# piljoong-jeong/nerf_meets_mlx

Hardware: AMD Instinct MI355X
Metric: train+render rays/sec on Lego 800x800 (synthetic), coarse+fine 64+128 (higher is better)
Workload: dtype split16 (fp16x2 render / bf16x2 train MFMA operands ~ 22 / 16 significand bits; fp32 accumulate)

## Files before the change

nerf_meets_mlx_amd/csrc/mlp.hip:

```cpp
#include "common.h"
#include "mlp_ring.h"
#include "mlp_layout.h"
#include "mlp_frag.h"
#include "mlp_arch2.h"
#include "mlp_input2.h"
#include "mlp_pack.h"
#include "hash_common.h"
#include "mlp_params.h"
#include "mlp_model.h"
#include "dw_split.h"
#include <limits.h>
#include <string.h>


namespace nerf {

extern int g_hash_combine_max_res;







// ... 781 lines not shown
      const int n = t - nw;
      src = base + 64 * 1024 + n;
      dst = a.grads + jb.b_off + n;
      if (jb.aux_row0 > 0) {
        if (n >= jb.aux_row0) dst = a.aux + (jb.n_valid - jb.aux_row0) * jb.k_valid + (n - jb.aux_row0);
        else if (n >= jb.n_grad) continue;
      }
    }
    float sum = 0.0f;
    int sidx = 0;
    for (; sidx + 8 <= S; sidx += 8) {
      float v[8];
#pragma unroll
      for (int q = 0; q < 8; ++q) v[q] = __builtin_nontemporal_load(src + (size_t)(sidx + q) * DW_SLOT_FLOATS);
#pragma unroll
      for (int q = 0; q < 8; ++q) sum += v[q];
    }
    for (; sidx < S; ++sidx) sum += __builtin_nontemporal_load(src + (size_t)sidx * DW_SLOT_FLOATS);
    *dst = sum;
  }
}



static_assert(LI::F_CHUNKS * RING_CHUNK == LI::F_TOTAL && LI::B_CHUNKS * RING_CHUNK == LI::B_PADDED, "whole ring chunks");

template <bool STORE, class WS>
__device__ __forceinline__ void fwd_tiles_img(const ImgArgs& a, WS& ws, int64_t tile0, int64_t ntiles, int lane) {
  constexpr int ST = 1;
  const int r = lane & 31, h = lane >> 5;
  int64_t tile = tile0 < ntiles ? tile0 : ntiles - 1;
  int64_t m = tile * 32 + r; if (m >= a.M) m = a.M - 1;
  bf16x8 xin[ST][3];
#pragma unroll
  for (int ks = 0; ks < 3; ++ks) row_pairs<CvtBf16>(a.x + m * LI::CIN, ks, h, LI::CIN, xin[0][ks]);
  int bad = nonfinite_flags<32>(nonfinite_bits(xin[0][0]) | nonfinite_bits(xin[0][1]) | nonfinite_bits(xin[0][2]), 0u);
  asm volatile("" : "+v"(bad));
  if (STORE) { store_frags<3>(a.acts, tile0, a.astride, LI::A_X, xin[0], r, h); ws.note_stores(3); }
  bf16x8 ha[ST][16], hb[ST][16];
  u32x4 mk[ST];
#define IMG_LAYER(KS, FB, BS, IN, OUT, LYR)                                                        \
  do { mk[0] = u32x4{0u, 0u, 0u, 0u};                                                              \
       layer_fwd<ST, KS, 8, true, STORE>(ws, FB, BS, IN, OUT, mk, lane);                           \
       if (STORE) { store_frags<16>(a.acts, tile0, a.astride, LI::A_H0 + 16 * (LYR), OUT[0], r, h); \
                    *reinterpret_cast<u32x4*>(frag_ptr(a.acts, tile0, a.astride, LI::A_MASK + (LYR), r, h)) = mk[0]; ws.note_stores(17); } } while (0)
  IMG_LAYER(3, LI::F_L0, 0, xin, ha, 0);
  IMG_LAYER(16, LI::F_L1 + 0 * 128, 256, ha, hb, 1);
  IMG_LAYER(16, LI::F_L1 + 1 * 128, 512, hb, ha, 2);
  IMG_LAYER(16, LI::F_L1 + 2 * 128, 768, ha, hb, 3);
  IMG_LAYER(16, LI::F_L1 + 3 * 128, 1024, hb, ha, 4);
  {
    bf16x8 cat[ST][19];
    if (STORE) {
#pragma unroll
      for (int k = 0; k < 3; ++k) xin[0][k] = *frag_ptr(a.acts, tile0, a.astride, LI::A_X + k, r, h);
    }
#pragma unroll
    for (int k = 0; k < 3; ++k) cat[0][k] = xin[0][k];
#pragma unroll
    for (int k = 0; k < 16; ++k) cat[0][3 + k] = ha[0][k];
    IMG_LAYER(19, LI::F_L5, 1280, cat, hb, 5);
  }
  IMG_LAYER(16, LI::F_L6, 1536, hb, ha, 6);
  IMG_LAYER(16, LI::F_L7, 1792, ha, hb, 7);
#undef IMG_LAYER
  f32x16 acc;
  acc_init_bias(acc, ws, LI::BI_OUT, h);
#pragma unroll
  for (int ks = 0; ks < 16; ++ks) {
    const bf16x8 wo = next_frag(ws, LI::F_OUT + ks, lane);
    acc = __builtin_amdgcn_mfma_f32_32x32x16_bf16(wo, hb[0][ks], acc, 0, 0, 0);
  }
  const int64_t mo = tile0 * 32 + r;
  if (h == 0 && tile0 < ntiles && mo < a.M) {
#pragma unroll
    for (int c = 0; c < 4; ++c)
      if (c < a.out_ch) a.out[mo * a.out_ch + c] = bad ? __builtin_nanf("") : acc[c];
  }
}

template <bool STORE>
__global__ void __launch_bounds__(512, 2) mlp_img_fwd_ring_kernel(ImgArgs a) {
  const int lane = threadIdx.x & 63;
  const int wv = __builtin_amdgcn_readfirstlane(threadIdx.x >> 6);
  const int64_t ntiles = (a.M + 31) >> 5, nsuper = (ntiles + 7) >> 3;
  RingW<LI::F_CHUNKS, LI::F_TOTAL, (STORE ? 2 : 4)> ws;
  ws.wsrc = reinterpret_cast<const char*>(a.wf);
  ws.lane16 = 16 * lane;
  ws.lds0 = __builtin_amdgcn_readfirstlane(lds_addr_of(ring_smem));
  ws.wv = wv;
  ws.start(lane);
  ring_load_bias(a.bias, LI::BI_TOTAL);
  __syncthreads();
  for (int64_t sp = blockIdx.x; sp < nsuper; sp += gridDim.x) {
    int ln = lane;
    asm volatile("" : "+v"(ln));
    ws.new_pass();
    fwd_tiles_img<STORE>(a, ws, sp * 8 + wv, ntiles, ln);
  }
  ws.drain();
}

__global__ void __launch_bounds__(512, 2) mlp_img_bwd_ring_kernel(ImgArgs a) {
  constexpr int ST = 1;
  const int lane0 = threadIdx.x & 63;
  const int wv = __builtin_amdgcn_readfirstlane(threadIdx.x >> 6);
  const int64_t ntiles = (a.M + 31) >> 5, nsuper = (ntiles + 7) >> 3;
  RingW<LI::B_CHUNKS, LI::B_TOTAL> ws;
  ws.wsrc = reinterpret_cast<const char*>(a.wb);
  ws.lane16 = 16 * lane0;
  ws.lds0 = __builtin_amdgcn_readfirstlane(lds_addr_of(ring_smem));
  ws.wv = wv;
  ws.start(lane0);
  for (int64_t sp = blockIdx.x; sp < nsuper; sp += gridDim.x) {
    int lane = lane0;
    asm volatile("" : "+v"(lane));
    ws.new_pass();
    const int r = lane & 31, h = lane >> 5;
    const int64_t tile0 = sp * 8 + wv;
    const int64_t tile = tile0 < ntiles ? tile0 : ntiles - 1;
    const int64_t m = tile * 32 + r;
    bf16x8 zo[ST][1];
#pragma unroll
    for (int j = 0; j < 8; ++j) zo[0][0][j] = (__bf16)0.0f;
    if (tile0 < ntiles && m < a.M && h == 0) {
#pragma unroll
      for (int c = 0; c < 4; ++c)
        if (c < a.out_ch) zo[0][0][c] = (__bf16)a.d_out[m * a.out_ch + c];
    }
    u32x4 mk[8][ST];
#pragma unroll
    for (int l = 0; l < 8; ++l)
      mk[l][0] = *reinterpret_cast<const u32x4*>(frag_ptr(a.acts, tile, a.astride, LI::A_MASK + l, r, h));
    store_frags<1>(a.dz, tile0, a.zstride, LI::Z_OUT, zo[0], r, h); ws.note_stores(1);
    bf16x8 za[ST][16], zb[ST][16];
    layer_bwd<ST, 1, 8, true>(ws, LI::B_OUT, zo, zb, mk[7], lane);
    store_frags<16>(a.dz, tile0, a.zstride, LI::Z_L0 + 112, zb[0], r, h); ws.note_stores(16);
    layer_bwd<ST, 16, 8, true>(ws, LI::B_L7 + 0 * 128, zb, za, mk[6], lane);
    store_frags<16>(a.dz, tile0, a.zstride, LI::Z_L0 + 96, za[0], r, h); ws.note_stores(16);
    layer_bwd<ST, 16, 8, true>(ws, LI::B_L7 + 1 * 128, za, zb, mk[5], lane);
    store_frags<16>(a.dz, tile0, a.zstride, LI::Z_L0 + 80, zb[0], r, h); ws.note_stores(16);
    layer_bwd<ST, 16, 8, true>(ws, LI::B_L7 + 2 * 128, zb, za, mk[4], lane);
    store_frags<16>(a.dz, tile0, a.zstride, LI::Z_L0 + 64, za[0], r, h); ws.note_stores(16);
    layer_bwd<ST, 16, 8, true>(ws, LI::B_L7 + 3 * 128, za, zb, mk[3], lane);
    store_frags<16>(a.dz, tile0, a.zstride, LI::Z_L0 + 48, zb[0], r, h); ws.note_stores(16);
    layer_bwd<ST, 16, 8, true>(ws, LI::B_L7 + 4 * 128, zb, za, mk[2], lane);
    store_frags<16>(a.dz, tile0, a.zstride, LI::Z_L0 + 32, za[0], r, h); ws.note_stores(16);
    layer_bwd<ST, 16, 8, true>(ws, LI::B_L7 + 5 * 128, za, zb, mk[1], lane);
    store_frags<16>(a.dz, tile0, a.zstride, LI::Z_L0 + 16, zb[0], r, h); ws.note_stores(16);
    layer_bwd<ST, 16, 8, true>(ws, LI::B_L7 + 6 * 128, zb, za, mk[0], lane);
    store_frags<16>(a.dz, tile0, a.zstride, LI::Z_L0 + 0, za[0], r, h); ws.note_stores(16);
  }
  ws.drain();
}



struct LdsW {
  __device__ __forceinline__ bf16x8 frag(int f, int lane) { return *reinterpret_cast<const bf16x8*>(ring_smem + f * 1024 + lane * 16); }
  __device__ __forceinline__ void note_stores(int) {}
  __device__ __forceinline__ float4 bias4(int slot) { return *reinterpret_cast<const float4*>(ring_smem + 32 * 1024 + slot * 4); }
};
__device__ __forceinline__ void lds_load_stream(const bf16x8* __restrict__ w, const float* __restrict__ bias) {
  for (int i = threadIdx.x; i < 32 * 64; i += blockDim.x) *reinterpret_cast<bf16x8*>(ring_smem + i * 16) = w[i];
  if (bias)
    for (int i = threadIdx.x; i < LN::BI_TOTAL; i += blockDim.x) *reinterpret_cast<float*>(ring_smem + 32 * 1024 + 4 * i) = bias[i];
  __syncthreads();
}


template <bool STORE, bool FUSED, bool LW = false>
__global__ void __launch_bounds__(512) mlp_small_fwd_kernel(SmallArgs a) {
  constexpr int ST = 1;
  lds_load_stream(a.wf, a.bias);
  const int lane0 = threadIdx.x & 63, wv = threadIdx.x >> 6;
  const bool rmaj = FUSED && !STORE && a.ray_major;
  const int64_t ntiles = rmaj ? ((a.B + 31) >> 5) * a.n : (a.M + 31) >> 5;
  LdsW ws;
  for (int64_t tile0 = (int64_t)blockIdx.x * 8 + wv; tile0 < ntiles; tile0 += (int64_t)gridDim.x * 8) {
    int lane = lane0;
    asm volatile("" : "+v"(lane));
    const int r = lane & 31, h = lane >> 5;
    const TileSample ts = small_tile_sample(a, tile0, r, rmaj);
    const int64_t m = ts.m;
    const bool valid = ts.valid;
    bf16x8 in[3];
    if (FUSED) {
      if (a.tables_h) ngp_row<true, LW, CvtBf16>(a, m, h, in);
      else ngp_row<false, LW, CvtBf16>(a, m, h, in);
    } else {
      small_row<CvtBf16>(a.x + m * LN::CIN, h, in);
    }
    bf16x8 xin[ST][2], din[ST][1];
    xin[0][0] = in[0]; xin[0][1] = in[1]; din[0][0] = in[2];
    int bad = nonfinite_flags<32>(nonfinite_bits(xin[0][0]) | nonfinite_bits(xin[0][1]), nonfinite_bits(din[0][0]));
    asm volatile("" : "+v"(bad));
#define SINK(slot0) FragSink<STORE>{a.acts, tile0, a.astride, slot0, r, h}
#define MASK_STORE(layer) do { if (STORE) *reinterpret_cast<u32x4*>(frag_ptr(a.acts, tile0, a.astride, LN::A_MASK + (layer), r, h)) = mk[0]; } while (0)
    if (STORE) { store_frags<2>(a.acts, tile0, a.astride, LN::A_X, xin[0], r, h); store_frags<1>(a.acts, tile0, a.astride, LN::A_DX, din[0], r, h); }
    u32x4 mk[ST];
    bf16x8 h0[ST][4], h1[ST][4], ft[ST][4];
    mk[0] = u32x4{0u, 0u, 0u, 0u};
    layer_fwd<ST, 2, 2, true, STORE>(ws, LN::F_L0, LN::BI_L0, xin, h0, mk, lane, SINK(LN::A_H0));
    MASK_STORE(0);
    mk[0] = u32x4{0u, 0u, 0u, 0u};
    layer_fwd<ST, 4, 2, true, STORE>(ws, LN::F_L1, LN::BI_L1, h0, h1, mk, lane, SINK(LN::A_H1));
    MASK_STORE(1);
    layer_fwd<ST, 4, 2, false, false>(ws, LN::F_FA, LN::BI_FEAT, h1, ft, mk, lane, SINK(LN::A_FEAT));
    float alpha;
    {
      f32x16 acc;
      acc_init_bias(acc, ws, LN::BI_ALPHA, h);
#pragma unroll
      for (int ks = 0; ks < 4; ++ks) acc = __builtin_amdgcn_mfma_f32_32x32x16_bf16(ws.frag(LN::F_FA + 8 + ks, lane), h1[0][ks], acc, 0, 0, 0);
      alpha = acc[0];
    }
    bf16x8 hd[ST][2];
    {
      bf16x8 cat[ST][5];
#pragma unroll
      for (int k = 0; k < 4; ++k) cat[0][k] = ft[0][k];
      cat[0][4] = din[0][0];
      mk[0] = u32x4{0u, 0u, 0u, 0u};
      layer_fwd<ST, 5, 1, true, STORE>(ws, LN::F_DIR, LN::BI_DIR, cat, hd, mk, lane, SINK(LN::A_HD));
      MASK_STORE(2);
    }
    {
      f32x16 acc;
      acc_init_bias(acc, ws, LN::BI_RGB, h);
#pragma unroll
      for (int ks = 0; ks < 2; ++ks) acc = __builtin_amdgcn_mfma_f32_32x32x16_bf16(ws.frag(LN::F_RGB + ks, lane), hd[0][ks], acc, 0, 0, 0);
      if (h == 0 && valid) {
        float4 o; o.x = acc[0]; o.y = acc[1]; o.z = acc[2]; o.w = alpha;
        *reinterpret_cast<float4*>(a.out + m * 4) = poison_raw(o, bad);
      }
    }
#undef SINK
#undef MASK_STORE
  }
}

__global__ void __launch_bounds__(512) mlp_small_bwd_kernel(SmallArgs a) {
  constexpr int ST = 1;
  lds_load_stream(a.wb, nullptr);
  const int lane0 = threadIdx.x & 63, wv = threadIdx.x >> 6;
  const int64_t ntiles = (a.M + 31) >> 5;
  LdsW ws;
  for (int64_t tile0 = (int64_t)blockIdx.x * 8 + wv; tile0 < ntiles; tile0 += (int64_t)gridDim.x * 8) {
    int lane = lane0;
    asm volatile("" : "+v"(lane));
    const int r = lane & 31, h = lane >> 5;
    const int64_t m = tile0 * 32 + r;
    float4 g = make_float4(0.f, 0.f, 0.f, 0.f);
    if (m < a.M && h == 0) g = *reinterpret_cast<const float4*>(a.d_raw + m * 4);
    bf16x8 zrgb[ST][1], zal[ST][1];
#pragma unroll
    for (int j = 0; j < 8; ++j) { zrgb[0][0][j] = (__bf16)0.0f; zal[0][0][j] = (__bf16)0.0f; }
    zrgb[0][0][0] = (__bf16)g.x; zrgb[0][0][1] = (__bf16)g.y; zrgb[0][0][2] = (__bf16)g.z;
    zal[0][0][0] = (__bf16)g.w;
    u32x4 mk[3][ST];
#pragma unroll
    for (int l = 0; l < 3; ++l)
      mk[l][0] = *reinterpret_cast<const u32x4*>(frag_ptr(const_cast<void*>(a.acts), tile0, a.astride, LN::A_MASK + l, r, h));
    store_frags<1>(a.dz, tile0, a.zstride, LN::Z_RGB, zrgb[0], r, h);
    store_frags<1>(a.dz, tile0, a.zstride, LN::Z_A, zal[0], r, h);
#define ZSINK(slot0) FragSink<true>{a.dz, tile0, a.zstride, slot0, r, h}
    bf16x8 zd[ST][2], zf[ST][4], z1[ST][4], z0[ST][4];
    layer_bwd<ST, 1, 1, true>(ws, LN::B_RGB, zrgb, zd, mk[2], lane, ZSINK(LN::Z_D));
    layer_bwd<ST, 2, 2, false>(ws, LN::B_DIR, zd, zf, mk[2], lane, ZSINK(LN::Z_F));
    {
      bf16x8 cat[ST][5];
#pragma unroll
      for (int k = 0; k < 4; ++k) cat[0][k] = zf[0][k];
      cat[0][4] = zal[0][0];
      layer_bwd<ST, 5, 2, true>(ws, LN::B_FA, cat, z1, mk[1], lane, ZSINK(LN::Z_L1));
    }
    layer_bwd<ST, 4, 2, true>(ws, LN::B_L1, z1, z0, mk[0], lane, ZSINK(LN::Z_L0));
#undef ZSINK
    if (a.d_x) {
      f32x16 acc;
#pragma unroll
      for (int i = 0; i < 16; ++i) acc[i] = 0.0f;
#pragma unroll
      for (int ns = 0; ns < 4; ++ns) acc = __builtin_amdgcn_mfma_f32_32x32x16_bf16(ws.frag(LN::B_L0 + ns, lane), z0[0][ns], acc, 0, 0, 0);
      if (m < a.M) {
#pragma unroll
        for (int q = 0; q < 4; ++q) {
          float4 o; o.x = acc[4 * q]; o.y = acc[4 * q + 1]; o.z = acc[4 * q + 2]; o.w = acc[4 * q + 3];
          *reinterpret_cast<float4*>(a.d_x + m * LN::CPOS + 8 * q + 4 * h) = o;
        }
      }
    }
  }
}

static int g_dw_wgs = 0;
static int g_dw_bias = -1;
static int g_bwd_stage = 0;
static int g_dw_ring_cap = 8;
static int g_dw_private = 4;
static int g_dw16_variant = 1;
static int g_dw_narrow_first = 1;
static int g_dw_factor = 1;
static int g_dw_job_mask = 0;
static int g_mlp_variant = 0;
static int g_ring_wgs = 0;
static int g_ngp_ray_major = 1;
int g_pass_queue = 1;
static int g_ring_split = 1;

static int cu_count() {
  constexpr int MAX_DEVICES = 64;
  static int n[MAX_DEVICES] = {};
  int dev = 0;
  if (hipGetDevice(&dev) != hipSuccess || dev < 0 || dev >= MAX_DEVICES) dev = 0;
  if (n[dev] == 0) {
    int v = 0;
    n[dev] = (hipDeviceGetAttribute(&v, hipDeviceAttributeMultiprocessorCount, dev) == hipSuccess && v > 0) ? v : 256;
  }
  return n[dev];
}
static inline int ring_wgs() { return g_ring_wgs > 0 ? g_ring_wgs : cu_count(); }
static inline unsigned ring_grid(int64_t ntiles) { return persistent_grid((ntiles + 7) / 8, ring_wgs()); }

struct Option { const char* key; int* var; bool (*rule)(int& v); const char* refusal; };
static bool opt_any(int&) { return true; }
static bool opt_flag(int& v) { v = v ? 1 : 0; return true; }
template <int LO, int HI> static bool opt_clamp(int& v) { v = v < LO ? LO : v > HI ? HI : v; return true; }
static const Option OPTIONS[] = {
    {"mlp_variant", &g_mlp_variant, opt_any, nullptr},
    {"ring_split", &g_ring_split, [](int& v) { return v == 1 || v == 2; }, "nerf_set_option: ring_split must be 1 or 2"},
    {"ring_workgroups", &g_ring_wgs, opt_clamp<0, INT_MAX>, nullptr},
    {"tile_pad16", &g_tile_pad16, opt_clamp<0, INT_MAX>, nullptr},
    {"dw_workgroups", &g_dw_wgs, opt_clamp<0, INT_MAX>, nullptr},
    {"dw_unit_bias", &g_dw_bias, opt_clamp<-1, INT_MAX>, nullptr},
    {"bwd_stage", &g_bwd_stage, opt_any, nullptr},
    {"dw_job_mask", &g_dw_job_mask, opt_any, nullptr},
    {"hash_combine_max_res", &g_hash_combine_max_res, opt_clamp<0, INT_MAX>, nullptr},
    {"ngp_ray_major", &g_ngp_ray_major, opt_flag, nullptr},
    {"dw22_variant", &s16::g_dw_variant, opt_flag, nullptr},
    {"dw16_variant", &g_dw16_variant, opt_clamp<0, 3>, nullptr},
    {"dw_private_tiles", &g_dw_private, opt_clamp<0, 4>, nullptr},
    {"dw_ring_cap", &g_dw_ring_cap, opt_clamp<2, 16>, nullptr},
    {"pass_queue", &g_pass_queue, opt_flag, nullptr},
    {"dw_narrow_first", &g_dw_narrow_first, opt_flag, nullptr},
    {"dw_factor", &g_dw_factor, opt_flag, nullptr},
    {"f22_tiles", &f22::g_tiles, [](int& v) { return v == 0 || v == 2 || v == 3; }, "nerf_set_option: f22_tiles must be 0 (automatic), 2 or 3"},
};

}

using namespace nerf;

extern "C" int nerf_set_option(const char* key, int value) {
  NERF_REQUIRE(key, NERF_E_NULL, "nerf_set_option: key is NULL");
  NERF_REQUIRE(strcmp(key, "mlp_precision") != 0, NERF_E_UNSUPPORTED,
               "nerf_set_option: \"mlp_precision\" is gone (ABI 3): set nerf_mlp_arch.precision of the model instead");
  for (const Option& o : OPTIONS) {
    if (strcmp(key, o.key)) continue;
    if (!o.rule(value)) return fail(NERF_E_UNSUPPORTED, "%s", o.refusal);
    *o.var = value;
    return NERF_OK;
  }
  return fail(NERF_E_UNSUPPORTED, "nerf_set_option: unknown key '%s'", key);
}

extern "C" int nerf_get_option(const char* key) {
  if (!key) return NERF_OPTION_UNKNOWN;
  for (const Option& o : OPTIONS)
    if (!strcmp(key, o.key)) return *o.var;
  return NERF_OPTION_UNKNOWN;
}

extern "C" int64_t nerf_mlp_param_count(const nerf_mlp_arch* arch) { return resolve(arch).params; }
extern "C" int64_t nerf_mlp_packed_bytes(const nerf_mlp_arch* arch) { return resolve(arch).packed_bytes; }
extern "C" int64_t nerf_mlp_acts_bytes(const nerf_mlp_arch* arch, int64_t M) { return resolve(arch).acts_bytes(M); }
extern "C" int64_t nerf_mlp_dz_bytes(const nerf_mlp_arch* arch, int64_t M) { return resolve(arch).dz_bytes(M); }

#define NERF_ARCH_MSG ": HIP kernels exist for (8x256, skip 4) with in=63+27 view head, or in=40 / no view head / out_ch<=4, and for (2x64, no skip) with in=32+16 view head"
#define NERF_RESOLVE(who)        \
  const Model m = resolve(arch); \
  NERF_REQUIRE(m.ok, NERF_E_UNSUPPORTED, who NERF_ARCH_MSG)

extern "C" int nerf_mlp_pack(const nerf_mlp_arch* arch, const float* params, void* packed, void* stream) {
  NERF_RESOLVE("nerf_mlp_pack");
  NERF_REQUIRE(params && packed, NERF_E_NULL, "nerf_mlp_pack: params/packed is NULL");
  auto s = as_stream(stream);
  bf16x8* wf = m.stream<bf16x8>(packed, S_FWD);
  bf16x8* wb = m.stream<bf16x8>(packed, S_BWD);
  float* bias = m.stream<float>(packed, S_BIAS);
  int rc;
  if (m.shape == Shape::Small) {
    rc = launch<pack_streams_kernel<SmallPack, CvtBf16, true>>("nerf_mlp_pack (2x64 model)", dim3(pack_blocks<SmallPack, true>()), dim3(256), 0, s,
                                                               params, wf, wb, bias, 0);
    if (!rc && m.split()) rc = s16x::small_pack(params, m.stream<void>(packed, S_S16), s);
  } else if (m.shape == Shape::Image) {
    rc = launch<pack_streams_kernel<ImgPack, CvtBf16, true>>("nerf_mlp_pack (image model)", dim3(pack_blocks<ImgPack, true>()), dim3(256), 0, s,
                                                             params, wf, wb, bias, m.out_ch);
    if (!rc && m.split()) rc = s16x::img_pack(params, m.out_ch, m.stream<void>(packed, S_S16), s);
    if (!rc && m.prec == Prec::F32) rc = f32::pack(params, m.stream<void>(packed, S_F32), m.out_ch, s);
  } else {
    rc = launch<pack_kernel>("nerf_mlp_pack", dim3(PACK_BLOCKS + PACK16_BLOCKS), dim3(256), 0, s, params, wf, wb, bias,
                             m.stream<bf16x8>(packed, S_FWD16));
    if (!rc && m.prec == Prec::F32) rc = f32::pack(params, m.stream<void>(packed, S_F32), 0, s);
    if (!rc && m.split()) rc = f22::pack(params, m.stream<void>(packed, S_F22), s);
    if (!rc && m.split()) rc = s16::pack(params, m.stream<void>(packed, S_S16), s);
  }
  return rc;
}

template <int MODE>
static int launch_fwd(const Model& m, const void* packed, const float* x, const float* rays, const float* z, int64_t M, int n,
                      int freq_mode, float* out, void* acts, void* stream) {
  FwdArgs a;
  a.queue = nullptr;
  a.wf = m.stream<bf16x8>(packed, S_FWD);
  a.bias = m.stream<float>(packed, S_BIAS);
  a.x = x; a.rays = rays; a.z = z; a.M = M; a.n = n; a.out = out; a.acts = acts; a.astride = m.astride();
  fill_freqs(a.fr.pos, a.fr.dir, freq_mode);
  const int64_t ntiles = (M + 31) / 32;
  auto s = as_stream(stream);
  const int variant = (g_mlp_variant == 0) ? (MODE == 1 ? (acts ? 3 : 4) : 1) : g_mlp_variant;
  if ((variant == 4 || variant == 5) && MODE == 1 && !acts) {
    const dim3 g(persistent_grid((M + 255) / 256, ring_wgs()));
    FwdArgs a16 = a;
    a16.queue = passq_slot();
    a16.wf = m.stream<bf16x8>(packed, S_FWD16);
    const char* what = "mlp forward (ring, 16x16x32)";
    if (variant == 4) return launch<mlp_fwd_ring16_kernel<8, 2>, mlp_fwd_ring16_kernel<4, 4>>(what, g, dim3(512), RING16_LDS_BYTES, s, a16);
    return launch<mlp_fwd_ring16_kernel<4, 4>, mlp_fwd_ring16_kernel<8, 2>>(what, g, dim3(256), RING16_LDS_BYTES, s, a16);
  }
  if (variant >= 3 && MODE == 1) {
    a.queue = passq_slot();
    if (acts && g_ring_split == 2) {
      return launch<mlp_fwd_ring_kernel<1, true, SPLIT_NW, SPLIT_CHUNK>>(
          "mlp forward (ring, 2 workgroups per CU)", dim3(persistent_grid((ntiles + SPLIT_NW - 1) / SPLIT_NW, 2 * (int64_t)ring_wgs())),
          dim3(64 * SPLIT_NW), SPLIT_LDS_BYTES, s, a);
    }
    return with_bool(acts != nullptr, [&](auto store) {
      constexpr bool ST = decltype(store)::value;
      return launch<mlp_fwd_ring_kernel<1, ST>, mlp_fwd_ring_kernel<1, !ST>>("mlp forward (ring)", dim3(ring_grid(ntiles)), dim3(512),
                                                                              RING_LDS_BYTES, s, a);
    });
  }
  const int st = variant == 2 ? 2 : 1;
  const int64_t blocks = (ntiles + 4 * st - 1) / (4 * st);
  NERF_REQUIRE(blocks < (1ll << 31), NERF_E_SHAPE, "mlp forward: M too large");
  return with_bool(st == 1, [&](auto one) { return with_bool(acts != nullptr, [&](auto store) {
    return launch<mlp_fwd_kernel<decltype(one)::value ? 1 : 2, MODE, decltype(store)::value>>("mlp forward", dim3((unsigned)blocks), dim3(256),
                                                                                                0, s, a);
  }); });
}


static int view_forward(const Model& m, const void* packed, const float* x, const float* rays, const float* z, int64_t M, int n,
                        int freq_mode, float* out, void* acts, void* stream);

extern "C" int nerf_mlp_forward_train(const nerf_mlp_arch* arch, const void* packed, const float* x, int64_t M,
                                      float* out, void* acts, void* stream) {
  NERF_RESOLVE("nerf_mlp_forward");
  if (M <= 0) return NERF_OK;
  NERF_REQUIRE(packed && x && out, NERF_E_NULL, "nerf_mlp_forward: NULL pointer");
  auto s = as_stream(stream);
  if (m.shape == Shape::Small) {
    SmallArgs a;
    small_args(a, m, packed);
    a.x = x; a.out = out; a.acts = acts; a.M = M;
    if (m.split()) return s16x::small_forward(a, false, dim3(small_grid(small_tiles(a))), s);
    return with_bool(acts != nullptr, [&](auto store) {
      return launch<mlp_small_fwd_kernel<decltype(store)::value, false>>("mlp forward (2x64 model)", dim3(small_grid((M + 31) / 32)), dim3(512),
                                                                         LN::LDS_BYTES, s, a);
    });
  }
  if (m.shape == Shape::Image) {
    if (m.prec == Prec::F32)
      return f32::forward(m.stream<void>(packed, S_F32), x, nullptr, nullptr, M, 1, 0, out, acts, m.out_ch, s);
    ImgArgs a;
    img_args(a, m, packed);
    a.x = x; a.out = out; a.acts = acts; a.M = M;
    if (m.split()) return s16x::img_forward(a, ring_wgs(), s);
    return with_bool(acts != nullptr, [&](auto store) {
      constexpr bool ST = decltype(store)::value;
      return launch<mlp_img_fwd_ring_kernel<ST>, mlp_img_fwd_ring_kernel<!ST>>("mlp forward (image model)", dim3(ring_grid((M + 31) / 32)),
                                                                               dim3(512), RING_LDS_BYTES, s, a);
    });
  }
  return view_forward(m, packed, x, nullptr, nullptr, M, 1, 0, out, acts, stream);
}

static int view_forward(const Model& m, const void* packed, const float* x, const float* rays, const float* z, int64_t M, int n,
                        int freq_mode, float* out, void* acts, void* stream) {
  auto s = as_stream(stream);
  if (m.split() && !acts)
    return f22::forward(m.stream<void>(packed, S_F22), x, rays, z, M, n, freq_mode, out, ring_wgs(), s);
  if (m.split())
    return s16::forward(m.stream<void>(packed, S_S16), m.stream<float>(packed, S_BIAS), x, rays, z, M, n, freq_mode, out, acts,
                        m.astride(), ring_wgs(), s);
  if (m.prec == Prec::F32) return f32::forward(m.stream<void>(packed, S_F32), x, rays, z, M, n, freq_mode, out, acts, 0, s);
  return x ? launch_fwd<0>(m, packed, x, rays, z, M, n, freq_mode, out, acts, stream)
           : launch_fwd<1>(m, packed, x, rays, z, M, n, freq_mode, out, acts, stream);
}

extern "C" int nerf_mlp_forward(const nerf_mlp_arch* arch, const void* packed, const float* x, int64_t M, float* out,
                                void* stream) {
  return nerf_mlp_forward_train(arch, packed, x, M, out, nullptr, stream);
}

extern "C" int nerf_query_fused(const nerf_mlp_arch* arch, const void* packed, const float* rays, const float* z,
                                int64_t B, int n, int freq_mode, float* raw, void* acts, void* stream) {
  const Model m = resolve(arch);
  NERF_REQUIRE(m.ok && m.shape == Shape::View, NERF_E_UNSUPPORTED, "nerf_query_fused" NERF_ARCH_MSG);
  NERF_REQUIRE(n >= 1, NERF_E_SHAPE, "nerf_query_fused: n must be >= 1");
  if (B <= 0) return NERF_OK;
  NERF_REQUIRE(packed && rays && z && raw, NERF_E_NULL, "nerf_query_fused: NULL pointer");
  NERF_REQUIRE(freq_mode == 0 || freq_mode == 1, NERF_E_UNSUPPORTED, "nerf_query_fused: freq_mode must be 0 or 1");
  NERF_REQUIRE(B * (int64_t)n < (1ll << 31), NERF_E_SHAPE, "nerf_query_fused: B*n must be < 2^31 samples per call");
  return view_forward(m, packed, nullptr, rays, z, B * n, n, freq_mode, raw, acts, stream);
}

static int launch_dw_part(const Model& m, DwArgs& d, int nj, int64_t ntiles, const void* acts, void* dz, float* grads,
                          hipStream_t s, int kind, int slot_base, int max_wgs, int aux_slot = -1) {
  static_assert(DW_SPLIT_MAX_JOBS == DW_MAX_JOBS, "dw_split.h sizes its arrays for DwArgs::jobs");
  DwCost cost[DW_MAX_JOBS];
  constexpr int SHARED_JOB_EXTRA_UNITS = 12;
  for (int j = 0; j < nj; ++j) cost[j] = DwCost{d.jobs[j].nf, d.jobs[j].kf + (d.jobs[j].aux_row0 > 0 ? SHARED_JOB_EXTRA_UNITS : 0)};
  int target_wgs = g_dw_wgs > 0 ? g_dw_wgs : cu_count();
  if (target_wgs > max_wgs) target_wgs = max_wgs;
  const int nw = dw_split(cost, nj, g_dw_bias >= 0 ? g_dw_bias : m.split() ? 2 : 128, target_wgs, (ntiles + 3) / 4, d.splits);
  NERF_REQUIRE(slot_base + nw <= DW_MAX_WGS, NERF_E_SHAPE, "nerf_mlp_backward: dw_workgroups must be <= %d", DW_MAX_WGS);
  bool all_tiny = true;
  for (int j = 0; j < nj; ++j) all_tiny = all_tiny && ((d.jobs[j].nf + 1) / 2) * ((d.jobs[j].kf + 1) / 2) <= 4;
  d.ntiles = (int)ntiles; d.astride = m.astride(); d.zstride = m.zstride();
  d.acts = acts; d.dz = dz; d.grads = grads;
  d.a_lo = m.info->a_lo; d.z_lo = m.info->z_lo; d.ring_cap = g_dw_ring_cap; d.private_max_tiles = g_dw_private;
  d.partial = m.dw_partial(dz, ntiles) + (size_t)slot_base * DW_SLOT_FLOATS;
  d.aux = aux_slot >= 0 ? m.dw_partial(dz, ntiles) + (size_t)aux_slot * DW_SLOT_FLOATS : nullptr;
  int rc;
  if (kind >= 2) {
    rc = launch_dw_wide_kernel(d, nw, kind == 2, s);
  } else if (kind == 1) {
    rc = s16::launch_dw_kernel(d, nw, true, s);
  } else if (g_dw16_variant == 3 || (g_dw16_variant == 1 && all_tiny)) {
    rc = s16::launch_dw_kernel(d, nw, false, s);
  } else {
    rc = launch<mlp_dw_kernel>("mlp dW", dim3(nw), dim3(64 * DW_WAVES), DW_LDS_BYTES, s, d);
  }
  if (rc) return rc;
  return launch<mlp_dw_reduce_kernel>("mlp dW reduce", dim3(257, nj), dim3(256), 0, s, d);
}

static int launch_dw(const Model& m, const void* packed, DwArgs& d, int nj, int64_t ntiles, const void* acts, void* dz, float* grads,
                     hipStream_t s, bool factored) {
  if (g_dw_job_mask) {
    hipError_t e = hipMemsetAsync(grads, 0, sizeof(float) * m.params, s);
    if (e != hipSuccess) return fail(NERF_E_HIP, "nerf_mlp_backward: memset: %s", hipGetErrorString(e));
  }
  const bool split_bf16 = m.split();
  if ((split_bf16 ? s16::g_dw_variant : g_dw16_variant) == 0)
    return launch_dw_part(m, d, nj, ntiles, acts, dz, grads, s, split_bf16 ? 1 : 0, 0, DW_MAX_WGS);
  DwArgs wide = d, rest = d;
  int nwide = 0, nrest = 0;
  for (int j = 0; j < nj; ++j) {
    if (d.jobs[j].nf == 16 && d.jobs[j].kf == 16) wide.jobs[nwide++] = d.jobs[j];
    else rest.jobs[nrest++] = d.jobs[j];
  }
  const int half = DW_MAX_WGS / 2;
  for (int turn = 0; turn < 2; ++turn) {
    const bool do_wide = (turn == 0) != (g_dw_narrow_first != 0);
    if (do_wide && nwide) {
      const int rc = launch_dw_part(m, wide, nwide, ntiles, acts, dz, grads, s, split_bf16 ? 2 : 3, half, half);
      if (rc) return rc;
    }
    if (!do_wide && nrest) {
      int rc = launch_dw_part(m, rest, nrest, ntiles, acts, dz, grads, s, split_bf16 ? 1 : 0, 0, half, factored ? half : -1);
      if (!rc && factored)
        rc = launch_dw_factor_post(m.stream<void>(packed, S_S16), m.stream<float>(packed, S_BIAS), rest.aux, grads, s);
      if (rc) return rc;
    }
  }
  return NERF_OK;
}

static int view_backward_chain(const Model& m, const void* packed, const void* acts, const float* d_raw, int64_t M, void* dz,
                               hipStream_t s) {
  const int64_t ntiles = (M + 31) / 32;
  if (m.split()) {
    if (g_bwd_stage != 2) {
      const int rcs = s16::backward_chain(m.stream<void>(packed, S_S16), acts, d_raw, M, dz, m.astride(), m.zstride(), ring_wgs(), s);
      if (rcs) return rcs;
    }
    return check_launch("mlp backward chain");
  }
  BwdArgs b;
  b.queue = nullptr;
  b.wb = m.stream<bf16x8>(packed, S_BWD);
  b.acts = acts; b.d_raw = d_raw; b.M = M; b.dz = dz; b.astride = m.astride(); b.zstride = m.zstride();
  const int variant = g_mlp_variant == 0 ? 3 : g_mlp_variant;
  const char* what = "mlp backward chain";
  if (variant >= 3) {
    b.queue = passq_slot();
    if (g_bwd_stage == 2) return check_launch(what);
    if (g_ring_split == 2)
      return launch<mlp_bwd_ring_kernel<SPLIT_NW, SPLIT_CHUNK>>(
          what, dim3(persistent_grid((ntiles + SPLIT_NW - 1) / SPLIT_NW, 2 * (int64_t)ring_wgs())), dim3(64 * SPLIT_NW), SPLIT_LDS_BYTES, s, b);
    return launch<mlp_bwd_ring_kernel<>>(what, dim3(ring_grid(ntiles)), dim3(512), RING_LDS_BYTES, s, b);
  }
  const int st = variant == 2 ? 2 : 1;
  const int64_t blocks = (ntiles + 4 * st - 1) / (4 * st);
  return with_bool(st == 1, [&](auto one) {
    return launch<mlp_bwd_kernel<decltype(one)::value ? 1 : 2>>(what, dim3((unsigned)blocks), dim3(256), 0, s, b);
  });
}

static int mlp_backward_impl(const nerf_mlp_arch* arch, const void* packed, const void* acts, const float* d_raw,
                             int64_t M, void* dz, float* grads, float* d_x, void* stream) {
  NERF_RESOLVE("nerf_mlp_backward");
  NERF_REQUIRE(!d_x || m.shape == Shape::Small, NERF_E_UNSUPPORTED,
               "nerf_mlp_backward_inputs: input gradients exist for the (2x64) model only (the 8x256 models take fixed encodings)");
  NERF_REQUIRE(packed && acts && d_raw && dz && grads, NERF_E_NULL, "nerf_mlp_backward: NULL pointer");
  NERF_REQUIRE(M > 0, NERF_E_SHAPE, "nerf_mlp_backward: M must be > 0");
  auto s = as_stream(stream);
  const int64_t ntiles = (M + 31) / 32;
  if (m.prec == Prec::F32)
    return f32::backward(m.stream<void>(packed, S_F32), acts, d_raw, M, dz, grads, m.shape == Shape::Image ? m.out_ch : 0, s);
  int rc;
  if (m.shape == Shape::Small) {
    SmallArgs a;
    small_args(a, m, packed);
    a.d_raw = d_raw; a.acts = const_cast<void*>(acts); a.dz = dz; a.M = M; a.d_x = d_x;
    if (m.split()) rc = s16x::small_backward_chain(a, s);
    else rc = launch<mlp_small_bwd_kernel>("mlp backward chain (2x64 model)", dim3(small_grid(ntiles)), dim3(512), LN::LDS_BYTES, s, a);
  } else if (m.shape == Shape::Image) {
    ImgArgs a;
    img_args(a, m, packed);
    a.d_out = d_raw; a.acts = const_cast<void*>(acts); a.dz = dz; a.M = M;
    if (m.split()) rc = s16x::img_backward_chain(a, ring_wgs(), s);
    else rc = launch<mlp_img_bwd_ring_kernel>("mlp backward chain (image model)", dim3(ring_grid(ntiles)), dim3(512), RING_LDS_BYTES, s, a);
  } else {
    rc = view_backward_chain(m, packed, acts, d_raw, M, dz, s);
    if (!rc && g_bwd_stage == 1) return NERF_OK;
  }
  if (rc) return rc;
  DwArgs d;
  const int mask = m.shape == Shape::View ? g_dw_job_mask : 0;
  const bool factored = g_dw_factor && m.can_factor() && !mask && s16::g_dw_variant != 0;
  const int nj = m.dw_jobs(d.jobs, mask, factored);
  return launch_dw(m, packed, d, nj, ntiles, acts, dz, grads, s, factored);
}

static int ngp_query_fused_impl(const nerf_mlp_arch* arch, const void* packed, const float* rays, const float* z,
                                int64_t B, int n, const float* tables, const void* tables_half, int L, int log2_T, int F,
                                const int* resolutions_host, const float* lw_host, int sh_degree, float pos_scale,
                                float pos_offset, float* raw, void* acts, void* stream) {
  const Model m = resolve(arch);
  NERF_REQUIRE(m.ok && m.shape == Shape::Small, NERF_E_UNSUPPORTED, "nerf_ngp_query_fused: needs the (2x64, in 32+16) model");
  NERF_REQUIRE(L == 16 && F == 2 && sh_degree == 3, NERF_E_UNSUPPORTED,
               "nerf_ngp_query_fused: fused rows exist for 16 levels x 2 features + SH degree 3 (use nerf_ngp_encode + nerf_mlp_forward otherwise)");
  NERF_REQUIRE(log2_T >= 1 && log2_T <= 30, NERF_E_SHAPE, "nerf_ngp_query_fused: need 1<=log2_T<=30");
  if (B <= 0 || n <= 0) return NERF_OK;
  NERF_REQUIRE(packed && rays && z && tables && resolutions_host && raw, NERF_E_NULL, "nerf_ngp_query_fused: NULL pointer");
  const int64_t M = B * n;
  NERF_REQUIRE(M < (1ll << 31), NERF_E_SHAPE, "nerf_ngp_query_fused: B*n must be < 2^31");
  LevelTab lt;
  if (lw_host)
    NERF_REQUIRE(level_tab_fill(lt, lw_host, L), NERF_E_SHAPE, "nerf_ngp_query_fused_lw: level weights must be finite and in [0, 1]");
  SmallArgs a;
  small_args(a, m, packed);
  a.out = raw; a.acts = acts; a.M = M; a.rays = rays; a.z = z; a.n = n; a.tables = tables; a.T = 1u << log2_T;
  a.pos_scale = pos_scale; a.pos_offset = pos_offset;
  for (int l = 0; l < L; ++l) a.rt.res[l] = (float)resolutions_host[l];
  if (lw_host) a.lw = lt;
  a.B = B;
  a.ray_major = small_ray_major(acts != nullptr, g_ngp_ray_major, B);
  const dim3 g(small_grid(small_tiles(a)));
  if (m.split()) return s16x::small_forward(a, lw_host != nullptr, g, as_stream(stream));
  a.tables_h = static_cast<const uint32_t*>(tables_half);
  return with_bool(acts != nullptr, [&](auto store) { return with_bool(lw_host != nullptr, [&](auto lw) {
    return launch<mlp_small_fwd_kernel<decltype(store)::value, true, decltype(lw)::value>>(
        lw_host ? "nerf_ngp_query_fused_lw" : "nerf_ngp_query_fused", g, dim3(512), LN::LDS_BYTES, as_stream(stream), a);
  }); });
}

extern "C" int nerf_ngp_query_fused_h(const nerf_mlp_arch* arch, const void* packed, const float* rays, const float* z,
                                      int64_t B, int n, const float* tables, const void* tables_half, int L, int log2_T, int F,
                                      const int* resolutions_host, int sh_degree, float pos_scale, float pos_offset,
                                      float* raw, void* acts, void* stream) {
  return ngp_query_fused_impl(arch, packed, rays, z, B, n, tables, tables_half, L, log2_T, F, resolutions_host, nullptr, sh_degree,
                              pos_scale, pos_offset, raw, acts, stream);
}

extern "C" int nerf_ngp_query_fused_lw(const nerf_mlp_arch* arch, const void* packed, const float* rays, const float* z,
                                       int64_t B, int n, const float* tables, const void* tables_half, int L, int log2_T, int F,
                                       const int* resolutions_host, const float* level_weights_host, int sh_degree,
                                       float pos_scale, float pos_offset, float* raw, void* acts, void* stream) {
  return ngp_query_fused_impl(arch, packed, rays, z, B, n, tables, tables_half, L, log2_T, F, resolutions_host, level_weights_host,
                              sh_degree, pos_scale, pos_offset, raw, acts, stream);
}

extern "C" int nerf_ngp_query_fused(const nerf_mlp_arch* arch, const void* packed, const float* rays, const float* z,
                                    int64_t B, int n, const float* tables, int L, int log2_T, int F,
                                    const int* resolutions_host, int sh_degree, float pos_scale, float pos_offset,
                                    float* raw, void* acts, void* stream) {
  return nerf_ngp_query_fused_h(arch, packed, rays, z, B, n, tables, nullptr, L, log2_T, F, resolutions_host, sh_degree, pos_scale,
                                pos_offset, raw, acts, stream);
}

extern "C" int nerf_mlp_backward(const nerf_mlp_arch* arch, const void* packed, const void* acts, const float* d_raw,
                                 int64_t M, void* dz, float* grads, void* stream) {
  return mlp_backward_impl(arch, packed, acts, d_raw, M, dz, grads, nullptr, stream);
}

extern "C" int nerf_mlp_backward_inputs(const nerf_mlp_arch* arch, const void* packed, const void* acts,
                                        const float* d_raw, int64_t M, void* dz, float* grads, float* d_x,
                                        void* stream) {
  NERF_REQUIRE(d_x, NERF_E_NULL, "nerf_mlp_backward_inputs: d_x is NULL");
  return mlp_backward_impl(arch, packed, acts, d_raw, M, dz, grads, d_x, stream);
}

namespace nerf {
__global__ void __launch_bounds__(256) decode_frags_kernel(const void* base, int64_t stride16, int slot0, int nfrag,
                                                           int64_t M, float* __restrict__ out, int lo_off) {
  const int64_t total = M * nfrag * 2;
  for (int64_t t = blockIdx.x * (int64_t)blockDim.x + threadIdx.x; t < total; t += (int64_t)gridDim.x * blockDim.x) {
    const int h = (int)(t & 1), ks = (int)((t >> 1) % nfrag);
    const int64_t m = t / (2 * nfrag);
    const bf16x8 v = *frag_ptr(const_cast<void*>(base), m >> 5, stride16, slot0 + ks, (int)(m & 31), h);
#pragma unroll
    for (int j = 0; j < 8; ++j) out[m * (16 * nfrag) + kperm(ks, h, j)] = (float)v[j];
    if (lo_off > 0) {
      const bf16x8 w = *frag_ptr(const_cast<void*>(base), m >> 5, stride16, slot0 + lo_off + ks, (int)(m & 31), h);
#pragma unroll
      for (int j = 0; j < 8; ++j) out[m * (16 * nfrag) + kperm(ks, h, j)] += (float)w[j];
    }
  }
}
}

extern "C" int nerf_mlp_debug_width(const nerf_mlp_arch* arch, int kind, int layer) {
  const Model m = resolve(arch);
  if (!m.ok) return -1;
  if (m.prec == Prec::F32) return f32::debug_width(kind, layer);
  const DebugSlot ds = m.debug_slot(kind, layer);
  return ds.nfrag ? 16 * ds.nfrag : -1;
}

extern "C" int nerf_mlp_debug_read(const nerf_mlp_arch* arch, const void* store, int kind, int layer, int64_t M,
                                   float* out, void* stream) {
  NERF_RESOLVE("nerf_mlp_debug_read");
  if (m.prec == Prec::F32) {
    NERF_REQUIRE(store && out, NERF_E_NULL, "nerf_mlp_debug_read: NULL pointer");
    return M <= 0 ? NERF_OK : f32::debug_read(store, kind, layer, M, out, as_stream(stream));
  }
  const DebugSlot ds = m.debug_slot(kind, layer);
  NERF_REQUIRE(ds.nfrag, NERF_E_SHAPE, "nerf_mlp_debug_read: no such (kind, layer) in this architecture's stores");
  NERF_REQUIRE(store && out, NERF_E_NULL, "nerf_mlp_debug_read: NULL pointer");
  if (M <= 0) return NERF_OK;
  const int lo_off = !m.split() ? 0 : kind == 0 ? m.info->a_lo : m.info->z_lo;
  return launch<decode_frags_kernel>("nerf_mlp_debug_read", dim3(grid_for(M * ds.nfrag * 2, 256)), dim3(256), 0, as_stream(stream), store,
                                     kind == 0 ? m.astride() : m.zstride(), ds.slot, ds.nfrag, M, out, lo_off);
}

NERF_STAMP2_EXPORT(nerf_debug_stamps2_ring16)
#ifdef NERF_CLOCK_STAMP
extern "C" int nerf_debug_stamps(unsigned long long* host_out, int nwg) {
  if (nwg > 4096) nwg = 4096;
  return hipMemcpyFromSymbol(host_out, HIP_SYMBOL(nerf::g_stamps), (size_t)nwg * 32) == hipSuccess ? 0 : -4;
}
#endif
```

nerf_meets_mlx_amd/csrc/mlp_dwf.hip:

```cpp
#include "common.h"
#include "launch.h"
#include "mlp_frag.h"

namespace nerf {

constexpr int DWF_ROWS = 2;
constexpr int DWF_BLOCKS_F = 256 / DWF_ROWS, DWF_BLOCKS_D = 128 / DWF_ROWS;

__device__ __forceinline__ double pair_value(const __bf16* __restrict__ wf, const FragElem& e) {
  FragElem hi = e, lo = e;
  hi.f = 2 * e.f; lo.f = 2 * e.f + 1;
  return (double)(float)wf[frag_elem_offset(hi)] + (double)(float)wf[frag_elem_offset(lo)];
}

__global__ void __launch_bounds__(256) mlp_dw_factor_post_kernel(const __bf16* __restrict__ wf, const float* __restrict__ bias,
                                                                 const float* __restrict__ aux, float* __restrict__ grads) {
  __shared__ double sh[256 * DWF_ROWS];
  __shared__ double sdb[128];
  const int t = threadIdx.x;
  const float* G = aux + DWF_G;
  const float* dbD = aux + DWF_DB;
  double acc[DWF_ROWS];
#pragma unroll
  for (int q = 0; q < DWF_ROWS; ++q) acc[q] = 0.0;
  if (blockIdx.x < DWF_BLOCKS_F) {
    const int k0 = DWF_ROWS * blockIdx.x;
    for (int e = t; e < 128 * DWF_ROWS; e += 256) {
      const int j = e / DWF_ROWS, q = e % DWF_ROWS;
      sh[e] = pair_value(wf, fwd_elem_dir0(j, k0 + q));
    }
    if (t < 128) sdb[t] = (double)dbD[t];
    __syncthreads();
    for (int j = 0; j < 128; ++j) {
      const double g = (double)G[j * 256 + t];
#pragma unroll
      for (int q = 0; q < DWF_ROWS; ++q) acc[q] = __builtin_fma(sh[j * DWF_ROWS + q], g, acc[q]);
    }
#pragma unroll
    for (int q = 0; q < DWF_ROWS; ++q) grads[L::P_WF + (k0 + q) * 256 + t] = (float)acc[q];
    if (t < DWF_ROWS) {
      double b = 0.0;
      for (int j = 0; j < 128; ++j) b = __builtin_fma(sh[j * DWF_ROWS + t], sdb[j], b);
      grads[L::P_BF + k0 + t] = (float)b;
    }
  } else {
    const int j0 = DWF_ROWS * (blockIdx.x - DWF_BLOCKS_F);
    for (int e = t; e < 256 * DWF_ROWS; e += 256) {
      const int q = e / 256, i = e % 256;
      sh[i * DWF_ROWS + q] = (double)G[(j0 + q) * 256 + i];
    }
    __syncthreads();
    for (int ks = 0; ks < 16; ++ks) {
      for (int h = 0; h < 2; ++h) {
        const FragElem e0 = fwd_elem_feature(t, kperm(ks, h, 0));
        FragElem eh = e0, el = e0;
        eh.f = 2 * e0.f; el.f = 2 * e0.f + 1;
        const bf16x8 vh = *reinterpret_cast<const bf16x8*>(wf + frag_elem_offset(eh));
        const bf16x8 vl = *reinterpret_cast<const bf16x8*>(wf + frag_elem_offset(el));
#pragma unroll
        for (int jj = 0; jj < 8; ++jj) {
          const double w = (double)(float)vh[jj] + (double)(float)vl[jj];
          const int i = kperm(ks, h, jj);
#pragma unroll
          for (int q = 0; q < DWF_ROWS; ++q) acc[q] = __builtin_fma(w, sh[i * DWF_ROWS + q], acc[q]);
        }
      }
    }
    const double bf = (double)bias[L::BI_FEAT + t];
#pragma unroll
    for (int q = 0; q < DWF_ROWS; ++q) grads[L::P_WD + (j0 + q) * 283 + t] = (float)__builtin_fma(bf, (double)dbD[j0 + q], acc[q]);
    if (t < DWF_ROWS) grads[L::P_BD + j0 + t] = dbD[j0 + t];
  }
}

int launch_dw_factor_post(const void* packed_s16, const float* bias_slots, const float* aux, float* grads, hipStream_t s) {
  return launch<mlp_dw_factor_post_kernel>("mlp dW post step (factored feature / dir0)", dim3(DWF_BLOCKS_F + DWF_BLOCKS_D), dim3(256), 0, s,
                                           static_cast<const __bf16*>(packed_s16), bias_slots, aux, grads);
}

}
```

nerf_meets_mlx_amd/csrc/mlp_frag.h:

```cpp
#pragma once
#include "mlp_layout.h"

namespace nerf {


__device__ __forceinline__ bf16x8* frag_ptr(void* base, int64_t tile, int64_t stride16, int slot, int r, int h) {
  char* tb = reinterpret_cast<char*>(base) + tile * stride16 * 16;
  return reinterpret_cast<bf16x8*>(tb + slot * 1024 + (unsigned)(32 * r + 16 * h));
}

#ifndef NERF_NT_STORES
#define NERF_NT_STORES 1
#endif
constexpr bool g_nt_stores = NERF_NT_STORES != 0;

__device__ __forceinline__ void store_frag(void* base, int64_t tile, int64_t stride16, int slot, const bf16x8& v,
                                           int r, int h) {
#if NERF_ABLATE == 7
  asm volatile("" :: "v"(v));
  return;
#endif
#if NERF_ABLATE == 8
  tile = tile & 7;
#endif
  if (g_nt_stores) __builtin_nontemporal_store(v, frag_ptr(base, tile, stride16, slot, r, h));
  else *frag_ptr(base, tile, stride16, slot, r, h) = v;
}
template <int COUNT>
__device__ __forceinline__ void store_frags(void* base, int64_t tile, int64_t stride16, int slot0,
                                            const bf16x8 (&frags)[COUNT], int r, int h) {
#pragma unroll
  for (int k = 0; k < COUNT; ++k) store_frag(base, tile, stride16, slot0 + k, frags[k], r, h);
}
struct NoSink {
  __device__ __forceinline__ void put(int, int, const bf16x8&) const {}
};
template <bool ON>
struct FragSink {
  void* base; int64_t tile0, stride16; int slot0, r, h;
  __device__ __forceinline__ void put(int t, int idx, const bf16x8& v) const {
    if (ON) store_frag(base, tile0 + t, stride16, slot0 + idx, v, r, h);
  }
};

template <class WS>
__device__ __forceinline__ void acc_init_bias(f32x16& acc, WS& ws, int slot_tile, int h) {
#pragma unroll
  for (int g = 0; g < 4; ++g) {
    const float4 b = ws.bias4(slot_tile + 8 * g + 4 * h);
    acc[4 * g + 0] = b.x; acc[4 * g + 1] = b.y; acc[4 * g + 2] = b.z; acc[4 * g + 3] = b.w;
  }
}

typedef unsigned int u32x4 __attribute__((ext_vector_type(4)));

typedef short s16x2 __attribute__((ext_vector_type(2)));
typedef __bf16 bf16x2 __attribute__((ext_vector_type(2)));
typedef float f32x2 __attribute__((ext_vector_type(2)));
__device__ __forceinline__ bf16x2 pack2(float a, float b) {
  const f32x2 v = {a, b};
  return __builtin_convertvector(v, bf16x2);
}
struct PackBf16 {
  static __device__ __forceinline__ void pack(const float (&v)[8], bf16x8& o) {
#pragma unroll
    for (int j = 0; j < 8; j += 2) { const bf16x2 a = pack2(v[j], v[j + 1]); o[j] = a[0]; o[j + 1] = a[1]; }
  }
};
struct CvtBf16 {
  static constexpr int FRAGS = 1;
  static __device__ __forceinline__ void pack(const float (&v)[8], bf16x8& o) {
#pragma unroll
    for (int j = 0; j < 8; ++j) o[j] = (__bf16)v[j];
  }
};
__device__ __forceinline__ bf16x2 relu_pack(float a, float b) {
  s16x2 q = __builtin_bit_cast(s16x2, pack2(a, b));
  const s16x2 zero = {0, 0};
  q = __builtin_elementwise_max(q, zero);
  return __builtin_bit_cast(bf16x2, q);
}
__device__ __forceinline__ unsigned nonfinite_bits(const bf16x8& f) {
  const u32x4 w = __builtin_bit_cast(u32x4, f);
  unsigned b = 0;
#pragma unroll
  for (int i = 0; i < 4; ++i) b |= (w[i] & 0x7F807F80u) + 0x00800080u;
  return b & 0x80008000u;
}
template <int XOR_MASKS>
__device__ __forceinline__ int nonfinite_flags(unsigned pos_bits, unsigned dir_bits) {
  const unsigned long long mp = __ballot(pos_bits != 0u), md = __ballot(dir_bits != 0u);
  const int lane = (int)__lane_id();
  int f = 0;
#pragma unroll
  for (int x = 0; x < 64; x += 16)
    if ((x & ~XOR_MASKS) == 0) f |= (int)((mp >> (lane ^ x)) & 1ull) | ((int)((md >> (lane ^ x)) & 1ull) << 1);
  return f;
}
__device__ __forceinline__ float4 poison_raw(float4 o, int flags) {
  const float qnan = __builtin_nanf("");
  if (flags) { o.x = qnan; o.y = qnan; o.z = qnan; }
  if (flags & 1) o.w = qnan;
  return o;
}

__device__ __forceinline__ unsigned nonzero_bits(bf16x2 p) {
  unsigned r;
  asm("v_pk_min_u16 %0, %1, 1 op_sel_hi:[1,0]" : "=v"(r) : "v"(__builtin_bit_cast(unsigned, p)));
  return r;
}
template <int B>
__device__ __forceinline__ bf16x2 keep_where(bf16x2 p, unsigned w) {
  unsigned sel, r;
  asm("v_pk_lshrrev_b16 %0, %2, %1 op_sel_hi:[0,1]" : "=v"(sel) : "v"(w), "n"(B));
  sel &= 0x00010001u;
  asm("v_pk_mul_lo_u16 %0, %1, %2" : "=v"(r) : "v"(__builtin_bit_cast(unsigned, p)), "v"(sel));
  return __builtin_bit_cast(bf16x2, r);
}

template <bool RELU, bool MASKOUT>
__device__ __forceinline__ void finish_quarter(const f32x16& acc, int q, int nt, bf16x8& lo, bf16x8& hi, u32x4& mask) {
  unsigned w = 0;
#pragma unroll
  for (int p = 0; p < 2; ++p) {
    const int i = 4 * q + 2 * p, k = 2 * q + p;
    const bf16x2 pr = RELU ? relu_pack(acc[i], acc[i + 1]) : pack2(acc[i], acc[i + 1]);
    if (MASKOUT) w |= nonzero_bits(pr) << k;
    if (i < 8) { lo[i] = pr[0]; lo[i + 1] = pr[1]; } else { hi[i - 8] = pr[0]; hi[i - 7] = pr[1]; }
  }
  if (MASKOUT) mask[nt >> 1] |= w << (8 * (nt & 1));
}

__host__ __device__ constexpr int quarter_pos(int ks_count, int q) {
  return ks_count >= 8 ? (q * ks_count) / 4 + 1 : (q < ks_count ? q : ks_count - 1);
}

struct DwJob {
  int dz_slot, nf;
  int act_slot, kf;
  int w_off, ldw, col0;
  int n_valid, k_valid;
  int b_off;
  int n_grad, aux_row0;
};
constexpr int DW_MAX_JOBS = 16;
struct DwArgs {
  DwJob jobs[DW_MAX_JOBS];
  int splits[DW_MAX_JOBS];
  int ntiles;
  int64_t astride, zstride;
  const void* acts;
  const void* dz;
  float* grads;
  float* partial;
  int ring_cap;
  int private_max_tiles;
  int a_lo, z_lo;
  float* aux;
};
constexpr int DW_SLOT_FLOATS = 64 * 1024 + 256;
constexpr int DW_MAX_WGS = 512;
constexpr int64_t DW_PARTIAL_BYTES = (int64_t)DW_MAX_WGS * DW_SLOT_FLOATS * 4;
constexpr int DWF_G = 0, DWF_DB = 128 * 256, DWF_FLOATS = DWF_DB + 128;
static_assert(DWF_FLOATS <= DW_SLOT_FLOATS, "the factored job's result fits one partial-tile slot");
int launch_dw_factor_post(const void* packed_s16, const float* bias_slots, const float* aux, float* grads, hipStream_t s);
int launch_dw_wide_kernel(const DwArgs& d, int workgroups, bool split_bf16, hipStream_t s);

}
```

nerf_meets_mlx_amd/csrc/mlp_index.h:

```cpp
#pragma once
#if !defined(__HIPCC__) && !defined(__host__)
#define __host__
#define __device__
#endif
#include "mlp_params.h"

namespace nerf {

namespace L {
constexpr int F_L0 = 0, F_L1 = 32, F_L5 = 544, F_L6 = 704, F_L7 = 832, F_FA = 960, F_DIR = 1104, F_RGB = 1176;
constexpr int F_TOTAL = 1184;
constexpr int B_RGB = 0, B_DIR = 4, B_FA = 68, B_L7 = 204, B_L6 = 332, B_L5 = 460, B_L4 = 588;
constexpr int B_TOTAL = 1100, B_PADDED = 1120;
constexpr int BI_FEAT = 2048, BI_ALPHA = 2304, BI_DIR = 2336, BI_RGB = 2464, BI_TOTAL = 2496;
}

__host__ __device__ constexpr int kperm(int ks, int h, int j) { return 16 * ks + 8 * (j >> 2) + 4 * h + (j & 3); }
__host__ __device__ constexpr int kperm_ks(int kk) { return kk >> 4; }
__host__ __device__ constexpr int kperm_h(int kk) { return (kk >> 2) & 1; }
__host__ __device__ constexpr int kperm_j(int kk) { return 4 * ((kk >> 3) & 1) + (kk & 3); }

__host__ __device__ constexpr int kperm16(int ks, int g, int j) { return 32 * ks + 16 * (j >> 2) + 4 * g + (j & 3); }
__host__ __device__ constexpr int pos_chan16(int ks, int g, int j) {
  const int sl = 8 * ks + j;
  if (sl < 12) return 3 + 6 * (2 * g + sl / 6) + (sl % 6);
  if (sl < 15) return 3 + 6 * (8 + (g >> 1)) + 3 * (g & 1) + (sl - 12);
  return g < 3 ? g : -1;
}
__host__ __device__ constexpr int dir_chan16(int g, int j) {
  if (j < 6) return 3 + 6 * g + j;
  return (j == 6 && g < 3) ? g : -1;
}

__host__ __device__ constexpr int fwd_index(int f, int r, int h, int j) {
  if (f < L::F_L1) {
    const int nt = f / 4, ks = f % 4;
    const int kk = kperm(ks, h, j);
    return kk < 63 ? L::P_W0 + (32 * nt + r) * 63 + kk : -1;
  }
  if (f < L::F_L5) {
    const int l = 1 + (f - L::F_L1) / 128, g = (f - L::F_L1) % 128;
    const int nt = g / 16, ks = g % 16;
    return L::pw(l) + (32 * nt + r) * 256 + kperm(ks, h, j);
  }
  if (f < L::F_L6) {
    const int g = f - L::F_L5;
    const int nt = g / 20, ks = g % 20;
    const int kk = kperm(ks, h, j), n = 32 * nt + r;
    if (kk < 64) return kk < 63 ? L::P_W5 + n * 319 + kk : -1;
    return L::P_W5 + n * 319 + 63 + (kk - 64);
  }
  if (f < L::F_FA) {
    const int l = 6 + (f - L::F_L6) / 128, g = (f - L::F_L6) % 128;
    const int nt = g / 16, ks = g % 16;
    return L::pw(l) + (32 * nt + r) * 256 + kperm(ks, h, j);
  }
  if (f < L::F_DIR) {
    const int g = f - L::F_FA;
    const int nt = g / 16, ks = g % 16;
    const int kk = kperm(ks, h, j);
    if (nt < 8) return L::P_WF + (32 * nt + r) * 256 + kk;
    return r == 0 ? L::P_WA + kk : -1;
  }
  if (f < L::F_RGB) {
    const int g = f - L::F_DIR;
    const int nt = g / 18, ks = g % 18;
    const int kk = kperm(ks, h, j), n = 32 * nt + r;
    if (kk < 256) return L::P_WD + n * 283 + kk;
    return (kk - 256) < 27 ? L::P_WD + n * 283 + kk : -1;
  }
  const int ks = f - L::F_RGB;
  return r < 3 ? L::P_WR + r * 128 + kperm(ks, h, j) : -1;
}

__host__ __device__ constexpr int bwd_index(int f, int r, int h, int j) {
  if (f < L::B_DIR) {
    const int nn = kperm(0, h, j);
    return nn < 3 ? L::P_WR + nn * 128 + 32 * f + r : -1;
  }
  if (f < L::B_FA) {
    const int g = f - L::B_DIR, kt = g / 8, ns = g % 8;
    return L::P_WD + kperm(ns, h, j) * 283 + 32 * kt + r;
  }
  if (f < L::B_L7) {
    const int g = f - L::B_FA, kt = g / 17, ns = g % 17;
    const int nn = kperm(ns, h, j);
    if (ns < 16) return L::P_WF + nn * 256 + 32 * kt + r;
    return nn == 256 ? L::P_WA + 32 * kt + r : -1;
  }
  const int g = f - L::B_L7, li = g / 128, q = g % 128, kt = q / 16, ns = q % 16;
  const int l = 7 - li, nn = kperm(ns, h, j), row = 32 * kt + r;
  if (l == 5) return L::P_W5 + nn * 319 + 63 + row;
  return L::pw(l) + nn * 256 + row;
}

__host__ __device__ constexpr int bias_index(int s) {
  if (s < L::BI_FEAT) return L::pb(s >> 8) + (s & 255);
  if (s < L::BI_ALPHA) return L::P_BF + (s - L::BI_FEAT);
  if (s < L::BI_DIR) return s == L::BI_ALPHA ? L::P_BA : -1;
  if (s < L::BI_RGB) return L::P_BD + (s - L::BI_DIR);
  return (s - L::BI_RGB) < 3 ? L::P_BR + (s - L::BI_RGB) : -1;
}
struct ViewPack {
  static constexpr int F_TOTAL = L::F_TOTAL, F_PADDED = L::F_TOTAL, B_TOTAL = L::B_TOTAL, B_PADDED = L::B_PADDED, BI_TOTAL = L::BI_TOTAL;
  static __host__ __device__ constexpr int fwd(int f, int r, int h, int j, int) { return fwd_index(f, r, h, j); }
  static __host__ __device__ constexpr int bwd(int f, int r, int h, int j, int) { return bwd_index(f, r, h, j); }
  static __host__ __device__ constexpr int bias(int s, int) { return bias_index(s); }
};
template <class S>
__host__ __device__ constexpr int pack_index(bool fw, int f, int r, int h, int j, int out_ch) {
  if (f >= (fw ? S::F_TOTAL : S::B_TOTAL)) return -1;
  return fw ? S::fwd(f, r, h, j, out_ch) : S::bwd(f, r, h, j, out_ch);
}

struct FragElem { int f, r, h, j; };
__host__ __device__ constexpr FragElem fwd_elem_feature(int row, int col) {
  return FragElem{L::F_FA + 16 * (row >> 5) + kperm_ks(col), row & 31, kperm_h(col), kperm_j(col)};
}
__host__ __device__ constexpr FragElem fwd_elem_dir0(int row, int col) {
  return FragElem{L::F_DIR + 18 * (row >> 5) + kperm_ks(col), row & 31, kperm_h(col), kperm_j(col)};
}
__host__ __device__ constexpr int frag_elem_offset(const FragElem& e) { return (e.f * 64 + 32 * e.h + e.r) * 8 + e.j; }

}
```

nerf_meets_mlx_amd/csrc/mlp_s16.h:

```cpp
#pragma once
#include <hip/hip_runtime.h>
#include <stdint.h>

namespace nerf {
struct DwArgs;
namespace s16 {

constexpr int A_LO = 158, A_MASK = 316, A_SLOTS = 325;
constexpr int Z_LO = 154, Z_SLOTS = 308;
constexpr int F_FRAGS = 2368, B_FRAGS = 2200, B_PADDED = 2208;
constexpr int64_t PACKED_BYTES = (int64_t)(F_FRAGS + B_PADDED) * 1024;

int pack(const float* params, void* packed_s16, hipStream_t s);
int forward(const void* packed_s16, const float* bias_slots, const float* x, const float* rays, const float* z, int64_t M,
            int n, int freq_mode, float* out, void* acts, int64_t astride16, int persistent_wgs, hipStream_t s);
int backward_chain(const void* packed_s16, const void* acts, const float* d_raw, int64_t M, void* dz, int64_t astride16,
                   int64_t zstride16, int persistent_wgs, hipStream_t s);
int launch_dw_kernel(const DwArgs& d, int workgroups, bool split_bf16, hipStream_t s);
extern int g_dw_variant;

}
}
```

nerf_meets_mlx_amd/csrc/mlp_s16.hip:

```cpp
#include "mlp_s16_dev.h"
#include "mlp_pack.h"
#include "mlp_s16.h"

#ifndef NERF_S16_RELOAD_PE
#define NERF_S16_RELOAD_PE 0
#endif

namespace nerf {
namespace s16 {

constexpr int F_CHUNKS = F_FRAGS / RING_CHUNK;
constexpr int B_CHUNKS = B_PADDED / RING_CHUNK;
static_assert(F_CHUNKS * RING_CHUNK == F_FRAGS && B_CHUNKS * RING_CHUNK == B_PADDED, "whole ring chunks");
static_assert(F_FRAGS == 2 * L::F_TOTAL && B_FRAGS == 2 * L::B_TOTAL, "pair streams");
static_assert(A_LO == L::A_MASK && A_MASK == 2 * L::A_MASK && A_SLOTS == A_MASK + 9, "activation slots");
static_assert(Z_LO == L::Z_SLOTS && Z_SLOTS == 2 * L::Z_SLOTS, "dZ slots");
constexpr int NW = 4;

typedef RingW<F_CHUNKS, F_FRAGS, 4, NW, RING_CHUNK, RING_STAGES, true> FwdRing;
typedef RingW<B_CHUNKS, B_FRAGS, 4, NW, RING_CHUNK, RING_STAGES, true> BwdRing;


struct ViewPairPack : ViewPack { static constexpr int B_PADDED = s16::B_PADDED / 2; };
static_assert(ViewPairPack::B_PADDED >= L::B_TOTAL, "the padded stream holds every transposed fragment");


template <int MODE, class WS>
__device__ __forceinline__ void fwd_tiles(const FwdArgs& a, WS& ws, int64_t tile0, int64_t ntiles, int lane, PassQueue& pq) {
  const int r = lane & 31, h = lane >> 5;
  bf16x8 peh[4], pel[4], dph[2], dpl[2];
  pq.ask(ws.wv, lane);
  {
    const int64_t tile = tile0 < ntiles ? tile0 : ntiles - 1;
    const int64_t m = clamp_sample(tile * 32 + r, a.M);
    if (MODE == 0) {
      const float* row = a.x + m * 90;
#pragma unroll
      for (int ks = 0; ks < 4; ++ks) row_pairs<SplitBf16>(row, ks, h, 63, peh[ks], pel[ks]);
#pragma unroll
      for (int ks = 0; ks < 2; ++ks) row_pairs<SplitBf16>(row + 63, ks, h, 27, dph[ks], dpl[ks]);
    } else {
      const Sample sm = load_sample(a.rays, a.z, m, a.n);
      encode_pairs<SinCodyWaite, SplitBf16, 0, 63, 10>(sm.p, a.fr.pos, h, peh[0], pel[0]); encode_pairs<SinCodyWaite, SplitBf16, 1, 63, 10>(sm.p, a.fr.pos, h, peh[1], pel[1]);
      encode_pairs<SinCodyWaite, SplitBf16, 2, 63, 10>(sm.p, a.fr.pos, h, peh[2], pel[2]); encode_pairs<SinCodyWaite, SplitBf16, 3, 63, 10>(sm.p, a.fr.pos, h, peh[3], pel[3]);
      encode_pairs<SinCodyWaite, SplitBf16, 0, 27, 4>(sm.d, a.fr.dir, h, dph[0], dpl[0]); encode_pairs<SinCodyWaite, SplitBf16, 1, 27, 4>(sm.d, a.fr.dir, h, dph[1], dpl[1]);
    }
  }
  pq.publish(ws.wv);
  store_frags<4>(a.acts, tile0, a.astride, L::A_PE, peh, r, h); store_frags<4>(a.acts, tile0, a.astride, A_LO + L::A_PE, pel, r, h);
  store_frags<2>(a.acts, tile0, a.astride, L::A_DPE, dph, r, h); store_frags<2>(a.acts, tile0, a.astride, A_LO + L::A_DPE, dpl, r, h);

  bf16x8 hah[16], hal[16], hbh[16], hbl[16];
  u32x4 mk;
#define SINK(slot0) PairSink{a.acts, tile0, a.astride, slot0, A_LO, r, h}
#define MASK_BEGIN() mk = u32x4{0u, 0u, 0u, 0u}
#define MASK_STORE(layer) *reinterpret_cast<u32x4*>(frag_ptr(a.acts, tile0, a.astride, A_MASK + (layer), r, h)) = mk
  MASK_BEGIN();
  layer_fwd<4, 8, true, true>(ws, L::F_L0, 0, peh, pel, hah, hal, mk, lane, SINK(L::A_H0));
  MASK_STORE(0);
  MASK_BEGIN();
  layer_fwd<16, 8, true, true>(ws, L::F_L1 + 0 * 128, 256, hah, hal, hbh, hbl, mk, lane, SINK(L::A_H0 + 16));
  MASK_STORE(1);
  MASK_BEGIN();
  layer_fwd<16, 8, true, true>(ws, L::F_L1 + 1 * 128, 512, hbh, hbl, hah, hal, mk, lane, SINK(L::A_H0 + 32));
  MASK_STORE(2);
  MASK_BEGIN();
  layer_fwd<16, 8, true, true>(ws, L::F_L1 + 2 * 128, 768, hah, hal, hbh, hbl, mk, lane, SINK(L::A_H0 + 48));
  MASK_STORE(3);
  MASK_BEGIN();
  layer_fwd<16, 8, true, true>(ws, L::F_L1 + 3 * 128, 1024, hbh, hbl, hah, hal, mk, lane, SINK(L::A_H0 + 64));
  MASK_STORE(4);
  {
    bf16x8 cth[20], ctl[20];
#pragma unroll
    for (int k = 0; k < 4; ++k) {
#if NERF_S16_RELOAD_PE
      cth[k] = *frag_ptr(a.acts, tile0, a.astride, L::A_PE + k, r, h);
      ctl[k] = *frag_ptr(a.acts, tile0, a.astride, A_LO + L::A_PE + k, r, h);
#else
      cth[k] = peh[k]; ctl[k] = pel[k];
#endif
    }
#pragma unroll
    for (int k = 0; k < 16; ++k) { cth[4 + k] = hah[k]; ctl[4 + k] = hal[k]; }
    MASK_BEGIN();
    layer_fwd<20, 8, true, true>(ws, L::F_L5, 1280, cth, ctl, hbh, hbl, mk, lane, SINK(L::A_H0 + 80));
    MASK_STORE(5);
  }
  MASK_BEGIN();
  layer_fwd<16, 8, true, true>(ws, L::F_L6, 1536, hbh, hbl, hah, hal, mk, lane, SINK(L::A_H0 + 96));
  MASK_STORE(6);
  MASK_BEGIN();
  layer_fwd<16, 8, true, true>(ws, L::F_L7, 1792, hah, hal, hbh, hbl, mk, lane, SINK(L::A_H0 + 112));
  MASK_STORE(7);
  layer_fwd<16, 8, false, false>(ws, L::F_FA, L::BI_FEAT, hbh, hbl, hah, hal, mk, lane, SINK(L::A_FEAT));
  const float alpha = head<16>(ws, L::F_FA + 128, L::BI_ALPHA, hbh, hbl, lane)[0];
  bf16x8 hdh[8], hdl[8];
  {
    bf16x8 cth[18], ctl[18];
#pragma unroll
    for (int k = 0; k < 16; ++k) { cth[k] = hah[k]; ctl[k] = hal[k]; }
#pragma unroll
    for (int k = 0; k < 2; ++k) {
#if NERF_S16_RELOAD_PE
      cth[16 + k] = *frag_ptr(a.acts, tile0, a.astride, L::A_DPE + k, r, h);
      ctl[16 + k] = *frag_ptr(a.acts, tile0, a.astride, A_LO + L::A_DPE + k, r, h);
#else
      cth[16 + k] = dph[k]; ctl[16 + k] = dpl[k];
#endif
    }
    MASK_BEGIN();
    layer_fwd<18, 4, true, true>(ws, L::F_DIR, L::BI_DIR, cth, ctl, hdh, hdl, mk, lane, SINK(L::A_HD));
    MASK_STORE(8);
  }
  const f32x16 rgb = head<8>(ws, L::F_RGB, L::BI_RGB, hdh, hdl, lane);
  const int64_t m = tile0 * 32 + r;
  if (h == 0 && tile0 < ntiles && m < a.M) {
    float4 o; o.x = rgb[0]; o.y = rgb[1]; o.z = rgb[2]; o.w = alpha;
    *reinterpret_cast<float4*>(a.out + m * 4) = o;
  }
#undef SINK
#undef MASK_BEGIN
#undef MASK_STORE
}

template <int MODE>
__global__ void __launch_bounds__(64 * NW) s16_fwd_kernel(FwdArgs a) {
  const int lane = threadIdx.x & 63;
  const int wv = __builtin_amdgcn_readfirstlane(threadIdx.x >> 6);
  const int64_t ntiles = (a.M + 31) >> 5, nsuper = (ntiles + NW - 1) / NW;
  FwdRing ws;
  ws.wsrc = reinterpret_cast<const char*>(a.wf);
  ws.lane16 = 16 * lane;
  ws.lds0 = __builtin_amdgcn_readfirstlane(lds_addr_of(ring_smem));
  ws.wv = wv;
  ws.start(lane);
  ring_load_bias(a.bias, L::BI_TOTAL, FwdRing::BIAS_OFF);
  __syncthreads();
  PassQueue pq;
  pq.init(a.queue, ws.lds0 + FwdRing::BIAS_OFF);
  for (int64_t sp = blockIdx.x; sp < nsuper;) {
    int ln = lane;
    asm volatile("" : "+v"(ln));
    ws.new_pass();
    fwd_tiles<MODE>(a, ws, sp * NW + wv, ntiles, ln, pq);
    sp = pq.next(sp);
  }
  ws.drain();
  pq.leave();
}


struct BwdArgs {
  unsigned* queue;
  const bf16x8* wb;
  const void* acts;
  const float* d_raw;
  int64_t M;
  void* dz;
  int64_t astride, zstride;
};

template <class WS>
__device__ __forceinline__ void bwd_tiles(const BwdArgs& a, WS& ws, int64_t tile0, int64_t ntiles, int lane, PassQueue& pq) {
  const int r = lane & 31, h = lane >> 5;
  const bool live = tile0 < ntiles;
  pq.ask(ws.wv, lane);
  const int64_t tile = live ? tile0 : ntiles - 1;
  bf16x8 zrh[1], zrl[1], zah[1], zal[1];
  {
    const int64_t m = tile * 32 + r;
    float4 g = make_float4(0.f, 0.f, 0.f, 0.f);
    if (live && m < a.M && h == 0) g = *reinterpret_cast<const float4*>(a.d_raw + m * 4);
    float vr[8] = {g.x, g.y, g.z, 0.f, 0.f, 0.f, 0.f, 0.f}, va[8] = {g.w, 0.f, 0.f, 0.f, 0.f, 0.f, 0.f, 0.f};
    split_slots<8>(vr, zrh, zrl);
    split_slots<8>(va, zah, zal);
  }
  pq.publish(ws.wv);
  u32x4 mk[9];
#pragma unroll
  for (int l = 0; l < 9; ++l)
    mk[l] = *reinterpret_cast<const u32x4*>(frag_ptr(const_cast<void*>(a.acts), tile, a.astride, A_MASK + l, r, h));
#define ZSINK(slot0) PairSink{a.dz, tile0, a.zstride, slot0, Z_LO, r, h}
  ZSINK(L::Z_RGB).put(0, zrh[0], zrl[0]);
  ZSINK(L::Z_A).put(0, zah[0], zal[0]);
  bf16x8 zdh[8], zdl[8];
  layer_bwd<1, 4, true>(ws, L::B_RGB, zrh, zrl, zdh, zdl, mk[8], lane, ZSINK(L::Z_D));
  bf16x8 zxh[16], zxl[16], zyh[16], zyl[16];
  layer_bwd<8, 8, false>(ws, L::B_DIR, zdh, zdl, zxh, zxl, mk[8], lane, ZSINK(L::Z_F));
  {
    bf16x8 cth[17], ctl[17];
#pragma unroll
    for (int k = 0; k < 16; ++k) { cth[k] = zxh[k]; ctl[k] = zxl[k]; }
    cth[16] = zah[0]; ctl[16] = zal[0];
    layer_bwd<17, 8, true>(ws, L::B_FA, cth, ctl, zyh, zyl, mk[7], lane, ZSINK(L::Z_L0 + 112));
  }
  layer_bwd<16, 8, true>(ws, L::B_L7, zyh, zyl, zxh, zxl, mk[6], lane, ZSINK(L::Z_L0 + 96));
  layer_bwd<16, 8, true>(ws, L::B_L6, zxh, zxl, zyh, zyl, mk[5], lane, ZSINK(L::Z_L0 + 80));
  layer_bwd<16, 8, true>(ws, L::B_L5, zyh, zyl, zxh, zxl, mk[4], lane, ZSINK(L::Z_L0 + 64));
  layer_bwd<16, 8, true>(ws, L::B_L4 + 0 * 128, zxh, zxl, zyh, zyl, mk[3], lane, ZSINK(L::Z_L0 + 48));
  layer_bwd<16, 8, true>(ws, L::B_L4 + 1 * 128, zyh, zyl, zxh, zxl, mk[2], lane, ZSINK(L::Z_L0 + 32));
  layer_bwd<16, 8, true>(ws, L::B_L4 + 2 * 128, zxh, zxl, zyh, zyl, mk[1], lane, ZSINK(L::Z_L0 + 16));
  layer_bwd<16, 8, true>(ws, L::B_L4 + 3 * 128, zyh, zyl, zxh, zxl, mk[0], lane, ZSINK(L::Z_L0 + 0));
#undef ZSINK
}

__global__ void __launch_bounds__(64 * NW) s16_bwd_kernel(BwdArgs a) {
  const int lane = threadIdx.x & 63;
  const int wv = __builtin_amdgcn_readfirstlane(threadIdx.x >> 6);
  const int64_t ntiles = (a.M + 31) >> 5, nsuper = (ntiles + NW - 1) / NW;
  BwdRing ws;
  ws.wsrc = reinterpret_cast<const char*>(a.wb);
  ws.lane16 = 16 * lane;
  ws.lds0 = __builtin_amdgcn_readfirstlane(lds_addr_of(ring_smem));
  ws.wv = wv;
  ws.start(lane);
  PassQueue pq;
  pq.init(a.queue, ws.lds0 + BwdRing::BIAS_OFF);
  for (int64_t sp = blockIdx.x; sp < nsuper;) {
    int ln = lane;
    asm volatile("" : "+v"(ln));
    ws.new_pass();
    bwd_tiles(a, ws, sp * NW + wv, ntiles, ln, pq);
    sp = pq.next(sp);
  }
  ws.drain();
  pq.leave();
}

#ifndef NERF_DWX
#define NERF_DWX 0
#endif
#if NERF_DWX & 4
#define DW_BARRIER() do {} while (0)
#else
#define DW_BARRIER() __builtin_amdgcn_s_barrier()
#endif
constexpr int DW_WAVES = 16, DW_NPW = 2;

__device__ __forceinline__ bf16x8 tr_pair(const char* blk, int hq, int fsel, int i16) {
  const int q = i16 >> 2, p = i16 & 3;
  const char* base = blk + 64 * (8 * hq + q) + 32 * fsel + 16 * (p & 1) + 8 * (p >> 1);
#if NERF_DWX & 2
  bf16x8 r; asm volatile("" : "=v"(r) : "v"(base)); return r;
#endif
  const s16x4 lo = __builtin_amdgcn_ds_read_tr16_b64_v4i16((__attribute__((address_space(3))) s16x4*)(base));
  const s16x4 hi = __builtin_amdgcn_ds_read_tr16_b64_v4i16((__attribute__((address_space(3))) s16x4*)(base + 256));
  union { struct { s16x4 a, b; } s; bf16x8 v; } cvt;
  cvt.s.a = lo; cvt.s.b = hi;
  return cvt.v;
}

constexpr int DW_LDS_BYTES = 160 * 1024;

constexpr int DWP_WAVE_BYTES = 10 * 1024;
template <int NT, int KT, bool SPLIT>
__device__ __forceinline__ void dw_private(const DwArgs& a, const DwJob& jb, int tile_lo, int tile_hi, char* smem, int wv, int lane) {
  constexpr int NP = 2 * (NT + KT);
  static_assert(NP * 1024 <= DWP_WAVE_BYTES && NT * KT <= 4, "wave-private dW: one stage per wave, at most four tiles");
  f32x16 acc[NT][KT];
#pragma unroll
  for (int i = 0; i < NT; ++i)
#pragma unroll
    for (int k = 0; k < KT; ++k)
#pragma unroll
      for (int e = 0; e < 16; ++e) acc[i][k][e] = 0.0f;
  float bsum[NT];
#pragma unroll
  for (int i = 0; i < NT; ++i) bsum[i] = 0.0f;
  const int g16 = lane >> 4, i16 = lane & 15, hq = g16 >> 1, fsel = g16 & 1;
  char* mine = smem + wv * DWP_WAVE_BYTES;
  const unsigned lds_mine = __builtin_amdgcn_readfirstlane(lds_addr_of(mine));
  const int src_row = lane >> 2, src_sel = (lane >> 1) & 1, src_half = lane & 1;
  const char* dzb = reinterpret_cast<const char*>(a.dz);
  const char* acb = reinterpret_cast<const char*>(a.acts);
  long long zstride_b = a.zstride * 16, astride_b = a.astride * 16;
  int z_lo = a.z_lo, a_lo = a.a_lo, dz_slot = jb.dz_slot, act_slot = jb.act_slot, nf = jb.nf, kf = jb.kf;
  asm volatile("" : "+s"(zstride_b), "+s"(astride_b), "+s"(z_lo), "+s"(a_lo), "+s"(dz_slot), "+s"(act_slot), "+s"(nf), "+s"(kf));
  const int ht_hi = SPLIT ? 2 * tile_hi : tile_hi;
  for (int ht = (SPLIT ? 2 * tile_lo : tile_lo) + wv; ht < ht_hi; ht += DW_WAVES) {
    asm volatile("s_waitcnt lgkmcnt(0)" ::: "memory");
#if !(NERF_DWX & 1)
    const int64_t tile = SPLIT ? ht >> 1 : ht;
    const unsigned row_off0 = (unsigned)(32 * ((SPLIT ? 16 * (ht & 1) : 0) + src_row) + 16 * src_half);
#pragma unroll
    for (int i = 0; i < NP; ++i) {
      const bool is_z = i < 2 * NT;
      const int j = is_z ? i : i - 2 * NT, nt_ = is_z ? NT : KT;
      const int lo_part = j >= nt_ ? 1 : 0, t = lo_part ? j - nt_ : j;
      const int nfr = is_z ? nf : kf;
      int fr = 2 * t + src_sel; if (fr >= nfr) fr = nfr - 1;
      const int slot = (is_z ? dz_slot + (SPLIT ? lo_part * z_lo : 0) : act_slot + (SPLIT ? lo_part * a_lo : 0)) + fr;
      const unsigned row_off = row_off0 + (SPLIT ? 0 : 512 * lo_part);
      dma_frag_nt((is_z ? dzb + tile * zstride_b : acb + tile * astride_b) + (int64_t)slot * 1024 + row_off, lds_mine + i * 1024);
    }
#endif
    asm volatile("s_waitcnt vmcnt(0)" ::: "memory");
    bf16x8 bh[KT], bl[KT];
#pragma unroll
    for (int k = 0; k < KT; ++k) {
      bh[k] = tr_pair(mine + (2 * NT + k) * 1024, hq, fsel, i16);
      bl[k] = tr_pair(mine + (2 * NT + KT + k) * 1024, hq, fsel, i16);
    }
#pragma unroll
    for (int i = 0; i < NT; ++i) {
      const bf16x8 ah = tr_pair(mine + i * 1024, hq, fsel, i16);
      const bf16x8 al = tr_pair(mine + (NT + i) * 1024, hq, fsel, i16);
#if !(NERF_DWX & 8)
      const bf16x2 ones = {(__bf16)1.0f, (__bf16)1.0f};
#pragma unroll
      for (int j = 0; j < 8; j += 2) {
        const bf16x2 ph = {ah[j], ah[j + 1]}, pl = {al[j], al[j + 1]};
        bsum[i] = __builtin_amdgcn_fdot2_f32_bf16(pl, ones, bsum[i], false);
        bsum[i] = __builtin_amdgcn_fdot2_f32_bf16(ph, ones, bsum[i], false);
      }
#endif
#if NERF_DWX & 16
      asm volatile("" :: "v"(ah), "v"(al), "v"(bh[0]), "v"(bl[0]));
#else
#pragma unroll
      for (int k = 0; k < KT; ++k) {
        if (SPLIT) {
          acc[i][k] = mfma32(al, bh[k], acc[i][k]);
          acc[i][k] = mfma32(ah, bl[k], acc[i][k]);
          acc[i][k] = mfma32(ah, bh[k], acc[i][k]);
        } else {
          acc[i][k] = mfma32(ah, bh[k], acc[i][k]);
          acc[i][k] = mfma32(al, bl[k], acc[i][k]);
        }
      }
#endif
    }
  }
  asm volatile("s_waitcnt vmcnt(0) lgkmcnt(0)" ::: "memory");
  float* xl = reinterpret_cast<float*>(smem);
  constexpr int GIVER_FLOATS = (NT * KT * 16 + NT) * 64;
#pragma unroll 1
  for (int h = DW_WAVES / 2; h >= 1; h >>= 1) {
    __builtin_amdgcn_s_barrier();
    if (wv >= h && wv < 2 * h) {
      float* dst = xl + (size_t)(wv - h) * GIVER_FLOATS + lane;
#pragma unroll
      for (int i = 0; i < NT; ++i) {
#pragma unroll
        for (int k = 0; k < KT; ++k)
#pragma unroll
          for (int e = 0; e < 16; ++e) dst[((i * KT + k) * 16 + e) * 64] = acc[i][k][e];
        dst[(NT * KT * 16 + i) * 64] = bsum[i];
      }
    }
    __builtin_amdgcn_s_barrier();
    if (wv < h) {
      const float* src = xl + (size_t)wv * GIVER_FLOATS + lane;
#pragma unroll
      for (int i = 0; i < NT; ++i) {
#pragma unroll
        for (int k = 0; k < KT; ++k)
#pragma unroll
          for (int e = 0; e < 16; ++e) acc[i][k][e] += src[((i * KT + k) * 16 + e) * 64];
        bsum[i] += src[(NT * KT * 16 + i) * 64];
      }
    }
  }
  if (wv != 0) return;
  const int rr = lane & 31, hh = lane >> 5;
  float* slot = a.partial + (size_t)blockIdx.x * DW_SLOT_FLOATS;
#pragma unroll
  for (int i = 0; i < NT; ++i) {
#pragma unroll
    for (int k = 0; k < KT; ++k) {
      float* tile = slot + (8 * i + k) * 1024;
#pragma unroll
      for (int e = 0; e < 16; ++e) tile[((e & 3) + 8 * (e >> 2) + 4 * hh) * 32 + rr] = acc[i][k][e];
    }
    if (jb.b_off >= 0) {
      const float tot = bsum[i] + __shfl_xor(bsum[i], 32, 64);
      if (hh == 0) slot[64 * 1024 + 32 * i + rr] = tot;
    }
  }
}

template <bool SPLIT>
__global__ void __launch_bounds__(64 * DW_WAVES) s16_dw_kernel(DwArgs a) {
  char* smem = ring_smem;
  int bj = blockIdx.x, job_id = 0;
  while (bj >= a.splits[job_id]) { bj -= a.splits[job_id]; ++job_id; }
  const DwJob jb = a.jobs[job_id];
  const int tile_lo = (int)((int64_t)a.ntiles * bj / a.splits[job_id]);
  const int tile_hi = (int)((int64_t)a.ntiles * (bj + 1) / a.splits[job_id]);
  const int tid = threadIdx.x, lane = tid & 63;
  const int wv = __builtin_amdgcn_readfirstlane(tid >> 6);
  const int n_tiles = (jb.nf + 1) >> 1, k_tiles = (jb.kf + 1) >> 1;
  const bool col_major = k_tiles <= 2;
  const int wr = col_major ? (wv & 3) : (wv >> 2), wc = col_major ? (wv >> 2) : (wv & 3);
  const int npairs = 2 * (n_tiles + k_tiles);
  if (a.private_max_tiles >= n_tiles * k_tiles && npairs * 1024 <= DWP_WAVE_BYTES) {
    switch (8 * n_tiles + k_tiles) {
      case 8 * 1 + 1: dw_private<1, 1, SPLIT>(a, jb, tile_lo, tile_hi, smem, wv, lane); return;
      case 8 * 1 + 2: dw_private<1, 2, SPLIT>(a, jb, tile_lo, tile_hi, smem, wv, lane); return;
      case 8 * 1 + 3: dw_private<1, 3, SPLIT>(a, jb, tile_lo, tile_hi, smem, wv, lane); return;
      case 8 * 1 + 4: dw_private<1, 4, SPLIT>(a, jb, tile_lo, tile_hi, smem, wv, lane); return;
      case 8 * 2 + 1: dw_private<2, 1, SPLIT>(a, jb, tile_lo, tile_hi, smem, wv, lane); return;
      case 8 * 2 + 2: dw_private<2, 2, SPLIT>(a, jb, tile_lo, tile_hi, smem, wv, lane); return;
      case 8 * 3 + 1: dw_private<3, 1, SPLIT>(a, jb, tile_lo, tile_hi, smem, wv, lane); return;
      case 8 * 4 + 1: dw_private<4, 1, SPLIT>(a, jb, tile_lo, tile_hi, smem, wv, lane); return;
      default: break;
    }
  }
  const bool active = (wr * DW_NPW < n_tiles) && (wc * 2 < k_tiles);
  const int kc = (k_tiles + 1) >> 1;
  int stride = npairs * 1024, ns = DW_LDS_BYTES / stride;
  if (ns > a.ring_cap) ns = a.ring_cap;
  const int cnt_w = (wv < npairs ? 1 : 0) + (wv + DW_WAVES < npairs ? 1 : 0);
  f32x16 acc[DW_NPW][2];
#pragma unroll
  for (int i = 0; i < DW_NPW; ++i)
#pragma unroll
    for (int k = 0; k < 2; ++k)
#pragma unroll
      for (int e = 0; e < 16; ++e) acc[i][k][e] = 0.0f;
  float bsum[2 * DW_NPW];
  bool own[2 * DW_NPW];
#pragma unroll
  for (int c = 0; c < 2 * DW_NPW; ++c) { bsum[c] = 0.0f; own[c] = (c % kc) == wc && !(NERF_DWX & 8); }
  const int g16 = lane >> 4, i16 = lane & 15, hq = g16 >> 1, fsel = g16 & 1;
  const unsigned lds0 = __builtin_amdgcn_readfirstlane(lds_addr_of(smem));
  const int src_row = lane >> 2, src_sel = (lane >> 1) & 1, src_half = lane & 1;
  const char* dzb = reinterpret_cast<const char*>(a.dz);
  const char* acb = reinterpret_cast<const char*>(a.acts);
  long long zstride_b = a.zstride * 16, astride_b = a.astride * 16;
  int z_lo = a.z_lo, a_lo = a.a_lo, dz_slot = jb.dz_slot, act_slot = jb.act_slot, nf = jb.nf, kf = jb.kf;
  asm volatile("" : "+s"(zstride_b), "+s"(astride_b), "+s"(z_lo), "+s"(a_lo), "+s"(dz_slot), "+s"(act_slot), "+s"(nf), "+s"(kf),
               "+s"(stride), "+s"(ns));

  auto issue = [&](int ht, int slot) {
#if NERF_DWX & 1
    return;
#endif
    const unsigned st = lds0 + __builtin_amdgcn_readfirstlane(slot) * stride;
    const int64_t tile = SPLIT ? ht >> 1 : ht;
    const unsigned row_off0 = (unsigned)(32 * ((SPLIT ? 16 * (ht & 1) : 0) + src_row) + 16 * src_half);
#pragma unroll
    for (int k = 0; k < DW_NPW; ++k) {
      const int i = wv + DW_WAVES * k;
      if (i < npairs) {
        const bool is_z = i < 2 * n_tiles;
        const int j = is_z ? i : i - 2 * n_tiles;
        const int nt_ = is_z ? n_tiles : k_tiles;
        const int lo_part = j >= nt_ ? 1 : 0;
        const int t = lo_part ? j - nt_ : j;
        const int nfr = is_z ? nf : kf;
        int fr = 2 * t + src_sel; if (fr >= nfr) fr = nfr - 1;
        const int slot_ = (is_z ? dz_slot + (SPLIT ? lo_part * z_lo : 0) : act_slot + (SPLIT ? lo_part * a_lo : 0)) + fr;
        const unsigned row_off = row_off0 + (SPLIT ? 0 : 512 * lo_part);
        const char* src = (is_z ? dzb + tile * zstride_b : acb + tile * astride_b) + (int64_t)slot_ * 1024 + row_off;
        dma_frag_nt(src, st + i * 1024);
      }
    }
  };
  auto process = [&](const char* st) {
    if (active) {
      bf16x8 bh[2], bl[2];
#pragma unroll
      for (int k = 0; k < 2; ++k) {
        const int kt = wc * 2 + k;
        const int b = 2 * n_tiles + (kt < k_tiles ? kt : 0);
        bh[k] = tr_pair(st + b * 1024, hq, fsel, i16);
        bl[k] = tr_pair(st + (b + k_tiles) * 1024, hq, fsel, i16);
      }
#pragma unroll
      for (int i = 0; i < DW_NPW; ++i) {
        const int nt = wr * DW_NPW + i;
        const int b = nt < n_tiles ? nt : 0;
        const bf16x8 ah = tr_pair(st + b * 1024, hq, fsel, i16);
        const bf16x8 al = tr_pair(st + (b + n_tiles) * 1024, hq, fsel, i16);
        const bf16x2 ones = {(__bf16)1.0f, (__bf16)1.0f};
        if (own[2 * i]) {
          asm volatile("" ::: "memory");
#pragma unroll
          for (int j = 0; j < 8; j += 2) { const bf16x2 q = {ah[j], ah[j + 1]}; bsum[2 * i] = __builtin_amdgcn_fdot2_f32_bf16(q, ones, bsum[2 * i], false); }
        }
        if (own[2 * i + 1]) {
          asm volatile("" ::: "memory");
#pragma unroll
          for (int j = 0; j < 8; j += 2) { const bf16x2 q = {al[j], al[j + 1]}; bsum[2 * i + 1] = __builtin_amdgcn_fdot2_f32_bf16(q, ones, bsum[2 * i + 1], false); }
        }
#if NERF_DWX & 16
        asm volatile("" :: "v"(ah), "v"(al), "v"(bh[0]), "v"(bl[0]), "v"(bh[1]), "v"(bl[1]));
#else
#pragma unroll
        for (int k = 0; k < 2; ++k) {
          if (SPLIT) {
            acc[i][k] = mfma32(al, bh[k], acc[i][k]);
            acc[i][k] = mfma32(ah, bl[k], acc[i][k]);
            acc[i][k] = mfma32(ah, bh[k], acc[i][k]);
          } else {
            acc[i][k] = mfma32(ah, bh[k], acc[i][k]);
            acc[i][k] = mfma32(al, bl[k], acc[i][k]);
          }
        }
#endif
      }
    }
  };
  auto wait_landed = [&](int younger) {
    switch (younger * cnt_w) {
#define NERF_VM_CASE(N) case N: asm volatile("s_waitcnt vmcnt(" #N ") lgkmcnt(0)" ::: "memory"); break;
      NERF_VM_CASE(0) NERF_VM_CASE(1) NERF_VM_CASE(2) NERF_VM_CASE(3) NERF_VM_CASE(4) NERF_VM_CASE(5) NERF_VM_CASE(6) NERF_VM_CASE(7)
      NERF_VM_CASE(8) NERF_VM_CASE(9) NERF_VM_CASE(10) NERF_VM_CASE(11) NERF_VM_CASE(12) NERF_VM_CASE(13) NERF_VM_CASE(14)
      NERF_VM_CASE(16) NERF_VM_CASE(18) NERF_VM_CASE(20) NERF_VM_CASE(22) NERF_VM_CASE(24) NERF_VM_CASE(26) NERF_VM_CASE(28)
#undef NERF_VM_CASE
      default: asm volatile("s_waitcnt vmcnt(0) lgkmcnt(0)" ::: "memory"); break;
    }
  };
  const int ht_lo = SPLIT ? 2 * tile_lo : tile_lo, n = SPLIT ? 2 * (tile_hi - tile_lo) : tile_hi - tile_lo;
  int issued = 0, slot_i = 0, slot_p = 0;
  for (; issued < ns && issued < n; ++issued) { issue(ht_lo + issued, slot_i); slot_i = slot_i + 1 == ns ? 0 : slot_i + 1; }
  for (int p = 0; p < n; p += 2) {
    wait_landed(issued - (p + 2 < n ? p + 2 : n));
    DW_BARRIER();
#pragma unroll
    for (int k = 0; k < 2; ++k)
      if (issued < n && issued - ns < p) { issue(ht_lo + issued, slot_i); slot_i = slot_i + 1 == ns ? 0 : slot_i + 1; ++issued; }
    process(smem + slot_p * stride); slot_p = slot_p + 1 == ns ? 0 : slot_p + 1;
    if (SPLIT || p + 1 < n) { process(smem + slot_p * stride); slot_p = slot_p + 1 == ns ? 0 : slot_p + 1; }
  }
  asm volatile("s_waitcnt lgkmcnt(0)" ::: "memory");
  __builtin_amdgcn_s_barrier();
  float* xb = reinterpret_cast<float*>(smem);
#pragma unroll
  for (int c = 0; c < 2 * DW_NPW; ++c)
    if (own[c] && active) xb[(wr * 2 * DW_NPW + c) * 64 + lane] = bsum[c];
  __builtin_amdgcn_s_barrier();
  if (!active) return;
  const int rr = lane & 31, hh = lane >> 5;
  float* slot = a.partial + (size_t)blockIdx.x * DW_SLOT_FLOATS;
#pragma unroll
  for (int i = 0; i < DW_NPW; ++i) {
    const int nt = wr * DW_NPW + i;
    if (nt >= n_tiles) continue;
#pragma unroll
    for (int k = 0; k < 2; ++k) {
      const int kt = wc * 2 + k;
      if (kt >= k_tiles) continue;
      float* tile = slot + (8 * nt + kt) * 1024;
#pragma unroll
      for (int e = 0; e < 16; ++e) tile[((e & 3) + 8 * (e >> 2) + 4 * hh) * 32 + rr] = acc[i][k][e];
    }
    if (wc == 0 && jb.b_off >= 0) {
      const float lo = xb[(wr * 2 * DW_NPW + 2 * i + 1) * 64 + lane], hi = xb[(wr * 2 * DW_NPW + 2 * i) * 64 + lane];
      const float t = lo + hi;
      const float tot = t + __shfl_xor(t, 32, 64);
      if (hh == 0) slot[64 * 1024 + 32 * nt + rr] = tot;
    }
  }
}


int pack(const float* params, void* packed_s16, hipStream_t s) {
  bf16x8* wf = static_cast<bf16x8*>(packed_s16);
  return launch<pack_streams_kernel<ViewPairPack, SplitBf16, false>>("nerf_mlp_pack (split-bf16 image)", dim3(pack_blocks<ViewPairPack, false>()),
                                                                     dim3(256), 0, s, params, wf, wf + (size_t)F_FRAGS * 64, nullptr, 0);
}

int forward(const void* packed_s16, const float* bias_slots, const float* x, const float* rays, const float* z, int64_t M,
            int n, int freq_mode, float* out, void* acts, int64_t astride16, int persistent_wgs, hipStream_t s) {
  FwdArgs a;
  a.queue = passq_slot();
  a.wf = reinterpret_cast<const bf16x8*>(packed_s16);
  a.bias = bias_slots;
  a.x = x; a.rays = rays; a.z = z; a.M = M; a.n = n; a.out = out; a.acts = acts; a.astride = astride16;
  fill_freqs(a.fr.pos, a.fr.dir, freq_mode);
  const int64_t nsuper = ((M + 31) / 32 + NW - 1) / NW;
  return with_bool(x != nullptr, [&](auto rows) {
    return launch<s16_fwd_kernel<decltype(rows)::value ? 0 : 1>>("mlp training forward (split bf16)", dim3(persistent_grid(nsuper, persistent_wgs)),
                                                                  dim3(64 * NW), FwdRing::LDS_BYTES, s, a);
  });
}

int backward_chain(const void* packed_s16, const void* acts, const float* d_raw, int64_t M, void* dz, int64_t astride16,
                   int64_t zstride16, int persistent_wgs, hipStream_t s) {
  BwdArgs b;
  b.queue = passq_slot();
  b.wb = reinterpret_cast<const bf16x8*>(static_cast<const char*>(packed_s16) + (size_t)F_FRAGS * 1024);
  b.acts = acts; b.d_raw = d_raw; b.M = M; b.dz = dz; b.astride = astride16; b.zstride = zstride16;
  const int64_t nsuper = ((M + 31) / 32 + NW - 1) / NW;
  return launch<s16_bwd_kernel>("mlp backward chain (split bf16)", dim3(persistent_grid(nsuper, persistent_wgs)), dim3(64 * NW),
                                BwdRing::LDS_BYTES, s, b);
}

int g_dw_variant = 1;

int launch_dw_kernel(const DwArgs& d, int workgroups, bool split_bf16, hipStream_t s) {
  return with_bool(split_bf16, [&](auto split) {
    return launch<s16_dw_kernel<decltype(split)::value>>(split_bf16 ? "mlp dW (split bf16)" : "mlp dW (bf16)", dim3(workgroups), dim3(64 * DW_WAVES),
                                                         DW_LDS_BYTES, s, d);
  });
}

}
}
```

nerf_meets_mlx_amd/engine/trainer.py:

```python
import os
from typing import Dict, Optional

import numpy as np
import torch

from .. import parallel, sampling
from ..models.NeRF import Adam, NeRF
from ..ops import index
from ..rendering import ray, render


class Trainer:
    def __init__(self, images: torch.Tensor, poses: torch.Tensor, K, near: float = 2.0, far: float = 6.0,
                 N_rand: int = 1024, n_depth_samples: int = 64, N_importance: int = 128, lrate: float = 5e-4,
                 lrate_decay: int = 500, white_bkgd: bool = True, ref_quirks: bool = True, seed: int = 0,
                 device="cuda", chunk: int = 1024 * 32, precision: int = 22, overlap_comm: bool = True):
        self.device = torch.device(device)
        self.images = images.to(self.device, torch.float32).contiguous()
        self.poses = poses.float().cpu()
        self.K = np.asarray(K, dtype=np.float64)
        self.H, self.W = int(images.shape[1]), int(images.shape[2])
        self.near, self.far = near, far
        self.N_rand, self.n, self.N = N_rand, n_depth_samples, N_importance
        self.lrate, self.lrate_decay = lrate, lrate_decay
        self.white_bkgd, self.q, self.chunk = white_bkgd, ref_quirks, chunk
        self.rank, self.world = parallel.world()
        self.seed = seed
        mk = lambda s: NeRF(channel_input=63, channel_input_views=27, is_use_view_directions=True,
                            device=self.device, seed=s, precision=precision)
        self.precision = precision
        self.coarse = mk(seed)
        self.fine = mk(seed + 1) if N_importance > 0 else None
        self.coarse.name = "coarse"
        if self.fine is not None:
            self.fine.name = "fine"
        self.opt = Adam(lrate, betas=(0.9, 0.999), shared_state=ref_quirks)
        self.it = 0
        self._comm = torch.cuda.Stream(device=self.device) if (self.world > 1 and overlap_comm) else None
        self.gen = torch.Generator(device=self.device)
        self.gen.manual_seed(parallel.rank_seed(seed, self.rank, 2))
        self._train_gen = torch.Generator(device=self.device)

    def _join_comm(self):
        if getattr(self, "_comm", None) is not None:
            torch.cuda.current_stream(self.device).wait_stream(self._comm)

    @property
    def fine(self):
        self._join_comm()
        return self._fine

    @fine.setter
    def fine(self, m):
        self._fine = m

    @property
    def opt(self):
        self._join_comm()
        return self._opt

    @opt.setter
    def opt(self, o):
        self._opt = o

    def image_choice(self) -> int:
        return parallel.counter_seed(self.seed, self.rank, 1, self.it) % int(self.images.shape[0])

    def train_uniforms(self, B: int) -> torch.Tensor:
        self._train_gen.manual_seed(parallel.counter_seed(self.seed, self.rank, 2, self.it))
        return torch.rand(B, self.N, device=self.device, generator=self._train_gen)

    def _step_net(self, model: NeRF, rays, z, target, white: bool, join: bool = True):
        raw = model.query(rays, z, ref_quirks=self.q, train=True)
        loss, d_raw, _ = render.composite_mse_backward(raw, z, rays, target, white)
        grads = model.backward(d_raw)
        if self._comm is None:
            parallel.allreduce_sum_(grads)
            self._opt.update(model, grads, grad_scale=1.0 / self.world)
            return loss
        cur = torch.cuda.current_stream(self.device)
        self._comm.wait_stream(cur)
        with torch.cuda.stream(self._comm):
            parallel.allreduce_sum_(grads)
            self._opt.update(model, grads, grad_scale=1.0 / self.world)
        if join:
            cur.wait_stream(self._comm)
        return loss

    def sample_batch(self, pixel_idx: Optional[torch.Tensor] = None, img_i: Optional[int] = None):
        if img_i is None:
            img_i = self.image_choice()
        if pixel_idx is None:
            return ray.sample_batch(self.H, self.W, self.K, self.poses[img_i, :3, :4], self.near, self.far,
                                    self.images[img_i], self.N_rand, parallel.counter_seed(self.seed, self.rank, 3, self.it))
        rays = ray.gen_rays(self.H, self.W, self.K, self.poses[img_i, :3, :4], self.near, self.far, pixel_idx)
        target = index.gather_rows(self.images[img_i].reshape(-1, self.images.shape[-1]), pixel_idx)
        return rays, target

    def train_step(self, rays=None, target=None, u=None) -> Dict[str, torch.Tensor]:
        if rays is None:
            rays, target = self.sample_batch()
        self._opt.learning_rate = self.lrate * (0.1 ** (self.it / (self.lrate_decay * 1000)))
        z = sampling.sample_coarse(rays, self.n)
        out = {"loss_coarse": self._step_net(self.coarse, rays, z, target, self.white_bkgd)}
        if self._fine is not None:
            raw = self.coarse.query(rays, z, ref_quirks=self.q)
            _, _, _, weights, _ = render.composite(raw, z, rays, 0.0, self.white_bkgd)
            if u is None:
                u = self.train_uniforms(rays.shape[0])
            _, z_fine = sampling.importance_sample(z, weights, self.N, u=u)
            white_fine = self.white_bkgd if not self.q else False
            out["loss_fine"] = self._step_net(self._fine, rays, z_fine, target, white_fine, join=False)
        self.it += 1
        return out

    def render_rays(self, rays: torch.Tensor, u=None, background=None):
        if background is not None:
            raise ValueError("Trainer.render_rays: background is a mode of NGPTrainer's march; this renderer composites onto white "
                             "or nothing (white_bkgd)")
        outs = []
        for s in range(0, rays.shape[0], self.chunk):
            r = rays[s:s + self.chunk]
            uu = None if u is None else u[s:s + self.chunk]
            if uu is None and self.N > 0:
                uu = torch.rand(r.shape[0], self.N, device=self.device, generator=self.gen)
            outs.append(render.render_rays_fused(r, self.coarse, self.fine, self.n, self.N, u=uu,
                                                 white_bkgd=self.white_bkgd, ref_quirks=self.q, with_coarse=False)["rgb_map"])
        return torch.cat(outs, 0)

    def render_frame(self, c2w, shard: bool = True, background=None) -> Optional[torch.Tensor]:
        lo, hi = parallel.shard_range(self.H * self.W, self.rank, self.world) if shard else (0, self.H * self.W)
        idx = torch.arange(lo, hi, device=self.device, dtype=torch.int64)
        rays = ray.gen_rays(self.H, self.W, self.K, np.asarray(c2w)[:3, :4], self.near, self.far, idx)
        if background is None:
            rgb = self.render_rays(rays)
        else:
            per_pixel = torch.is_tensor(background) and background.dim() == 2 and background.shape[0] == self.H * self.W
            rgb = self.render_rays(rays, background=background[lo:hi] if per_pixel else background)
        if shard and self.world > 1:
            rgb = parallel.gather_rows_to_rank0(rgb, self.H * self.W)
            if rgb is None:
                return None
        return rgb.reshape(self.H, self.W, 3)

    def psnr(self, c2w, gt: torch.Tensor, background=None) -> float:
        img = self.render_frame(c2w, shard=False, background=background)
        mse = torch.mean((img - gt.to(self.device)) ** 2)
        return float(10.0 * torch.log10(1.0 / mse))

    def _mesh_field(self):
        from .mesh import RELU
        model = self.fine if self.fine is not None else self.coarse
        return (lambda rays, z: model.query(rays, z, ref_quirks=self.q)), RELU

    def _mesh_box(self, aabb):
        if aabb is None:
            raise ValueError("Trainer mesh export: the 8 x 256 field has no scene box, pass aabb=(lo, hi)")
        lo, hi = aabb
        return [float(x) for x in lo], [float(x) for x in hi]

    def density_volume(self, resolution: int, aabb=None) -> torch.Tensor:
        from . import mesh
        lo, hi = self._mesh_box(aabb)
        query, act = self._mesh_field()
        return mesh.density_volume(query, act, resolution, lo, hi, device=self.device)

    def extract_mesh(self, resolution: int = 256, threshold: float = 2.5, aabb=None, colors: bool = True,
                     min_component: int = 0, largest_only: bool = False, opening_radius: int = 0, simplify_grid: int = 0,
                     simplify_placement: str = "quadric", smooth_iterations: int = 0, smooth_lambda: float = 0.5,
                     smooth_mu: float = -0.53):
        from . import mesh
        lo, hi = self._mesh_box(aabb)
        mesh.check_volume_options(min_component, largest_only, opening_radius, mesh.check_mesh_args(resolution, lo, hi, threshold)[0])
        mesh.check_surface_options(simplify_grid, simplify_placement, smooth_iterations, smooth_lambda, smooth_mu)
        query, act = self._mesh_field()
        return mesh.extract(query, act, resolution, threshold, lo, hi, colors=colors, device=self.device,
                            min_component=min_component, largest_only=largest_only, opening_radius=opening_radius,
                            simplify_grid=simplify_grid, simplify_placement=simplify_placement,
                            smooth_iterations=smooth_iterations, smooth_lambda=smooth_lambda, smooth_mu=smooth_mu)

    def mesh_distance(self, mesh, other, n: int = 1 << 20, tau=None, seed: int = 0, aabb=None):
        from . import mesh as M
        lo, hi = self._mesh_box(aabb)
        return M.mesh_distance(mesh, other, n, lo, hi, seed=seed, tau=tau)

    def texture_mesh(self, mesh, texels: int = 8):
        from .mesh import bake_texture
        return bake_texture(self._mesh_field()[0], mesh, texels)

    def project_texture(self, mesh, texels: int = 8, views=None, source: str = "images", mode: str = "blend", fallback: bool = True,
                        depth_tol=None):
        from . import mesh as M
        if source not in ("images", "field"):
            raise ValueError(f"project_texture: source must be 'images' or 'field', got {source!r}")
        n_all = int(self.poses.shape[0])
        idx = list(range(n_all)) if views is None else [int(v) for v in views]
        if any(not 0 <= v < n_all for v in idx):
            raise ValueError(f"project_texture: views must be indices into the {n_all} training poses, got {views!r}")
        if source == "images" and self.images.shape[-1] != 3:
            raise ValueError("project_texture: this trainer holds RGBA frames, which have no colour behind their transparent pixels; "
                             "use source=\"field\"")
        if depth_tol is None:
            try:
                lo, hi = self._mesh_box(None)
            except ValueError:
                raise ValueError("project_texture: this trainer has no scene box to derive depth_tol from, pass depth_tol (a length "
                                 "of the scene, about two voxels of the lattice the mesh came from)") from None
            depth_tol = M.PROJECT_DEPTH_TOL_CELLS * max(h - l for l, h in zip(lo, hi)) / 256.0
        poses = self.poses[idx, :3, :4] if idx else self.poses[:0, :3, :4]
        if source == "images":
            images = self.images[idx].contiguous() if idx else self.images[:0]
        else:
            frames = [self.render_frame(self.poses[v], shard=False).reshape(self.H, self.W, 3) for v in idx]
            images = torch.stack(frames).contiguous() if frames else torch.zeros(0, self.H, self.W, 3, device=self.device)
        fb = self.texture_mesh(mesh, texels) if fallback else None
        return M.project_texture(mesh, images, poses, self.K, texels=texels, depth_tol=depth_tol, mode=mode, fallback=fb,
                                 near=float(self.near))

    def render_mesh(self, mesh, c2w, texture=None, background=None):
        from .mesh import render_mesh
        return render_mesh(mesh, c2w, self.K, self.H, self.W, texture=texture, background=background, near=float(self.near))

    def mesh_psnr(self, mesh, c2w, gt: torch.Tensor, texture=None, background=None) -> float:
        img = self.render_mesh(mesh, c2w, texture=texture, background=background).rgb
        mse = torch.mean((img - gt.to(self.device)) ** 2)
        return float(10.0 * torch.log10(1.0 / mse))

    def mip_texture(self, mesh, texture):
        from .mesh import build_mipmaps
        return build_mipmaps(texture, mesh)

    def render_mesh_mip(self, mesh, c2w, pyramid, background=None, lod_scale: float = 1.0):
        from .mesh import render_mesh_mip
        return render_mesh_mip(mesh, c2w, self.K, self.H, self.W, pyramid, background=background, near=float(self.near),
                               lod_scale=lod_scale)

    def mesh_psnr_mip(self, mesh, c2w, gt: torch.Tensor, pyramid, background=None, lod_scale: float = 1.0) -> float:
        img = self.render_mesh_mip(mesh, c2w, pyramid, background=background, lod_scale=lod_scale).rgb
        mse = torch.mean((img - gt.to(self.device)) ** 2)
        return float(10.0 * torch.log10(1.0 / mse))

    def _checkpoint_buffers(self):
        b = {"coarse": self.coarse}
        if self.fine is not None:
            b["fine"] = self.fine
        return b

    def sync_optimizer_state(self):
        self._join_comm()

    def state_dict(self):
        return {"it": self.it, "seed": int(self.seed),
                "params": {k: m.params.detach().cpu().clone() for k, m in self._checkpoint_buffers().items()},
                "adam": self.opt.state_dict()}

    def load_state_dict(self, sd, allow_legacy_rng: bool = False):
        legacy = [k for k in sd if str(k).startswith("rng_")]
        if (legacy or "seed" not in sd) and not allow_legacy_rng:
            raise ValueError("checkpoint predates the stateless random streams (" + (", ".join(legacy) or "no `seed` entry") +
                             "): resuming it is not a bit-identical continuation of the run that wrote it; pass "
                             "allow_legacy_rng=True to continue on this trainer's (seed, rank, iteration) streams anyway")
        self.it = int(sd["it"])
        bufs = self._checkpoint_buffers()
        params = sd.get("params", {k: sd[k] for k in bufs if k in sd})
        missing = [k for k in bufs if k not in params]
        if missing:
            raise KeyError(f"checkpoint has no parameters for {missing} (has {sorted(params)})")
        for k, m in bufs.items():
            m.load_flat(params[k])
        adam = sd.get("adam", {})
        if "state" not in adam:
            adam = {"state": adam, "step_count": {}}
        self.opt.load_state_dict(adam, device=self.device)
        if "seed" in sd:
            self.seed = int(sd["seed"])
            self.gen.manual_seed(parallel.rank_seed(self.seed, self.rank, 2))

    @staticmethod
    def _npz_path(path: str) -> str:
        return path if path.endswith(".npz") else path + ".npz"

    def save(self, path: str) -> str:
        import json
        sd = self.state_dict()
        arrays = {"it": np.array(sd["it"], dtype=np.int64), "seed": np.array(sd["seed"], dtype=np.int64)}
        for k, t in sd["params"].items():
            arrays[f"params/{k}"] = t.numpy()
        for k, (m, v) in sd["adam"]["state"].items():
            arrays[f"adam/{k}/m"], arrays[f"adam/{k}/v"] = m.numpy(), v.numpy()
            arrays[f"adam/{k}/steps"] = np.array(sd["adam"]["step_count"].get(k, 0), dtype=np.int64)
        arrays["adam_lr"] = np.array(sd["adam"]["learning_rate"], dtype=np.float64)
        for k, t in sd.get("extra", {}).items():
            arrays[f"extra/{k}"] = t.numpy()
        path = self._npz_path(path)
        tmp = path + ".tmp.npz"
        np.savez(tmp, **arrays)
        os.replace(tmp, path)
        return path

    def load(self, path: str, allow_legacy_rng: bool = False):
        import json
        path = path if os.path.exists(path) else self._npz_path(path)
        z = np.load(path)
        sd = {"it": int(z["it"]), "params": {}, "adam": {"state": {}, "step_count": {}}}
        for k in z.files:
            if k.startswith("params/"):
                sd["params"][k[7:]] = torch.from_numpy(z[k])
            elif k.startswith("adam/") and k.endswith("/m"):
                name = k[5:-2]
                sd["adam"]["state"][name] = [torch.from_numpy(z[k]), torch.from_numpy(z[f"adam/{name}/v"])]
                sd["adam"]["step_count"][name] = int(z[f"adam/{name}/steps"])
            elif k.startswith("extra/"):
                sd.setdefault("extra", {})[k[6:]] = torch.from_numpy(z[k])
        if "adam_lr" in z.files:
            sd["adam"]["learning_rate"] = float(z["adam_lr"])
        if "seed" in z.files:
            sd["seed"] = int(z["seed"])
        for k in z.files:
            if k.startswith("rng_"):
                sd[k] = True
        self.load_state_dict(sd, allow_legacy_rng=allow_legacy_rng)
        return sd["it"]
```

nerf_meets_mlx_amd/models/NeRF.py:

```python
import ctypes as C
import math
from typing import Dict, List, Optional

import numpy as np
import torch

from .. import _native as N
from . import embedding

_LAYERS = None


def layer_shapes(n_layers=8, width=256, cin=63, cdir=27, skips=(4,), use_viewdirs=True, cout=4):
    s = [("pos0", width, cin)]
    for i in range(n_layers - 1):
        s.append((f"pos{i + 1}", width, width + cin if i in skips else width))
    if use_viewdirs:
        s += [("feature", width, width), ("alpha", 1, width), ("dir0", width // 2, width + cdir), ("rgb", 3, width // 2)]
    else:
        s += [("output", cout, width)]
    return s


class NeRF:

    def __init__(self, n_layers=8, width_layers=256, channel_input=3, channel_input_views=3, channel_output=4,
                 list_skip_connection_layers=[4], is_use_view_directions=False, device="cuda", seed: Optional[int] = None,
                 precision: int = 22):
        self.D, self.W = n_layers, width_layers
        self.channel_input_pos, self.channel_input_dir = channel_input, channel_input_views
        self.list_skip_connection_layers = list(list_skip_connection_layers)
        self.is_use_view_directions = is_use_view_directions
        self.device = torch.device(device)
        self.shapes = layer_shapes(n_layers, width_layers, channel_input, channel_input_views,
                                   tuple(self.list_skip_connection_layers), is_use_view_directions, channel_output)
        self.n_params = sum(o * i + o for _, o, i in self.shapes)
        self.arch = N.MlpArch(n_layers, width_layers, channel_input, channel_input_views,
                              self.list_skip_connection_layers[0] if len(self.list_skip_connection_layers) == 1 else -1,
                              int(bool(is_use_view_directions)), channel_output, int(precision))
        if precision not in (16, 22, 32):
            raise ValueError("NeRF: precision must be 16 (bf16 MFMA operands), 32 (fp32 MFMA) or 22 (float32 tolerance on the "
                             "16-bit matrix pipe: split-bf16 training, split-fp16 inference)")
        self.precision = int(precision)
        self.out_dim = 4 if is_use_view_directions else channel_output
        rng = np.random.default_rng(seed)
        chunks = []
        for _, o, i in self.shapes:
            k = 1.0 / math.sqrt(i)
            chunks.append(rng.uniform(-k, k, size=(o, i)).astype(np.float32).reshape(-1))
            chunks.append(rng.uniform(-k, k, size=(o,)).astype(np.float32))
        self.params = torch.from_numpy(np.concatenate(chunks)).to(self.device)
        self.grads = torch.zeros_like(self.params)
        self._packed = None
        self._dirty = True
        self._packed_version = -1
        self._ws: Dict[str, torch.Tensor] = {}
        self.name: Optional[str] = None
        self._gen = 0
        self._acts_gen = -1
        self._acts_M = -1

    def parameters(self) -> Dict[str, object]:
        views, off = {}, 0
        for name, o, i in self.shapes:
            views[name] = {"weight": self.params[off:off + o * i].view(o, i), "bias": self.params[off + o * i:off + o * i + o]}
            off += o * i + o
        tree = {"list_linears_pos": [views[f"pos{l}"] for l in range(self.D)]}
        if self.is_use_view_directions:
            tree.update({"list_linears_dir": [views["dir0"]], "feature_linear": views["feature"],
                         "alpha_linear": views["alpha"], "rgb_linear": views["rgb"]})
        else:
            tree["output_linear"] = views["output"]
        return tree

    def trainable(self) -> torch.Tensor:
        if not self.params.requires_grad:
            self.params.requires_grad_(True)
        return self.params

    def load_flat(self, flat: torch.Tensor):
        assert flat.numel() == self.n_params
        with torch.no_grad():
            self.params.copy_(flat.to(self.device, torch.float32).reshape(-1))
        self._dirty = True

    def mark_updated(self):
        self._dirty = True

    def activation_generation(self) -> int:
        return self._acts_gen

    def packed(self) -> torch.Tensor:
        lib = N.lib()
        if self._packed is None:
            nbytes = lib.nerf_mlp_packed_bytes(C.byref(self.arch))
            if nbytes < 0:
                raise ValueError("libnerf_hip error -3: this NeRF architecture / precision has no HIP kernel (supported: "
                                 "n_layers=8, width=256, skips=[4] with in=63+27 + view head [precision 16, 22, 32], or in=40 without "
                                 "view head and out<=4 [16, 22, 32]; n_layers=2, width=64, skips=[] with in=32+16 + view head [16, 22])")
            self._packed = torch.empty(nbytes, dtype=torch.uint8, device=self.device)
        if self._dirty or self.params._version != self._packed_version:
            N.check(lib.nerf_mlp_pack(C.byref(self.arch), N.ptr(self.params), N.ptr(self._packed), N.stream()))
            self._dirty = False
            self._packed_version = self.params._version
        return self._packed

    def _begin_train_pass(self, M: int) -> torch.Tensor:
        acts = self._workspace("acts", N.lib().nerf_mlp_acts_bytes(C.byref(self.arch), M))
        self._gen += 1
        self._acts_gen, self._acts_M = self._gen, M
        return acts

    def _workspace(self, key: str, nbytes: int) -> torch.Tensor:
        t = self._ws.get(key)
        if t is None or t.numel() < nbytes:
            t = torch.empty(nbytes, dtype=torch.uint8, device=self.device)
            self._ws[key] = t
        return t

    def forward(self, x: torch.Tensor, train: bool = False) -> torch.Tensor:
        x = N.f32(x).reshape(-1, x.shape[-1])
        M = x.shape[0]
        out = torch.empty(M, self.out_dim, dtype=torch.float32, device=x.device)
        acts = None
        if train:
            acts = self._begin_train_pass(M)
        N.check(N.lib().nerf_mlp_forward_train(C.byref(self.arch), N.ptr(self.packed()), N.ptr(x), M, N.ptr(out),
                                               N.ptr(acts), N.stream()))
        return out

    __call__ = forward

    def query(self, rays: torch.Tensor, z: torch.Tensor, ref_quirks: bool = True, train: bool = False) -> torch.Tensor:
        B, n = z.shape
        raw = torch.empty(B, n, 4, dtype=torch.float32, device=z.device)
        acts = None
        if train:
            acts = self._begin_train_pass(B * n)
        N.check(N.lib().nerf_query_fused(C.byref(self.arch), N.ptr(self.packed()), N.ptr(rays), N.ptr(z), B, n,
                                         0 if ref_quirks else 1, N.ptr(raw), N.ptr(acts), N.stream()))
        return raw

    def backward(self, d_raw: torch.Tensor, need_input_grad: bool = False, generation: Optional[int] = None):
        d_raw = N.f32(d_raw)
        M = d_raw.numel() // self.out_dim
        if generation is not None and generation != self._acts_gen:
            raise RuntimeError(f"NeRF.backward: the activations of forward #{generation} were overwritten by train-mode "
                               f"forward #{self._acts_gen} of the same model (one activation workspace per model: run "
                               "backward before the next train-mode forward, or use a second model object)")
        assert M == self._acts_M, "backward() needs a matching query/forward(train=True) first"
        dz = self._workspace("dz", N.lib().nerf_mlp_dz_bytes(C.byref(self.arch), M))
        if need_input_grad:
            d_x = torch.empty(M, self.channel_input_pos, dtype=torch.float32, device=d_raw.device)
            N.check(N.lib().nerf_mlp_backward_inputs(C.byref(self.arch), N.ptr(self.packed()), N.ptr(self._ws["acts"]),
                                                     N.ptr(d_raw), M, N.ptr(dz), N.ptr(self.grads), N.ptr(d_x), N.stream()))
            return self.grads, d_x
        N.check(N.lib().nerf_mlp_backward(C.byref(self.arch), N.ptr(self.packed()), N.ptr(self._ws["acts"]),
                                          N.ptr(d_raw), M, N.ptr(dz), N.ptr(self.grads), N.stream()))
        return self.grads


def debug_layer(model: NeRF, kind: str, layer: int) -> torch.Tensor:
    k = {"acts": 0, "dz": 1}[kind]
    w = N.lib().nerf_mlp_debug_width(C.byref(model.arch), k, layer)
    if w < 0:
        raise ValueError("debug_layer: no such (kind, layer) in this model's training stores (include/nerf_hip.h, nerf_mlp_debug_read)")
    M = model._acts_M
    out = torch.empty(M, w, dtype=torch.float32, device=model.device)
    N.check(N.lib().nerf_mlp_debug_read(C.byref(model.arch), N.ptr(model._ws[kind]), k, layer, M, N.ptr(out), N.stream()))
    return out


class Adam:

    def __init__(self, learning_rate: float, betas=(0.9, 0.999), eps: float = 1e-8, bias_correction: bool = False,
                 shared_state: bool = True):
        self.learning_rate = learning_rate
        self.betas, self.eps = betas, eps
        self.bias_correction, self.shared_state = bias_correction, shared_state
        self.state: Dict[str, List[torch.Tensor]] = {}
        self.step_count: Dict[str, int] = {}
        self._auto_names: Dict[int, str] = {}

    def key_of(self, model) -> str:
        if self.shared_state:
            return "shared"
        name = getattr(model, "name", None)
        if name:
            return str(name)
        return self._auto_names.setdefault(id(model), f"model{len(self._auto_names)}")

    def update(self, model: NeRF, grads: Optional[torch.Tensor] = None, grad_scale: float = 1.0, zero_grads: bool = False):
        g = model.grads if grads is None else grads
        key = self.key_of(model)
        if key not in self.state:
            self.state[key] = [torch.zeros_like(model.params), torch.zeros_like(model.params)]
        self.step_count[key] = self.step_count.get(key, 0) + 1
        m, v = self.state[key]
        half = getattr(model, "half", None)
        if zero_grads or g.dtype == torch.int64 or half is not None:
            N.check(N.lib().nerf_adam_step_shadow(N.ptr(model.params), N.ptr(g), N.ptr(m), N.ptr(v), model.n_params,
                                                  float(self.learning_rate), float(self.betas[0]), float(self.betas[1]),
                                                  float(self.eps), int(self.bias_correction), self.step_count[key],
                                                  float(grad_scale), int(g.dtype == torch.int64), int(bool(zero_grads)),
                                                  N.ptr(half), N.stream()))
            if half is not None:
                model.mark_updated(shadow_written=True)
                return
        else:
            N.check(N.lib().nerf_adam_step(N.ptr(model.params), N.ptr(g), N.ptr(m), N.ptr(v), model.n_params,
                                           float(self.learning_rate), float(self.betas[0]), float(self.betas[1]),
                                           float(self.eps), int(self.bias_correction), self.step_count[key],
                                           float(grad_scale), N.stream()))
        model.mark_updated()

    def update_spans(self, model, spans, grad_scale: float = 1.0):
        key = self.key_of(model)
        if key not in self.state:
            self.state[key] = [torch.zeros_like(model.params), torch.zeros_like(model.params)]
        self.step_count[key] = self.step_count.get(key, 0) + 1
        m, v = self.state[key]
        half = getattr(model, "half", None)
        for lo, hi, g in spans:
            assert g.numel() == hi - lo and g.is_contiguous()
            N.check(N.lib().nerf_adam_step_shadow(N.ptr(model.params[lo:hi]), N.ptr(g), N.ptr(m[lo:hi]), N.ptr(v[lo:hi]), hi - lo,
                                                  float(self.learning_rate), float(self.betas[0]), float(self.betas[1]),
                                                  float(self.eps), int(self.bias_correction), self.step_count[key],
                                                  float(grad_scale), int(g.dtype == torch.int64), 0,
                                                  N.ptr(half[lo:hi]) if half is not None else None, N.stream()))
        model.mark_updated()

    def state_dict(self) -> Dict[str, object]:
        return {"state": {k: [t.detach().cpu() for t in v] for k, v in self.state.items()},
                "step_count": dict(self.step_count), "learning_rate": float(self.learning_rate)}

    def load_state_dict(self, sd, device="cuda"):
        self.state = {k: [t.to(device, torch.float32).contiguous().clone() for t in v] for k, v in sd["state"].items()}
        self.step_count = {k: int(v) for k, v in sd.get("step_count", {}).items()}
        for k in self.state:
            self.step_count.setdefault(k, 0)
        if "learning_rate" in sd:
            self.learning_rate = float(sd["learning_rate"])


def inference_wrapper_batch(model, chunk):
    if chunk is None:
        return model
    return lambda x: torch.cat([model.forward(x[i:i + chunk]) for i in range(0, x.shape[0], chunk)], dim=0)


def run_model(pos, embed_pos, dir, embed_dir, model, netchunk=64 * 1024):
    assert len(pos.shape) == 3, f"[ERROR] {pos.shape=} should have dimensions as: [n_rays, n_depth_samples, 3d position]!"
    B, n = pos.shape[0], pos.shape[1]
    x = embedding.embed(pos, embed_pos, dir, embed_dir)
    out = inference_wrapper_batch(model, netchunk)(x)
    return out.reshape(B, n, out.shape[-1])


class NetworkQuery:

    def __init__(self, embed_pos, embed_dir, netchunk, ref_quirks=True):
        self.embed_pos, self.embed_dir, self.netchunk, self.ref_quirks = embed_pos, embed_dir, netchunk, ref_quirks

    def __call__(self, inputs, viewdirs, model):
        return run_model(inputs, self.embed_pos, viewdirs, self.embed_dir, model, netchunk=self.netchunk)

    def fused(self, rays, z, model, train=False):
        return model.query(rays, z, ref_quirks=self.ref_quirks, train=train)


def create_NeRF(args, device="cuda", ref_quirks: bool = True, seed: Optional[int] = 0, precision: int = 22):
    from ..rendering.render import render_rays, render_rays_eval
    is_use_dir = bool(args.use_viewdirs)
    embed_pos, ch_pos = embedding.get_embedder(args.multires, ref_quirks=ref_quirks)
    embed_dir, ch_dir = embedding.get_embedder(args.multires_views, ref_quirks=ref_quirks) if is_use_dir else (None, 0)
    output_ch = 5 if args.N_importance else 4
    query = NetworkQuery(embed_pos, embed_dir, args.netchunk, ref_quirks)
    mk = lambda d, w, s: NeRF(n_layers=d, width_layers=w, channel_input=ch_pos, channel_output=output_ch,
                              list_skip_connection_layers=[4], channel_input_views=ch_dir,
                              is_use_view_directions=is_use_dir, device=device, seed=s, precision=precision)
    model_coarse = mk(args.netdepth, args.netwidth, seed)
    model_fine = mk(args.netdepth_fine, args.netwidth_fine, None if seed is None else seed + 1) if args.N_importance > 0 else None
    optimizer = Adam(learning_rate=args.lrate, betas=(0.9, 0.999), shared_state=ref_quirks)
    kw = {
        "use_viewdirs": is_use_dir, "white_bkgd": args.white_bkgd, "network_query_fn": query, "is_test": True,
        "render_rays_func": render_rays, "network_coarse": model_coarse, "n_depth_samples": args.n_depth_samples,
        "network_fine": model_fine, "perturb": args.perturb, "raw_noise_std": args.raw_noise_std,
        "N_importance": args.N_importance,
    }
    if args.dataset_type != "llff" or args.no_ndc:
        kw["ndc"] = False
        kw["lindisp"] = args.lindisp
    kw_test = kw if ref_quirks else dict(kw)
    kw_test["perturb"] = False
    kw_test["raw_noise_std"] = 0
    kw_test["is_test"] = False
    kw_test["render_rays_func"] = render_rays_eval
    return kw, kw_test, 0, optimizer
```

Measured before the change: 1.330 million.

## Fold feature layer into view-direction layer for split-bf16 training

Adds a train_fold mode that precomposes W' = W_D[:, :256]·W_F, so the training forward and backward chain feed h7 straight into the direction layer and skip the linear feature layer's matmul, activation stores and dZ. The packing writes the folded fragments plus fp32 copies of W_F^T, W_D1 and the bias into freed fragment space, and the factored dW post step uses those copies to recover the gradients of the original weights. The trainer turns the mode on for both coarse and fine models. This cuts one 256x256 layer per sample in forward and backward, at the cost of a repack whenever the parameters change, different rounding because W' is a product, and no feature-layer activations left for debugging.

```diff
diff --git a/nerf_meets_mlx_amd/csrc/mlp.hip b/nerf_meets_mlx_amd/csrc/mlp.hip
--- a/nerf_meets_mlx_amd/csrc/mlp.hip
+++ b/nerf_meets_mlx_amd/csrc/mlp.hip
@@ -1107,6 +1107,7 @@
 static int g_dw16_variant = 1;
 static int g_dw_narrow_first = 1;
 static int g_dw_factor = 1;
+static int g_train_fold = 0;
 static int g_dw_job_mask = 0;
 static int g_mlp_variant = 0;
 static int g_ring_wgs = 0;
@@ -1125,6 +1126,8 @@
   }
   return n[dev];
 }
+static inline bool dw_factored(const Model& m) { return g_dw_factor && m.can_factor() && !g_dw_job_mask && s16::g_dw_variant != 0; }
+static inline bool train_folded(const Model& m) { return g_train_fold && dw_factored(m); }
 static inline int ring_wgs() { return g_ring_wgs > 0 ? g_ring_wgs : cu_count(); }
 static inline unsigned ring_grid(int64_t ntiles) { return persistent_grid((ntiles + 7) / 8, ring_wgs()); }
 
@@ -1150,6 +1153,7 @@
     {"pass_queue", &g_pass_queue, opt_flag, nullptr},
     {"dw_narrow_first", &g_dw_narrow_first, opt_flag, nullptr},
     {"dw_factor", &g_dw_factor, opt_flag, nullptr},
+    {"train_fold", &g_train_fold, opt_flag, nullptr},
     {"f22_tiles", &f22::g_tiles, [](int& v) { return v == 0 || v == 2 || v == 3; }, "nerf_set_option: f22_tiles must be 0 (automatic), 2 or 3"},
 };
 
@@ -1209,7 +1213,7 @@
                              m.stream<bf16x8>(packed, S_FWD16));
     if (!rc && m.prec == Prec::F32) rc = f32::pack(params, m.stream<void>(packed, S_F32), 0, s);
     if (!rc && m.split()) rc = f22::pack(params, m.stream<void>(packed, S_F22), s);
-    if (!rc && m.split()) rc = s16::pack(params, m.stream<void>(packed, S_S16), s);
+    if (!rc && m.split()) rc = s16::pack(params, m.stream<void>(packed, S_S16), train_folded(m), s);
   }
   return rc;
 }
@@ -1300,7 +1304,7 @@
     return f22::forward(m.stream<void>(packed, S_F22), x, rays, z, M, n, freq_mode, out, ring_wgs(), s);
   if (m.split())
     return s16::forward(m.stream<void>(packed, S_S16), m.stream<float>(packed, S_BIAS), x, rays, z, M, n, freq_mode, out, acts,
-                        m.astride(), ring_wgs(), s);
+                        m.astride(), ring_wgs(), train_folded(m), s);
   if (m.prec == Prec::F32) return f32::forward(m.stream<void>(packed, S_F32), x, rays, z, M, n, freq_mode, out, acts, 0, s);
   return x ? launch_fwd<0>(m, packed, x, rays, z, M, n, freq_mode, out, acts, stream)
            : launch_fwd<1>(m, packed, x, rays, z, M, n, freq_mode, out, acts, stream);
@@ -1379,7 +1383,7 @@
     if (!do_wide && nrest) {
       int rc = launch_dw_part(m, rest, nrest, ntiles, acts, dz, grads, s, split_bf16 ? 1 : 0, 0, half, factored ? half : -1);
       if (!rc && factored)
-        rc = launch_dw_factor_post(m.stream<void>(packed, S_S16), m.stream<float>(packed, S_BIAS), rest.aux, grads, s);
+        rc = launch_dw_factor_post(m.stream<void>(packed, S_S16), m.stream<float>(packed, S_BIAS), rest.aux, grads, train_folded(m), s);
       if (rc) return rc;
     }
   }
@@ -1391,7 +1395,7 @@
   const int64_t ntiles = (M + 31) / 32;
   if (m.split()) {
     if (g_bwd_stage != 2) {
-      const int rcs = s16::backward_chain(m.stream<void>(packed, S_S16), acts, d_raw, M, dz, m.astride(), m.zstride(), ring_wgs(), s);
+      const int rcs = s16::backward_chain(m.stream<void>(packed, S_S16), acts, d_raw, M, dz, m.astride(), m.zstride(), ring_wgs(), train_folded(m), s);
       if (rcs) return rcs;
     }
     return check_launch("mlp backward chain");
@@ -1448,7 +1452,7 @@
   if (rc) return rc;
   DwArgs d;
   const int mask = m.shape == Shape::View ? g_dw_job_mask : 0;
-  const bool factored = g_dw_factor && m.can_factor() && !mask && s16::g_dw_variant != 0;
+  const bool factored = dw_factored(m);
   const int nj = m.dw_jobs(d.jobs, mask, factored);
   return launch_dw(m, packed, d, nj, ntiles, acts, dz, grads, s, factored);
 }
diff --git a/nerf_meets_mlx_amd/csrc/mlp_dwf.hip b/nerf_meets_mlx_amd/csrc/mlp_dwf.hip
--- a/nerf_meets_mlx_amd/csrc/mlp_dwf.hip
+++ b/nerf_meets_mlx_amd/csrc/mlp_dwf.hip
@@ -13,6 +13,7 @@
   return (double)(float)wf[frag_elem_offset(hi)] + (double)(float)wf[frag_elem_offset(lo)];
 }
 
+template <bool FOLD>
 __global__ void __launch_bounds__(256) mlp_dw_factor_post_kernel(const __bf16* __restrict__ wf, const float* __restrict__ bias,
                                                                  const float* __restrict__ aux, float* __restrict__ grads) {
   __shared__ double sh[256 * DWF_ROWS];
@@ -20,6 +21,7 @@
   const int t = threadIdx.x;
   const float* G = aux + DWF_G;
   const float* dbD = aux + DWF_DB;
+  const float* cp = reinterpret_cast<const float*>(wf);
   double acc[DWF_ROWS];
 #pragma unroll
   for (int q = 0; q < DWF_ROWS; ++q) acc[q] = 0.0;
@@ -27,7 +29,7 @@
     const int k0 = DWF_ROWS * blockIdx.x;
     for (int e = t; e < 128 * DWF_ROWS; e += 256) {
       const int j = e / DWF_ROWS, q = e % DWF_ROWS;
-      sh[e] = pair_value(wf, fwd_elem_dir0(j, k0 + q));
+      sh[e] = FOLD ? (double)cp[LF::C_WD1 + j * 256 + k0 + q] : pair_value(wf, fwd_elem_dir0(j, k0 + q));
     }
     if (t < 128) sdb[t] = (double)dbD[t];
     __syncthreads();
@@ -50,6 +52,13 @@
       sh[i * DWF_ROWS + q] = (double)G[(j0 + q) * 256 + i];
     }
     __syncthreads();
+    if constexpr (FOLD) {
+      for (int i = 0; i < 256; ++i) {
+        const double w = (double)cp[LF::C_WFT + i * 256 + t];
+#pragma unroll
+        for (int q = 0; q < DWF_ROWS; ++q) acc[q] = __builtin_fma(w, sh[i * DWF_ROWS + q], acc[q]);
+      }
+    } else
     for (int ks = 0; ks < 16; ++ks) {
       for (int h = 0; h < 2; ++h) {
         const FragElem e0 = fwd_elem_feature(t, kperm(ks, h, 0));
@@ -66,16 +75,18 @@
         }
       }
     }
-    const double bf = (double)bias[L::BI_FEAT + t];
+    const double bf = (double)(FOLD ? cp[LF::C_BF + t] : bias[L::BI_FEAT + t]);
 #pragma unroll
     for (int q = 0; q < DWF_ROWS; ++q) grads[L::P_WD + (j0 + q) * 283 + t] = (float)__builtin_fma(bf, (double)dbD[j0 + q], acc[q]);
     if (t < DWF_ROWS) grads[L::P_BD + j0 + t] = dbD[j0 + t];
   }
 }
 
-int launch_dw_factor_post(const void* packed_s16, const float* bias_slots, const float* aux, float* grads, hipStream_t s) {
-  return launch<mlp_dw_factor_post_kernel>("mlp dW post step (factored feature / dir0)", dim3(DWF_BLOCKS_F + DWF_BLOCKS_D), dim3(256), 0, s,
-                                           static_cast<const __bf16*>(packed_s16), bias_slots, aux, grads);
+int launch_dw_factor_post(const void* packed_s16, const float* bias_slots, const float* aux, float* grads, bool fold, hipStream_t s) {
+  return with_bool(fold, [&](auto fd) {
+    return launch<mlp_dw_factor_post_kernel<decltype(fd)::value>>("mlp dW post step (factored feature / dir0)", dim3(DWF_BLOCKS_F + DWF_BLOCKS_D),
+                                                                  dim3(256), 0, s, static_cast<const __bf16*>(packed_s16), bias_slots, aux, grads);
+  });
 }
 
 }
diff --git a/nerf_meets_mlx_amd/csrc/mlp_frag.h b/nerf_meets_mlx_amd/csrc/mlp_frag.h
--- a/nerf_meets_mlx_amd/csrc/mlp_frag.h
+++ b/nerf_meets_mlx_amd/csrc/mlp_frag.h
@@ -163,7 +163,7 @@
 constexpr int64_t DW_PARTIAL_BYTES = (int64_t)DW_MAX_WGS * DW_SLOT_FLOATS * 4;
 constexpr int DWF_G = 0, DWF_DB = 128 * 256, DWF_FLOATS = DWF_DB + 128;
 static_assert(DWF_FLOATS <= DW_SLOT_FLOATS, "the factored job's result fits one partial-tile slot");
-int launch_dw_factor_post(const void* packed_s16, const float* bias_slots, const float* aux, float* grads, hipStream_t s);
+int launch_dw_factor_post(const void* packed_s16, const float* bias_slots, const float* aux, float* grads, bool fold, hipStream_t s);
 int launch_dw_wide_kernel(const DwArgs& d, int workgroups, bool split_bf16, hipStream_t s);
 
 }
diff --git a/nerf_meets_mlx_amd/csrc/mlp_index.h b/nerf_meets_mlx_amd/csrc/mlp_index.h
--- a/nerf_meets_mlx_amd/csrc/mlp_index.h
+++ b/nerf_meets_mlx_amd/csrc/mlp_index.h
@@ -94,6 +94,46 @@
   return L::pw(l) + nn * 256 + row;
 }
 
+namespace LF {
+constexpr int F_A = L::F_FA, F_DIR = F_A + 16, F_RGB = F_DIR + 72, F_TOTAL = F_RGB + 8;
+constexpr int B_RGB = 0, B_DA = 4, B_L7 = B_DA + 72, B_TOTAL = B_L7 + 7 * 128;
+constexpr int B_PADDED = 976;
+constexpr int B_SHIFT = L::B_L7 - B_L7;
+constexpr int C_WFT = 2 * F_TOTAL * 256, C_WFT_END = C_WFT + 256 * 256;
+constexpr int C_WD1 = (2 * L::F_TOTAL + 2 * B_PADDED) * 256, C_BF = C_WD1 + 128 * 256, C_BP = C_BF + 256, C_USED = C_BP + 128;
+constexpr int C_END = (2 * L::F_TOTAL + 2 * 1104) * 256;
+static_assert(C_WFT_END == 2 * L::F_TOTAL * 256, "W_F^T fills the forward stream's freed fragments exactly");
+static_assert(C_USED <= C_END, "the copies fit the transposed stream's freed fragments");
+}
+__host__ __device__ constexpr int fold_wp(int n, int k) { return -2 - (n * 256 + k); }
+__host__ __device__ constexpr bool is_fold_wp(int src) { return src <= -2; }
+__host__ __device__ constexpr int fold_wp_n(int src) { return (-2 - src) >> 8; }
+__host__ __device__ constexpr int fold_wp_k(int src) { return (-2 - src) & 255; }
+
+__host__ __device__ constexpr int fwd_index_fold(int f, int r, int h, int j) {
+  if (f < LF::F_A) return fwd_index(f, r, h, j);
+  if (f < LF::F_DIR) return r == 0 ? L::P_WA + kperm(f - LF::F_A, h, j) : -1;
+  if (f < LF::F_RGB) {
+    const int g = f - LF::F_DIR;
+    const int nt = g / 18, ks = g % 18;
+    const int kk = kperm(ks, h, j), n = 32 * nt + r;
+    if (kk < 256) return fold_wp(n, kk);
+    return (kk - 256) < 27 ? L::P_WD + n * 283 + kk : -1;
+  }
+  const int ks = f - LF::F_RGB;
+  return r < 3 ? L::P_WR + r * 128 + kperm(ks, h, j) : -1;
+}
+__host__ __device__ constexpr int bwd_index_fold(int f, int r, int h, int j) {
+  if (f < LF::B_DA) return bwd_index(f, r, h, j);
+  if (f < LF::B_L7) {
+    const int g = f - LF::B_DA, kt = g / 9, ns = g % 9;
+    const int nn = kperm(ns, h, j), row = 32 * kt + r;
+    if (ns < 8) return fold_wp(nn, row);
+    return nn == 128 ? L::P_WA + row : -1;
+  }
+  return bwd_index(f + LF::B_SHIFT, r, h, j);
+}
+
 __host__ __device__ constexpr int bias_index(int s) {
   if (s < L::BI_FEAT) return L::pb(s >> 8) + (s & 255);
   if (s < L::BI_ALPHA) return L::P_BF + (s - L::BI_FEAT);
@@ -120,6 +160,12 @@
 __host__ __device__ constexpr FragElem fwd_elem_dir0(int row, int col) {
   return FragElem{L::F_DIR + 18 * (row >> 5) + kperm_ks(col), row & 31, kperm_h(col), kperm_j(col)};
 }
+__host__ __device__ constexpr FragElem fold_elem_fwd(int n, int k) {
+  return FragElem{LF::F_DIR + 18 * (n >> 5) + kperm_ks(k), n & 31, kperm_h(k), kperm_j(k)};
+}
+__host__ __device__ constexpr FragElem fold_elem_bwd(int n, int k) {
+  return FragElem{LF::B_DA + 9 * (k >> 5) + kperm_ks(n), k & 31, kperm_h(n), kperm_j(n)};
+}
 __host__ __device__ constexpr int frag_elem_offset(const FragElem& e) { return (e.f * 64 + 32 * e.h + e.r) * 8 + e.j; }
 
 }
diff --git a/nerf_meets_mlx_amd/csrc/mlp_s16.h b/nerf_meets_mlx_amd/csrc/mlp_s16.h
--- a/nerf_meets_mlx_amd/csrc/mlp_s16.h
+++ b/nerf_meets_mlx_amd/csrc/mlp_s16.h
@@ -11,11 +11,16 @@
 constexpr int F_FRAGS = 2368, B_FRAGS = 2200, B_PADDED = 2208;
 constexpr int64_t PACKED_BYTES = (int64_t)(F_FRAGS + B_PADDED) * 1024;
 
-int pack(const float* params, void* packed_s16, hipStream_t s);
+int pack(const float* params, void* packed_s16, bool fold, hipStream_t s);
 int forward(const void* packed_s16, const float* bias_slots, const float* x, const float* rays, const float* z, int64_t M,
-            int n, int freq_mode, float* out, void* acts, int64_t astride16, int persistent_wgs, hipStream_t s);
+            int n, int freq_mode, float* out, void* acts, int64_t astride16, int persistent_wgs, bool fold, hipStream_t s);
 int backward_chain(const void* packed_s16, const void* acts, const float* d_raw, int64_t M, void* dz, int64_t astride16,
-                   int64_t zstride16, int persistent_wgs, hipStream_t s);
+                   int64_t zstride16, int persistent_wgs, bool fold, hipStream_t s);
+int pack_folded(const float* params, void* packed_s16, hipStream_t s);
+int forward_folded(const void* packed_s16, const float* bias_slots, const float* x, const float* rays, const float* z, int64_t M,
+                   int n, int freq_mode, float* out, void* acts, int64_t astride16, int persistent_wgs, hipStream_t s);
+int backward_chain_folded(const void* packed_s16, const void* acts, const float* d_raw, int64_t M, void* dz, int64_t astride16,
+                          int64_t zstride16, int persistent_wgs, hipStream_t s);
 int launch_dw_kernel(const DwArgs& d, int workgroups, bool split_bf16, hipStream_t s);
 extern int g_dw_variant;
 
diff --git a/nerf_meets_mlx_amd/csrc/mlp_s16.hip b/nerf_meets_mlx_amd/csrc/mlp_s16.hip
--- a/nerf_meets_mlx_amd/csrc/mlp_s16.hip
+++ b/nerf_meets_mlx_amd/csrc/mlp_s16.hip
@@ -1,232 +1,11 @@
-#include "mlp_s16_dev.h"
+#include "mlp_s16_view.h"
 #include "mlp_pack.h"
-#include "mlp_s16.h"
-
-#ifndef NERF_S16_RELOAD_PE
-#define NERF_S16_RELOAD_PE 0
-#endif
 
 namespace nerf {
 namespace s16 {
 
-constexpr int F_CHUNKS = F_FRAGS / RING_CHUNK;
-constexpr int B_CHUNKS = B_PADDED / RING_CHUNK;
-static_assert(F_CHUNKS * RING_CHUNK == F_FRAGS && B_CHUNKS * RING_CHUNK == B_PADDED, "whole ring chunks");
-static_assert(F_FRAGS == 2 * L::F_TOTAL && B_FRAGS == 2 * L::B_TOTAL, "pair streams");
-static_assert(A_LO == L::A_MASK && A_MASK == 2 * L::A_MASK && A_SLOTS == A_MASK + 9, "activation slots");
-static_assert(Z_LO == L::Z_SLOTS && Z_SLOTS == 2 * L::Z_SLOTS, "dZ slots");
-constexpr int NW = 4;
-
-typedef RingW<F_CHUNKS, F_FRAGS, 4, NW, RING_CHUNK, RING_STAGES, true> FwdRing;
-typedef RingW<B_CHUNKS, B_FRAGS, 4, NW, RING_CHUNK, RING_STAGES, true> BwdRing;
-
-
 struct ViewPairPack : ViewPack { static constexpr int B_PADDED = s16::B_PADDED / 2; };
 static_assert(ViewPairPack::B_PADDED >= L::B_TOTAL, "the padded stream holds every transposed fragment");
-
-
-template <int MODE, class WS>
-__device__ __forceinline__ void fwd_tiles(const FwdArgs& a, WS& ws, int64_t tile0, int64_t ntiles, int lane, PassQueue& pq) {
-  const int r = lane & 31, h = lane >> 5;
-  bf16x8 peh[4], pel[4], dph[2], dpl[2];
-  pq.ask(ws.wv, lane);
-  {
-    const int64_t tile = tile0 < ntiles ? tile0 : ntiles - 1;
-    const int64_t m = clamp_sample(tile * 32 + r, a.M);
-    if (MODE == 0) {
-      const float* row = a.x + m * 90;
-#pragma unroll
-      for (int ks = 0; ks < 4; ++ks) row_pairs<SplitBf16>(row, ks, h, 63, peh[ks], pel[ks]);
-#pragma unroll
-      for (int ks = 0; ks < 2; ++ks) row_pairs<SplitBf16>(row + 63, ks, h, 27, dph[ks], dpl[ks]);
-    } else {
-      const Sample sm = load_sample(a.rays, a.z, m, a.n);
-      encode_pairs<SinCodyWaite, SplitBf16, 0, 63, 10>(sm.p, a.fr.pos, h, peh[0], pel[0]); encode_pairs<SinCodyWaite, SplitBf16, 1, 63, 10>(sm.p, a.fr.pos, h, peh[1], pel[1]);
-      encode_pairs<SinCodyWaite, SplitBf16, 2, 63, 10>(sm.p, a.fr.pos, h, peh[2], pel[2]); encode_pairs<SinCodyWaite, SplitBf16, 3, 63, 10>(sm.p, a.fr.pos, h, peh[3], pel[3]);
-      encode_pairs<SinCodyWaite, SplitBf16, 0, 27, 4>(sm.d, a.fr.dir, h, dph[0], dpl[0]); encode_pairs<SinCodyWaite, SplitBf16, 1, 27, 4>(sm.d, a.fr.dir, h, dph[1], dpl[1]);
-    }
-  }
-  pq.publish(ws.wv);
-  store_frags<4>(a.acts, tile0, a.astride, L::A_PE, peh, r, h); store_frags<4>(a.acts, tile0, a.astride, A_LO + L::A_PE, pel, r, h);
-  store_frags<2>(a.acts, tile0, a.astride, L::A_DPE, dph, r, h); store_frags<2>(a.acts, tile0, a.astride, A_LO + L::A_DPE, dpl, r, h);
-
-  bf16x8 hah[16], hal[16], hbh[16], hbl[16];
-  u32x4 mk;
-#define SINK(slot0) PairSink{a.acts, tile0, a.astride, slot0, A_LO, r, h}
-#define MASK_BEGIN() mk = u32x4{0u, 0u, 0u, 0u}
-#define MASK_STORE(layer) *reinterpret_cast<u32x4*>(frag_ptr(a.acts, tile0, a.astride, A_MASK + (layer), r, h)) = mk
-  MASK_BEGIN();
-  layer_fwd<4, 8, true, true>(ws, L::F_L0, 0, peh, pel, hah, hal, mk, lane, SINK(L::A_H0));
-  MASK_STORE(0);
-  MASK_BEGIN();
-  layer_fwd<16, 8, true, true>(ws, L::F_L1 + 0 * 128, 256, hah, hal, hbh, hbl, mk, lane, SINK(L::A_H0 + 16));
-  MASK_STORE(1);
-  MASK_BEGIN();
-  layer_fwd<16, 8, true, true>(ws, L::F_L1 + 1 * 128, 512, hbh, hbl, hah, hal, mk, lane, SINK(L::A_H0 + 32));
-  MASK_STORE(2);
-  MASK_BEGIN();
-  layer_fwd<16, 8, true, true>(ws, L::F_L1 + 2 * 128, 768, hah, hal, hbh, hbl, mk, lane, SINK(L::A_H0 + 48));
-  MASK_STORE(3);
-  MASK_BEGIN();
-  layer_fwd<16, 8, true, true>(ws, L::F_L1 + 3 * 128, 1024, hbh, hbl, hah, hal, mk, lane, SINK(L::A_H0 + 64));
-  MASK_STORE(4);
-  {
-    bf16x8 cth[20], ctl[20];
-#pragma unroll
-    for (int k = 0; k < 4; ++k) {
-#if NERF_S16_RELOAD_PE
-      cth[k] = *frag_ptr(a.acts, tile0, a.astride, L::A_PE + k, r, h);
-      ctl[k] = *frag_ptr(a.acts, tile0, a.astride, A_LO + L::A_PE + k, r, h);
-#else
-      cth[k] = peh[k]; ctl[k] = pel[k];
-#endif
-    }
-#pragma unroll
-    for (int k = 0; k < 16; ++k) { cth[4 + k] = hah[k]; ctl[4 + k] = hal[k]; }
-    MASK_BEGIN();
-    layer_fwd<20, 8, true, true>(ws, L::F_L5, 1280, cth, ctl, hbh, hbl, mk, lane, SINK(L::A_H0 + 80));
-    MASK_STORE(5);
-  }
-  MASK_BEGIN();
-  layer_fwd<16, 8, true, true>(ws, L::F_L6, 1536, hbh, hbl, hah, hal, mk, lane, SINK(L::A_H0 + 96));
-  MASK_STORE(6);
-  MASK_BEGIN();
-  layer_fwd<16, 8, true, true>(ws, L::F_L7, 1792, hah, hal, hbh, hbl, mk, lane, SINK(L::A_H0 + 112));
-  MASK_STORE(7);
-  layer_fwd<16, 8, false, false>(ws, L::F_FA, L::BI_FEAT, hbh, hbl, hah, hal, mk, lane, SINK(L::A_FEAT));
-  const float alpha = head<16>(ws, L::F_FA + 128, L::BI_ALPHA, hbh, hbl, lane)[0];
-  bf16x8 hdh[8], hdl[8];
-  {
-    bf16x8 cth[18], ctl[18];
-#pragma unroll
-    for (int k = 0; k < 16; ++k) { cth[k] = hah[k]; ctl[k] = hal[k]; }
-#pragma unroll
-    for (int k = 0; k < 2; ++k) {
-#if NERF_S16_RELOAD_PE
-      cth[16 + k] = *frag_ptr(a.acts, tile0, a.astride, L::A_DPE + k, r, h);
-      ctl[16 + k] = *frag_ptr(a.acts, tile0, a.astride, A_LO + L::A_DPE + k, r, h);
-#else
-      cth[16 + k] = dph[k]; ctl[16 + k] = dpl[k];
-#endif
-    }
-    MASK_BEGIN();
-    layer_fwd<18, 4, true, true>(ws, L::F_DIR, L::BI_DIR, cth, ctl, hdh, hdl, mk, lane, SINK(L::A_HD));
-    MASK_STORE(8);
-  }
-  const f32x16 rgb = head<8>(ws, L::F_RGB, L::BI_RGB, hdh, hdl, lane);
-  const int64_t m = tile0 * 32 + r;
-  if (h == 0 && tile0 < ntiles && m < a.M) {
-    float4 o; o.x = rgb[0]; o.y = rgb[1]; o.z = rgb[2]; o.w = alpha;
-    *reinterpret_cast<float4*>(a.out + m * 4) = o;
-  }
-#undef SINK
-#undef MASK_BEGIN
-#undef MASK_STORE
-}
-
-template <int MODE>
-__global__ void __launch_bounds__(64 * NW) s16_fwd_kernel(FwdArgs a) {
-  const int lane = threadIdx.x & 63;
-  const int wv = __builtin_amdgcn_readfirstlane(threadIdx.x >> 6);
-  const int64_t ntiles = (a.M + 31) >> 5, nsuper = (ntiles + NW - 1) / NW;
-  FwdRing ws;
-  ws.wsrc = reinterpret_cast<const char*>(a.wf);
-  ws.lane16 = 16 * lane;
-  ws.lds0 = __builtin_amdgcn_readfirstlane(lds_addr_of(ring_smem));
-  ws.wv = wv;
-  ws.start(lane);
-  ring_load_bias(a.bias, L::BI_TOTAL, FwdRing::BIAS_OFF);
-  __syncthreads();
-  PassQueue pq;
-  pq.init(a.queue, ws.lds0 + FwdRing::BIAS_OFF);
-  for (int64_t sp = blockIdx.x; sp < nsuper;) {
-    int ln = lane;
-    asm volatile("" : "+v"(ln));
-    ws.new_pass();
-    fwd_tiles<MODE>(a, ws, sp * NW + wv, ntiles, ln, pq);
-    sp = pq.next(sp);
-  }
-  ws.drain();
-  pq.leave();
-}
-
-
-struct BwdArgs {
-  unsigned* queue;
-  const bf16x8* wb;
-  const void* acts;
-  const float* d_raw;
-  int64_t M;
-  void* dz;
-  int64_t astride, zstride;
-};
-
-template <class WS>
-__device__ __forceinline__ void bwd_tiles(const BwdArgs& a, WS& ws, int64_t tile0, int64_t ntiles, int lane, PassQueue& pq) {
-  const int r = lane & 31, h = lane >> 5;
-  const bool live = tile0 < ntiles;
-  pq.ask(ws.wv, lane);
-  const int64_t tile = live ? tile0 : ntiles - 1;
-  bf16x8 zrh[1], zrl[1], zah[1], zal[1];
-  {
-    const int64_t m = tile * 32 + r;
-    float4 g = make_float4(0.f, 0.f, 0.f, 0.f);
-    if (live && m < a.M && h == 0) g = *reinterpret_cast<const float4*>(a.d_raw + m * 4);
-    float vr[8] = {g.x, g.y, g.z, 0.f, 0.f, 0.f, 0.f, 0.f}, va[8] = {g.w, 0.f, 0.f, 0.f, 0.f, 0.f, 0.f, 0.f};
-    split_slots<8>(vr, zrh, zrl);
-    split_slots<8>(va, zah, zal);
-  }
-  pq.publish(ws.wv);
-  u32x4 mk[9];
-#pragma unroll
-  for (int l = 0; l < 9; ++l)
-    mk[l] = *reinterpret_cast<const u32x4*>(frag_ptr(const_cast<void*>(a.acts), tile, a.astride, A_MASK + l, r, h));
-#define ZSINK(slot0) PairSink{a.dz, tile0, a.zstride, slot0, Z_LO, r, h}
-  ZSINK(L::Z_RGB).put(0, zrh[0], zrl[0]);
-  ZSINK(L::Z_A).put(0, zah[0], zal[0]);
-  bf16x8 zdh[8], zdl[8];
-  layer_bwd<1, 4, true>(ws, L::B_RGB, zrh, zrl, zdh, zdl, mk[8], lane, ZSINK(L::Z_D));
-  bf16x8 zxh[16], zxl[16], zyh[16], zyl[16];
-  layer_bwd<8, 8, false>(ws, L::B_DIR, zdh, zdl, zxh, zxl, mk[8], lane, ZSINK(L::Z_F));
-  {
-    bf16x8 cth[17], ctl[17];
-#pragma unroll
-    for (int k = 0; k < 16; ++k) { cth[k] = zxh[k]; ctl[k] = zxl[k]; }
-    cth[16] = zah[0]; ctl[16] = zal[0];
-    layer_bwd<17, 8, true>(ws, L::B_FA, cth, ctl, zyh, zyl, mk[7], lane, ZSINK(L::Z_L0 + 112));
-  }
-  layer_bwd<16, 8, true>(ws, L::B_L7, zyh, zyl, zxh, zxl, mk[6], lane, ZSINK(L::Z_L0 + 96));
-  layer_bwd<16, 8, true>(ws, L::B_L6, zxh, zxl, zyh, zyl, mk[5], lane, ZSINK(L::Z_L0 + 80));
-  layer_bwd<16, 8, true>(ws, L::B_L5, zyh, zyl, zxh, zxl, mk[4], lane, ZSINK(L::Z_L0 + 64));
-  layer_bwd<16, 8, true>(ws, L::B_L4 + 0 * 128, zxh, zxl, zyh, zyl, mk[3], lane, ZSINK(L::Z_L0 + 48));
-  layer_bwd<16, 8, true>(ws, L::B_L4 + 1 * 128, zyh, zyl, zxh, zxl, mk[2], lane, ZSINK(L::Z_L0 + 32));
-  layer_bwd<16, 8, true>(ws, L::B_L4 + 2 * 128, zxh, zxl, zyh, zyl, mk[1], lane, ZSINK(L::Z_L0 + 16));
-  layer_bwd<16, 8, true>(ws, L::B_L4 + 3 * 128, zyh, zyl, zxh, zxl, mk[0], lane, ZSINK(L::Z_L0 + 0));
-#undef ZSINK
-}
-
-__global__ void __launch_bounds__(64 * NW) s16_bwd_kernel(BwdArgs a) {
-  const int lane = threadIdx.x & 63;
-  const int wv = __builtin_amdgcn_readfirstlane(threadIdx.x >> 6);
-  const int64_t ntiles = (a.M + 31) >> 5, nsuper = (ntiles + NW - 1) / NW;
-  BwdRing ws;
-  ws.wsrc = reinterpret_cast<const char*>(a.wb);
-  ws.lane16 = 16 * lane;
-  ws.lds0 = __builtin_amdgcn_readfirstlane(lds_addr_of(ring_smem));
-  ws.wv = wv;
-  ws.start(lane);
-  PassQueue pq;
-  pq.init(a.queue, ws.lds0 + BwdRing::BIAS_OFF);
-  for (int64_t sp = blockIdx.x; sp < nsuper;) {
-    int ln = lane;
-    asm volatile("" : "+v"(ln));
-    ws.new_pass();
-    bwd_tiles(a, ws, sp * NW + wv, ntiles, ln, pq);
-    sp = pq.next(sp);
-  }
-  ws.drain();
-  pq.leave();
-}
 
 #ifndef NERF_DWX
 #define NERF_DWX 0
@@ -557,14 +336,17 @@
 }
 
 
-int pack(const float* params, void* packed_s16, hipStream_t s) {
+int pack(const float* params, void* packed_s16, bool fold, hipStream_t s) {
   bf16x8* wf = static_cast<bf16x8*>(packed_s16);
+  if (fold) return pack_folded(params, packed_s16, s);
   return launch<pack_streams_kernel<ViewPairPack, SplitBf16, false>>("nerf_mlp_pack (split-bf16 image)", dim3(pack_blocks<ViewPairPack, false>()),
                                                                      dim3(256), 0, s, params, wf, wf + (size_t)F_FRAGS * 64, nullptr, 0);
 }
 
 int forward(const void* packed_s16, const float* bias_slots, const float* x, const float* rays, const float* z, int64_t M,
-            int n, int freq_mode, float* out, void* acts, int64_t astride16, int persistent_wgs, hipStream_t s) {
+            int n, int freq_mode, float* out, void* acts, int64_t astride16, int persistent_wgs, bool fold, hipStream_t s) {
+  if (fold)
+    return forward_folded(packed_s16, bias_slots, x, rays, z, M, n, freq_mode, out, acts, astride16, persistent_wgs, s);
   FwdArgs a;
   a.queue = passq_slot();
   a.wf = reinterpret_cast<const bf16x8*>(packed_s16);
@@ -573,20 +355,21 @@
   fill_freqs(a.fr.pos, a.fr.dir, freq_mode);
   const int64_t nsuper = ((M + 31) / 32 + NW - 1) / NW;
   return with_bool(x != nullptr, [&](auto rows) {
-    return launch<s16_fwd_kernel<decltype(rows)::value ? 0 : 1>>("mlp training forward (split bf16)", dim3(persistent_grid(nsuper, persistent_wgs)),
-                                                                  dim3(64 * NW), FwdRing::LDS_BYTES, s, a);
+    return launch<s16_fwd_kernel<decltype(rows)::value ? 0 : 1, false>>("mlp training forward (split bf16)", dim3(persistent_grid(nsuper, persistent_wgs)),
+                                                                         dim3(64 * NW), FwdRing::LDS_BYTES, s, a);
   });
 }
 
 int backward_chain(const void* packed_s16, const void* acts, const float* d_raw, int64_t M, void* dz, int64_t astride16,
-                   int64_t zstride16, int persistent_wgs, hipStream_t s) {
+                   int64_t zstride16, int persistent_wgs, bool fold, hipStream_t s) {
+  if (fold) return backward_chain_folded(packed_s16, acts, d_raw, M, dz, astride16, zstride16, persistent_wgs, s);
   BwdArgs b;
   b.queue = passq_slot();
   b.wb = reinterpret_cast<const bf16x8*>(static_cast<const char*>(packed_s16) + (size_t)F_FRAGS * 1024);
   b.acts = acts; b.d_raw = d_raw; b.M = M; b.dz = dz; b.astride = astride16; b.zstride = zstride16;
   const int64_t nsuper = ((M + 31) / 32 + NW - 1) / NW;
-  return launch<s16_bwd_kernel>("mlp backward chain (split bf16)", dim3(persistent_grid(nsuper, persistent_wgs)), dim3(64 * NW),
-                                BwdRing::LDS_BYTES, s, b);
+  return launch<s16_bwd_kernel<false>>("mlp backward chain (split bf16)", dim3(persistent_grid(nsuper, persistent_wgs)), dim3(64 * NW),
+                                       BwdRing::LDS_BYTES, s, b);
 }
 
 int g_dw_variant = 1;
diff --git a/nerf_meets_mlx_amd/csrc/mlp_s16_view.h b/nerf_meets_mlx_amd/csrc/mlp_s16_view.h
--- /dev/null
+++ b/nerf_meets_mlx_amd/csrc/mlp_s16_view.h
@@ -0,0 +1,259 @@
+#pragma once
+#include <type_traits>
+#include "mlp_s16_dev.h"
+#include "mlp_s16.h"
+
+#ifndef NERF_S16_RELOAD_PE
+#define NERF_S16_RELOAD_PE 0
+#endif
+
+namespace nerf {
+namespace s16 {
+
+constexpr int F_CHUNKS = F_FRAGS / RING_CHUNK;
+constexpr int B_CHUNKS = B_PADDED / RING_CHUNK;
+static_assert(F_CHUNKS * RING_CHUNK == F_FRAGS && B_CHUNKS * RING_CHUNK == B_PADDED, "whole ring chunks");
+static_assert(F_FRAGS == 2 * L::F_TOTAL && B_FRAGS == 2 * L::B_TOTAL, "pair streams");
+static_assert(A_LO == L::A_MASK && A_MASK == 2 * L::A_MASK && A_SLOTS == A_MASK + 9, "activation slots");
+static_assert(Z_LO == L::Z_SLOTS && Z_SLOTS == 2 * L::Z_SLOTS, "dZ slots");
+constexpr int NW = 4;
+
+typedef RingW<F_CHUNKS, F_FRAGS, 4, NW, RING_CHUNK, RING_STAGES, true> FwdRing;
+typedef RingW<B_CHUNKS, B_FRAGS, 4, NW, RING_CHUNK, RING_STAGES, true> BwdRing;
+constexpr int FF_FRAGS = 2 * LF::F_TOTAL, FB_FRAGS = 2 * LF::B_TOTAL, FB_PADDED = 2 * LF::B_PADDED;
+constexpr int FF_CHUNKS = FF_FRAGS / RING_CHUNK;
+constexpr int FB_CHUNKS = FB_PADDED / RING_CHUNK;
+typedef RingW<FF_CHUNKS, FF_FRAGS, 4, NW, RING_CHUNK, RING_STAGES, true> FwdRingFold;
+typedef RingW<FB_CHUNKS, FB_FRAGS, 4, NW, RING_CHUNK, RING_STAGES, true> BwdRingFold;
+constexpr int ring_chunks(int frags) { return (frags + RING_CHUNK - 1) / RING_CHUNK; }
+static_assert(F_CHUNKS == ring_chunks(F_FRAGS) && B_CHUNKS == ring_chunks(B_FRAGS), "ring chunk counts of the unfolded streams");
+static_assert(FF_CHUNKS == ring_chunks(FF_FRAGS) && FB_CHUNKS == ring_chunks(FB_FRAGS), "ring chunk counts of the folded streams");
+static_assert(FF_CHUNKS * RING_CHUNK == FF_FRAGS && FB_CHUNKS * RING_CHUNK == FB_PADDED && FB_PADDED >= FB_FRAGS, "whole ring chunks (folded)");
+static_assert(FF_FRAGS % 4 == 0 && FB_FRAGS % 4 == 0, "a pass is whole fragment groups");
+static_assert(FF_FRAGS == F_FRAGS - 256 && FB_FRAGS == B_FRAGS - 256, "the fold removes 128 pairs from each stream");
+static_assert((int64_t)LF::C_END * 4 == PACKED_BYTES && (int64_t)LF::C_WFT * 4 == (int64_t)FF_FRAGS * 1024 &&
+              (int64_t)LF::C_WD1 * 4 == (int64_t)(F_FRAGS + FB_PADDED) * 1024, "the fp32 copies start where the folded streams end");
+
+
+
+template <int MODE, bool FOLD, class WS>
+__device__ __forceinline__ void fwd_tiles(const FwdArgs& a, WS& ws, int64_t tile0, int64_t ntiles, int lane, PassQueue& pq) {
+  const int r = lane & 31, h = lane >> 5;
+  bf16x8 peh[4], pel[4], dph[2], dpl[2];
+  pq.ask(ws.wv, lane);
+  {
+    const int64_t tile = tile0 < ntiles ? tile0 : ntiles - 1;
+    const int64_t m = clamp_sample(tile * 32 + r, a.M);
+    if (MODE == 0) {
+      const float* row = a.x + m * 90;
+#pragma unroll
+      for (int ks = 0; ks < 4; ++ks) row_pairs<SplitBf16>(row, ks, h, 63, peh[ks], pel[ks]);
+#pragma unroll
+      for (int ks = 0; ks < 2; ++ks) row_pairs<SplitBf16>(row + 63, ks, h, 27, dph[ks], dpl[ks]);
+    } else {
+      const Sample sm = load_sample(a.rays, a.z, m, a.n);
+      encode_pairs<SinCodyWaite, SplitBf16, 0, 63, 10>(sm.p, a.fr.pos, h, peh[0], pel[0]); encode_pairs<SinCodyWaite, SplitBf16, 1, 63, 10>(sm.p, a.fr.pos, h, peh[1], pel[1]);
+      encode_pairs<SinCodyWaite, SplitBf16, 2, 63, 10>(sm.p, a.fr.pos, h, peh[2], pel[2]); encode_pairs<SinCodyWaite, SplitBf16, 3, 63, 10>(sm.p, a.fr.pos, h, peh[3], pel[3]);
+      encode_pairs<SinCodyWaite, SplitBf16, 0, 27, 4>(sm.d, a.fr.dir, h, dph[0], dpl[0]); encode_pairs<SinCodyWaite, SplitBf16, 1, 27, 4>(sm.d, a.fr.dir, h, dph[1], dpl[1]);
+    }
+  }
+  pq.publish(ws.wv);
+  store_frags<4>(a.acts, tile0, a.astride, L::A_PE, peh, r, h); store_frags<4>(a.acts, tile0, a.astride, A_LO + L::A_PE, pel, r, h);
+  store_frags<2>(a.acts, tile0, a.astride, L::A_DPE, dph, r, h); store_frags<2>(a.acts, tile0, a.astride, A_LO + L::A_DPE, dpl, r, h);
+
+  bf16x8 hah[16], hal[16], hbh[16], hbl[16];
+  u32x4 mk;
+#define SINK(slot0) PairSink{a.acts, tile0, a.astride, slot0, A_LO, r, h}
+#define MASK_BEGIN() mk = u32x4{0u, 0u, 0u, 0u}
+#define MASK_STORE(layer) *reinterpret_cast<u32x4*>(frag_ptr(a.acts, tile0, a.astride, A_MASK + (layer), r, h)) = mk
+  MASK_BEGIN();
+  layer_fwd<4, 8, true, true>(ws, L::F_L0, 0, peh, pel, hah, hal, mk, lane, SINK(L::A_H0));
+  MASK_STORE(0);
+  MASK_BEGIN();
+  layer_fwd<16, 8, true, true>(ws, L::F_L1 + 0 * 128, 256, hah, hal, hbh, hbl, mk, lane, SINK(L::A_H0 + 16));
+  MASK_STORE(1);
+  MASK_BEGIN();
+  layer_fwd<16, 8, true, true>(ws, L::F_L1 + 1 * 128, 512, hbh, hbl, hah, hal, mk, lane, SINK(L::A_H0 + 32));
+  MASK_STORE(2);
+  MASK_BEGIN();
+  layer_fwd<16, 8, true, true>(ws, L::F_L1 + 2 * 128, 768, hah, hal, hbh, hbl, mk, lane, SINK(L::A_H0 + 48));
+  MASK_STORE(3);
+  MASK_BEGIN();
+  layer_fwd<16, 8, true, true>(ws, L::F_L1 + 3 * 128, 1024, hbh, hbl, hah, hal, mk, lane, SINK(L::A_H0 + 64));
+  MASK_STORE(4);
+  {
+    bf16x8 cth[20], ctl[20];
+#pragma unroll
+    for (int k = 0; k < 4; ++k) {
+#if NERF_S16_RELOAD_PE
+      cth[k] = *frag_ptr(a.acts, tile0, a.astride, L::A_PE + k, r, h);
+      ctl[k] = *frag_ptr(a.acts, tile0, a.astride, A_LO + L::A_PE + k, r, h);
+#else
+      cth[k] = peh[k]; ctl[k] = pel[k];
+#endif
+    }
+#pragma unroll
+    for (int k = 0; k < 16; ++k) { cth[4 + k] = hah[k]; ctl[4 + k] = hal[k]; }
+    MASK_BEGIN();
+    layer_fwd<20, 8, true, true>(ws, L::F_L5, 1280, cth, ctl, hbh, hbl, mk, lane, SINK(L::A_H0 + 80));
+    MASK_STORE(5);
+  }
+  MASK_BEGIN();
+  layer_fwd<16, 8, true, true>(ws, L::F_L6, 1536, hbh, hbl, hah, hal, mk, lane, SINK(L::A_H0 + 96));
+  MASK_STORE(6);
+  MASK_BEGIN();
+  layer_fwd<16, 8, true, true>(ws, L::F_L7, 1792, hah, hal, hbh, hbl, mk, lane, SINK(L::A_H0 + 112));
+  MASK_STORE(7);
+  if constexpr (!FOLD) layer_fwd<16, 8, false, false>(ws, L::F_FA, L::BI_FEAT, hbh, hbl, hah, hal, mk, lane, SINK(L::A_FEAT));
+  const float alpha = head<16>(ws, FOLD ? LF::F_A : L::F_FA + 128, L::BI_ALPHA, hbh, hbl, lane)[0];
+  bf16x8 hdh[8], hdl[8];
+  {
+    bf16x8 cth[18], ctl[18];
+#pragma unroll
+    for (int k = 0; k < 16; ++k) { cth[k] = FOLD ? hbh[k] : hah[k]; ctl[k] = FOLD ? hbl[k] : hal[k]; }
+#pragma unroll
+    for (int k = 0; k < 2; ++k) {
+#if NERF_S16_RELOAD_PE
+      cth[16 + k] = *frag_ptr(a.acts, tile0, a.astride, L::A_DPE + k, r, h);
+      ctl[16 + k] = *frag_ptr(a.acts, tile0, a.astride, A_LO + L::A_DPE + k, r, h);
+#else
+      cth[16 + k] = dph[k]; ctl[16 + k] = dpl[k];
+#endif
+    }
+    MASK_BEGIN();
+    layer_fwd<18, 4, true, true>(ws, FOLD ? LF::F_DIR : L::F_DIR, L::BI_DIR, cth, ctl, hdh, hdl, mk, lane, SINK(L::A_HD));
+    MASK_STORE(8);
+  }
+  const f32x16 rgb = head<8>(ws, FOLD ? LF::F_RGB : L::F_RGB, L::BI_RGB, hdh, hdl, lane);
+  const int64_t m = tile0 * 32 + r;
+  if (h == 0 && tile0 < ntiles && m < a.M) {
+    float4 o; o.x = rgb[0]; o.y = rgb[1]; o.z = rgb[2]; o.w = alpha;
+    *reinterpret_cast<float4*>(a.out + m * 4) = o;
+  }
+#undef SINK
+#undef MASK_BEGIN
+#undef MASK_STORE
+}
+
+template <int MODE, bool FOLD>
+__global__ void __launch_bounds__(64 * NW) s16_fwd_kernel(FwdArgs a) {
+  typedef std::conditional_t<FOLD, FwdRingFold, FwdRing> Ring;
+  const int lane = threadIdx.x & 63;
+  const int wv = __builtin_amdgcn_readfirstlane(threadIdx.x >> 6);
+  const int64_t ntiles = (a.M + 31) >> 5, nsuper = (ntiles + NW - 1) / NW;
+  Ring ws;
+  ws.wsrc = reinterpret_cast<const char*>(a.wf);
+  ws.lane16 = 16 * lane;
+  ws.lds0 = __builtin_amdgcn_readfirstlane(lds_addr_of(ring_smem));
+  ws.wv = wv;
+  ws.start(lane);
+  if constexpr (FOLD) {
+    const float* bp = reinterpret_cast<const float*>(a.wf) + LF::C_BP;
+    for (int i = threadIdx.x; i < L::BI_TOTAL; i += blockDim.x) {
+      const bool dir = i >= L::BI_DIR && i < L::BI_DIR + 128;
+      *reinterpret_cast<float*>(ring_smem + Ring::BIAS_OFF + 4 * i) = dir ? bp[i - L::BI_DIR] : a.bias[i];
+    }
+  } else ring_load_bias(a.bias, L::BI_TOTAL, Ring::BIAS_OFF);
+  __syncthreads();
+  PassQueue pq;
+  pq.init(a.queue, ws.lds0 + Ring::BIAS_OFF);
+  for (int64_t sp = blockIdx.x; sp < nsuper;) {
+    int ln = lane;
+    asm volatile("" : "+v"(ln));
+    ws.new_pass();
+    fwd_tiles<MODE, FOLD>(a, ws, sp * NW + wv, ntiles, ln, pq);
+    sp = pq.next(sp);
+  }
+  ws.drain();
+  pq.leave();
+}
+
+
+struct BwdArgs {
+  unsigned* queue;
+  const bf16x8* wb;
+  const void* acts;
+  const float* d_raw;
+  int64_t M;
+  void* dz;
+  int64_t astride, zstride;
+};
+
+template <bool FOLD, class WS>
+__device__ __forceinline__ void bwd_tiles(const BwdArgs& a, WS& ws, int64_t tile0, int64_t ntiles, int lane, PassQueue& pq) {
+  const int r = lane & 31, h = lane >> 5;
+  const bool live = tile0 < ntiles;
+  pq.ask(ws.wv, lane);
+  const int64_t tile = live ? tile0 : ntiles - 1;
+  bf16x8 zrh[1], zrl[1], zah[1], zal[1];
+  {
+    const int64_t m = tile * 32 + r;
+    float4 g = make_float4(0.f, 0.f, 0.f, 0.f);
+    if (live && m < a.M && h == 0) g = *reinterpret_cast<const float4*>(a.d_raw + m * 4);
+    float vr[8] = {g.x, g.y, g.z, 0.f, 0.f, 0.f, 0.f, 0.f}, va[8] = {g.w, 0.f, 0.f, 0.f, 0.f, 0.f, 0.f, 0.f};
+    split_slots<8>(vr, zrh, zrl);
+    split_slots<8>(va, zah, zal);
+  }
+  pq.publish(ws.wv);
+  u32x4 mk[9];
+#pragma unroll
+  for (int l = 0; l < 9; ++l)
+    mk[l] = *reinterpret_cast<const u32x4*>(frag_ptr(const_cast<void*>(a.acts), tile, a.astride, A_MASK + l, r, h));
+#define ZSINK(slot0) PairSink{a.dz, tile0, a.zstride, slot0, Z_LO, r, h}
+  ZSINK(L::Z_RGB).put(0, zrh[0], zrl[0]);
+  ZSINK(L::Z_A).put(0, zah[0], zal[0]);
+  bf16x8 zdh[8], zdl[8];
+  layer_bwd<1, 4, true>(ws, L::B_RGB, zrh, zrl, zdh, zdl, mk[8], lane, ZSINK(L::Z_D));
+  bf16x8 zxh[16], zxl[16], zyh[16], zyl[16];
+  if constexpr (FOLD) {
+    bf16x8 cth[9], ctl[9];
+#pragma unroll
+    for (int k = 0; k < 8; ++k) { cth[k] = zdh[k]; ctl[k] = zdl[k]; }
+    cth[8] = zah[0]; ctl[8] = zal[0];
+    layer_bwd<9, 8, true>(ws, LF::B_DA, cth, ctl, zyh, zyl, mk[7], lane, ZSINK(L::Z_L0 + 112));
+  } else {
+    layer_bwd<8, 8, false>(ws, L::B_DIR, zdh, zdl, zxh, zxl, mk[8], lane, ZSINK(L::Z_F));
+    bf16x8 cth[17], ctl[17];
+#pragma unroll
+    for (int k = 0; k < 16; ++k) { cth[k] = zxh[k]; ctl[k] = zxl[k]; }
+    cth[16] = zah[0]; ctl[16] = zal[0];
+    layer_bwd<17, 8, true>(ws, L::B_FA, cth, ctl, zyh, zyl, mk[7], lane, ZSINK(L::Z_L0 + 112));
+  }
+  constexpr int SH = FOLD ? LF::B_SHIFT : 0;
+  layer_bwd<16, 8, true>(ws, L::B_L7 - SH, zyh, zyl, zxh, zxl, mk[6], lane, ZSINK(L::Z_L0 + 96));
+  layer_bwd<16, 8, true>(ws, L::B_L6 - SH, zxh, zxl, zyh, zyl, mk[5], lane, ZSINK(L::Z_L0 + 80));
+  layer_bwd<16, 8, true>(ws, L::B_L5 - SH, zyh, zyl, zxh, zxl, mk[4], lane, ZSINK(L::Z_L0 + 64));
+  layer_bwd<16, 8, true>(ws, L::B_L4 + 0 * 128 - SH, zxh, zxl, zyh, zyl, mk[3], lane, ZSINK(L::Z_L0 + 48));
+  layer_bwd<16, 8, true>(ws, L::B_L4 + 1 * 128 - SH, zyh, zyl, zxh, zxl, mk[2], lane, ZSINK(L::Z_L0 + 32));
+  layer_bwd<16, 8, true>(ws, L::B_L4 + 2 * 128 - SH, zxh, zxl, zyh, zyl, mk[1], lane, ZSINK(L::Z_L0 + 16));
+  layer_bwd<16, 8, true>(ws, L::B_L4 + 3 * 128 - SH, zyh, zyl, zxh, zxl, mk[0], lane, ZSINK(L::Z_L0 + 0));
+#undef ZSINK
+}
+
+template <bool FOLD>
+__global__ void __launch_bounds__(64 * NW) s16_bwd_kernel(BwdArgs a) {
+  typedef std::conditional_t<FOLD, BwdRingFold, BwdRing> Ring;
+  const int lane = threadIdx.x & 63;
+  const int wv = __builtin_amdgcn_readfirstlane(threadIdx.x >> 6);
+  const int64_t ntiles = (a.M + 31) >> 5, nsuper = (ntiles + NW - 1) / NW;
+  Ring ws;
+  ws.wsrc = reinterpret_cast<const char*>(a.wb);
+  ws.lane16 = 16 * lane;
+  ws.lds0 = __builtin_amdgcn_readfirstlane(lds_addr_of(ring_smem));
+  ws.wv = wv;
+  ws.start(lane);
+  PassQueue pq;
+  pq.init(a.queue, ws.lds0 + Ring::BIAS_OFF);
+  for (int64_t sp = blockIdx.x; sp < nsuper;) {
+    int ln = lane;
+    asm volatile("" : "+v"(ln));
+    ws.new_pass();
+    bwd_tiles<FOLD>(a, ws, sp * NW + wv, ntiles, ln, pq);
+    sp = pq.next(sp);
+  }
+  ws.drain();
+  pq.leave();
+}
+
+}
+}
diff --git a/nerf_meets_mlx_amd/csrc/mlp_s16f.hip b/nerf_meets_mlx_amd/csrc/mlp_s16f.hip
--- /dev/null
+++ b/nerf_meets_mlx_amd/csrc/mlp_s16f.hip
@@ -0,0 +1,109 @@
+#include "mlp_s16_view.h"
+
+namespace nerf {
+namespace s16 {
+
+constexpr int FOLD_PACK_PAIRS = (LF::F_TOTAL + LF::B_PADDED) * 64;
+constexpr int FOLD_PACK_THREADS = FOLD_PACK_PAIRS + (LF::C_WFT_END - LF::C_WFT) + (LF::C_END - LF::C_WD1);
+__global__ void __launch_bounds__(256) pack_fold_kernel(const float* __restrict__ p, bf16x8* __restrict__ img) {
+  const int tid = blockIdx.x * 256 + threadIdx.x;
+  bf16x8* wf = img;
+  bf16x8* wb = img + (size_t)F_FRAGS * 64;
+  float* cp = reinterpret_cast<float*>(img);
+  if (tid < FOLD_PACK_PAIRS) {
+    const bool fw = tid < LF::F_TOTAL * 64;
+    const int t = fw ? tid : tid - LF::F_TOTAL * 64;
+    const int f = t >> 6, lane = t & 63, r = lane & 31, h = lane >> 5;
+    int src[8];
+#pragma unroll
+    for (int j = 0; j < 8; ++j) src[j] = !fw && f >= LF::B_TOTAL ? -1 : fw ? fwd_index_fold(f, r, h, j) : bwd_index_fold(f, r, h, j);
+    const bool wp = is_fold_wp(src[0]);
+    if (wp && !fw) return;
+    float v[8];
+    if (wp) {
+      const int n = fold_wp_n(src[0]);
+      double acc[8];
+#pragma unroll
+      for (int j = 0; j < 8; ++j) acc[j] = 0.0;
+      for (int q = 0; q < 256; ++q) {
+        const double wd = (double)p[L::P_WD + n * 283 + q];
+#pragma unroll
+        for (int j = 0; j < 8; ++j) acc[j] = __builtin_fma(wd, (double)p[L::P_WF + q * 256 + fold_wp_k(src[j])], acc[j]);
+      }
+#pragma unroll
+      for (int j = 0; j < 8; ++j) v[j] = (float)acc[j];
+    } else {
+#pragma unroll
+      for (int j = 0; j < 8; ++j) v[j] = src[j] >= 0 ? p[src[j]] : 0.0f;
+    }
+    bf16x8 o[2];
+    SplitBf16::pack(v, o[0], o[1]);
+    bf16x8* dst = fw ? wf : wb;
+    dst[(2 * f) * 64 + lane] = o[0];
+    dst[(2 * f + 1) * 64 + lane] = o[1];
+    if (wp) {
+      __bf16* tb = reinterpret_cast<__bf16*>(wb);
+#pragma unroll
+      for (int j = 0; j < 8; ++j) {
+        const FragElem e = fold_elem_bwd(fold_wp_n(src[j]), fold_wp_k(src[j]));
+        FragElem eh = e, el = e;
+        eh.f = 2 * e.f; el.f = 2 * e.f + 1;
+        tb[frag_elem_offset(eh)] = o[0][j];
+        tb[frag_elem_offset(el)] = o[1][j];
+      }
+    }
+    return;
+  }
+  int c = tid - FOLD_PACK_PAIRS;
+  if (c < LF::C_WFT_END - LF::C_WFT) {
+    cp[LF::C_WFT + c] = p[L::P_WF + (c & 255) * 256 + (c >> 8)];
+    return;
+  }
+  c += LF::C_WD1 - (LF::C_WFT_END - LF::C_WFT);
+  if (c >= LF::C_END) return;
+  float v = 0.0f;
+  if (c < LF::C_BF) { const int e = c - LF::C_WD1; v = p[L::P_WD + (e >> 8) * 283 + (e & 255)]; }
+  else if (c < LF::C_BP) v = p[L::P_BF + (c - LF::C_BF)];
+  else if (c < LF::C_USED) {
+    const int n = c - LF::C_BP;
+    double acc = 0.0;
+    for (int q = 0; q < 256; ++q) acc = __builtin_fma((double)p[L::P_WD + n * 283 + q], (double)p[L::P_BF + q], acc);
+    v = (float)(acc + (double)p[L::P_BD + n]);
+  }
+  cp[c] = v;
+}
+
+int pack_folded(const float* params, void* packed_s16, hipStream_t s) {
+  return launch<pack_fold_kernel>("nerf_mlp_pack (split-bf16 image, folded)", dim3((FOLD_PACK_THREADS + 255) / 256), dim3(256), 0, s, params,
+                                  static_cast<bf16x8*>(packed_s16));
+}
+
+int forward_folded(const void* packed_s16, const float* bias_slots, const float* x, const float* rays, const float* z, int64_t M,
+                   int n, int freq_mode, float* out, void* acts, int64_t astride16, int persistent_wgs, hipStream_t s) {
+  FwdArgs a;
+  a.queue = passq_slot();
+  a.wf = reinterpret_cast<const bf16x8*>(packed_s16);
+  a.bias = bias_slots;
+  a.x = x; a.rays = rays; a.z = z; a.M = M; a.n = n; a.out = out; a.acts = acts; a.astride = astride16;
+  fill_freqs(a.fr.pos, a.fr.dir, freq_mode);
+  const int64_t nsuper = ((M + 31) / 32 + NW - 1) / NW;
+  return with_bool(x != nullptr, [&](auto rows) {
+    return launch<s16_fwd_kernel<decltype(rows)::value ? 0 : 1, true>>("mlp training forward (split bf16, folded)",
+                                                                        dim3(persistent_grid(nsuper, persistent_wgs)), dim3(64 * NW),
+                                                                        FwdRingFold::LDS_BYTES, s, a);
+  });
+}
+
+int backward_chain_folded(const void* packed_s16, const void* acts, const float* d_raw, int64_t M, void* dz, int64_t astride16,
+                          int64_t zstride16, int persistent_wgs, hipStream_t s) {
+  BwdArgs b;
+  b.queue = passq_slot();
+  b.wb = reinterpret_cast<const bf16x8*>(static_cast<const char*>(packed_s16) + (size_t)F_FRAGS * 1024);
+  b.acts = acts; b.d_raw = d_raw; b.M = M; b.dz = dz; b.astride = astride16; b.zstride = zstride16;
+  const int64_t nsuper = ((M + 31) / 32 + NW - 1) / NW;
+  return launch<s16_bwd_kernel<true>>("mlp backward chain (split bf16, folded)", dim3(persistent_grid(nsuper, persistent_wgs)), dim3(64 * NW),
+                                      BwdRingFold::LDS_BYTES, s, b);
+}
+
+}
+}
diff --git a/nerf_meets_mlx_amd/engine/trainer.py b/nerf_meets_mlx_amd/engine/trainer.py
--- a/nerf_meets_mlx_amd/engine/trainer.py
+++ b/nerf_meets_mlx_amd/engine/trainer.py
@@ -32,6 +32,9 @@
         self.coarse = mk(seed)
         self.fine = mk(seed + 1) if N_importance > 0 else None
         self.coarse.name = "coarse"
+        for net in (self.coarse, self.fine):
+            if net is not None:
+                net.train_fold = True
         if self.fine is not None:
             self.fine.name = "fine"
         self.opt = Adam(lrate, betas=(0.9, 0.999), shared_state=ref_quirks)
diff --git a/nerf_meets_mlx_amd/models/NeRF.py b/nerf_meets_mlx_amd/models/NeRF.py
--- a/nerf_meets_mlx_amd/models/NeRF.py
+++ b/nerf_meets_mlx_amd/models/NeRF.py
@@ -1,3 +1,4 @@
+import contextlib
 import ctypes as C
 import math
 from typing import Dict, List, Optional
@@ -59,6 +60,11 @@
         self._gen = 0
         self._acts_gen = -1
         self._acts_M = -1
+        self.train_fold = False
+        self._packed_form = 0
+        self._acts_form = 0
+        self._can_fold = (precision == 22 and bool(is_use_view_directions) and n_layers == 8 and width_layers == 256
+                          and channel_input == 63 and channel_input_views == 27 and self.list_skip_connection_layers == [4])
 
     def parameters(self) -> Dict[str, object]:
         views, off = {}, 0
@@ -90,6 +96,29 @@
     def activation_generation(self) -> int:
         return self._acts_gen
 
+    def train_form(self) -> int:
+        if not (self.train_fold and self._can_fold):
+            return 0
+        lib = N.lib()
+        return int(lib.nerf_get_option(b"train_fold") in (0, 1) and lib.nerf_get_option(b"dw_factor") == 1
+                   and lib.nerf_get_option(b"dw22_variant") != 0 and lib.nerf_get_option(b"dw_job_mask") == 0)
+
+    @contextlib.contextmanager
+    def _form(self, form: int):
+        if not self._can_fold:
+            yield
+            return
+        lib = N.lib()
+        before = lib.nerf_get_option(b"train_fold")
+        if before not in (0, 1):
+            yield
+            return
+        N.check(lib.nerf_set_option(b"train_fold", int(form)))
+        try:
+            yield
+        finally:
+            lib.nerf_set_option(b"train_fold", before)
+
     def packed(self) -> torch.Tensor:
         lib = N.lib()
         if self._packed is None:
@@ -99,10 +128,13 @@
                                  "n_layers=8, width=256, skips=[4] with in=63+27 + view head [precision 16, 22, 32], or in=40 without "
                                  "view head and out<=4 [16, 22, 32]; n_layers=2, width=64, skips=[] with in=32+16 + view head [16, 22])")
             self._packed = torch.empty(nbytes, dtype=torch.uint8, device=self.device)
-        if self._dirty or self.params._version != self._packed_version:
-            N.check(lib.nerf_mlp_pack(C.byref(self.arch), N.ptr(self.params), N.ptr(self._packed), N.stream()))
+        form = self.train_form()
+        if self._dirty or self.params._version != self._packed_version or form != self._packed_form:
+            with self._form(form):
+                N.check(lib.nerf_mlp_pack(C.byref(self.arch), N.ptr(self.params), N.ptr(self._packed), N.stream()))
             self._dirty = False
             self._packed_version = self.params._version
+            self._packed_form = form
         return self._packed
 
     def _begin_train_pass(self, M: int) -> torch.Tensor:
@@ -125,8 +157,12 @@
         acts = None
         if train:
             acts = self._begin_train_pass(M)
-        N.check(N.lib().nerf_mlp_forward_train(C.byref(self.arch), N.ptr(self.packed()), N.ptr(x), M, N.ptr(out),
-                                               N.ptr(acts), N.stream()))
+        packed = self.packed()
+        with self._form(self._packed_form):
+            N.check(N.lib().nerf_mlp_forward_train(C.byref(self.arch), N.ptr(packed), N.ptr(x), M, N.ptr(out),
+                                                   N.ptr(acts), N.stream()))
+        if train:
+            self._acts_form = self._packed_form
         return out
 
     __call__ = forward
@@ -137,8 +173,12 @@
         acts = None
         if train:
             acts = self._begin_train_pass(B * n)
-        N.check(N.lib().nerf_query_fused(C.byref(self.arch), N.ptr(self.packed()), N.ptr(rays), N.ptr(z), B, n,
-                                         0 if ref_quirks else 1, N.ptr(raw), N.ptr(acts), N.stream()))
+        packed = self.packed()
+        with self._form(self._packed_form):
+            N.check(N.lib().nerf_query_fused(C.byref(self.arch), N.ptr(packed), N.ptr(rays), N.ptr(z), B, n,
+                                             0 if ref_quirks else 1, N.ptr(raw), N.ptr(acts), N.stream()))
+        if train:
+            self._acts_form = self._packed_form
         return raw
 
     def backward(self, d_raw: torch.Tensor, need_input_grad: bool = False, generation: Optional[int] = None):
@@ -150,18 +190,26 @@
                                "backward before the next train-mode forward, or use a second model object)")
         assert M == self._acts_M, "backward() needs a matching query/forward(train=True) first"
         dz = self._workspace("dz", N.lib().nerf_mlp_dz_bytes(C.byref(self.arch), M))
+        packed = self.packed()
+        if self._packed_form != getattr(self, "_acts_form", 0):
+            raise RuntimeError("NeRF.backward: the training form (train_fold / the options it depends on) changed between the "
+                               "train-mode forward and backward; run the forward again")
         if need_input_grad:
             d_x = torch.empty(M, self.channel_input_pos, dtype=torch.float32, device=d_raw.device)
             N.check(N.lib().nerf_mlp_backward_inputs(C.byref(self.arch), N.ptr(self.packed()), N.ptr(self._ws["acts"]),
                                                      N.ptr(d_raw), M, N.ptr(dz), N.ptr(self.grads), N.ptr(d_x), N.stream()))
             return self.grads, d_x
-        N.check(N.lib().nerf_mlp_backward(C.byref(self.arch), N.ptr(self.packed()), N.ptr(self._ws["acts"]),
-                                          N.ptr(d_raw), M, N.ptr(dz), N.ptr(self.grads), N.stream()))
+        with self._form(self._packed_form):
+            N.check(N.lib().nerf_mlp_backward(C.byref(self.arch), N.ptr(packed), N.ptr(self._ws["acts"]),
+                                              N.ptr(d_raw), M, N.ptr(dz), N.ptr(self.grads), N.stream()))
         return self.grads
 
 
 def debug_layer(model: NeRF, kind: str, layer: int) -> torch.Tensor:
     k = {"acts": 0, "dz": 1}[kind]
+    if layer == 8 and getattr(model, "_acts_form", 0):
+        raise ValueError("debug_layer: a folded model (train_fold) neither computes nor stores the feature layer's activations and "
+                         "dZ (layer 8): its dir0 reads h7 through W' = W_D[:, :256] W_F")
     w = N.lib().nerf_mlp_debug_width(C.byref(model.arch), k, layer)
     if w < 0:
         raise ValueError("debug_layer: no such (kind, layer) in this model's training stores (include/nerf_hip.h, nerf_mlp_debug_read)")
```

New measurement: 1.366 million, median of 6. 1.03x the previous value.
